# ClimateImpactLab/climate_toolbox

Hardware: AMD Instinct MI355X
Metric: gridcell-region-timesteps/sec (higher is better)
Workload: dtype f32

## Files before the change

climate_toolbox_amd/_lib.py:

```python
from __future__ import annotations

import ctypes as C
import os

_HERE = os.path.dirname(os.path.abspath(__file__))
LIB_PATH = os.path.join(_HERE, "lib", "libwagg.so")

EKEY, EINTERNAL = -6, -7
PLAN_NO_LC, PLAN_NO_STREAM, PLAN_NO_LINES, PLAN_LC_MFMA, PLAN_SERIAL_BUILD = 1, 2, 4, 8, 16
FORM_FULL, FORM_TILES, FORM_ENTRIES = 0, 1, 2
FORCE_FORM = {None: 0, "auto": 0, "full": 1, "tiles": 2, "entries": 3}
HOST_PIN, HOST_WHOLE, HOST_LINES, HOST_LINES_WHOLE = 1, 2, 4, 8
DENSE_GENERAL_SORT = 16
GATHER_AUTO, GATHER_RCCL, GATHER_PEER = 0, 1, 2
LAYOUT_TG, LAYOUT_GT = 0, 1
OUT_TR, OUT_RT = 0, 1

EXPORTS = (
    "wagg_version", "wagg_device_count", "wagg_shard_rows", "wagg_last_error", "wagg_profile_enable", "wagg_profile_read",
    "wagg_profile_event_overhead",
    "wagg_resolve_cells", "wagg_backup_fill", "wagg_relabel", "wagg_factorize_i64", "wagg_factorize_bytes",
    "wagg_plan_create", "wagg_plan_destroy", "wagg_plan_get_info", "wagg_plan_get_den", "wagg_plan_status",
    "wagg_apply_f32", "wagg_apply_f64", "wagg_apply_host_f32", "wagg_apply_host_f64",
    "wagg_apply_host_ex_f32", "wagg_apply_host_ex_f64", "wagg_dense_apply_host_f32", "wagg_dense_apply_host_f64",
    "wagg_apply_poly_f32", "wagg_apply_poly_f64", "wagg_apply_edd_f32", "wagg_apply_edd_f64",
    "wagg_apply_poly_host_f32", "wagg_apply_poly_host_f64", "wagg_apply_edd_host_f32", "wagg_apply_edd_host_f64",
    "wagg_gather_f32", "wagg_gather_f64",
    "wagg_transform_poly_f32", "wagg_transform_poly_f64", "wagg_transform_edd_f32", "wagg_transform_edd_f64",
    "wagg_any_less_f32", "wagg_any_less_f64",
    "wagg_dense_create_synth", "wagg_dense_create_host", "wagg_dense_create_from_segments", "wagg_dense_create_synth_blocklocal", "wagg_dense_create_synth_sparse", "wagg_dense_get_info",
    "wagg_dense_destroy", "wagg_dense_clone", "wagg_release_scratch", "wagg_scratch_bytes", "wagg_dense_get_den", "wagg_dense_apply_f32", "wagg_dense_apply_poly_f32",
    "wagg_dense_apply_edd_f32", "wagg_dense_saw_inf",
    "wagg_dense_create_synth_f64", "wagg_dense_create_host_f64", "wagg_dense_create_from_segments_f64",
    "wagg_dense_create_synth_blocklocal_f64", "wagg_dense_apply_f64", "wagg_dense_apply_poly_f64", "wagg_dense_apply_edd_f64",
    "wagg_synth_field_f32", "wagg_synth_field_f64",
    "wagg_apply_host_multi_f32", "wagg_apply_host_multi_f64", "wagg_dense_apply_host_multi_f32", "wagg_dense_apply_host_multi_f64",
    "wagg_host_block_plan", "wagg_host_stats_read",
    "wagg_combine_planes_f32", "wagg_combine_planes_f64", "wagg_take_axis", "wagg_relayout_f32", "wagg_relayout_f64",
    "wagg_dense_create_from_csr", "wagg_dense_create_from_csr_f64", "wagg_synth_table_csr", "wagg_relayout_to_f64", "wagg_upload",
    "wagg_shard_group_create", "wagg_shard_group_destroy", "wagg_shard_group_info",
    "wagg_apply_sharded_f32", "wagg_apply_sharded_f64", "wagg_dense_apply_sharded_f32", "wagg_dense_apply_sharded_f64",
    "wagg_apply", "wagg_struct_size", "wagg_struct_ordinals", "wagg_plan_get_info_sized", "wagg_dense_get_info_sized",
    "wagg_host_stats_read_sized",
    "wagg_plan_create_many", "wagg_plan_many_info", "wagg_plan_get_den_many",
    "wagg_period_reduce_f32", "wagg_period_reduce_f64", "wagg_period_reduce_work_bytes",
    "wagg_season_reduce_f32", "wagg_season_reduce_f64", "wagg_season_reduce_work_bytes", "wagg_season_mask",
    "wagg_edd_ladder_reduce_f32", "wagg_edd_ladder_reduce_f64", "wagg_edd_ladder_work_bytes",
    "wagg_bin_days_reduce_f32", "wagg_bin_days_reduce_f64", "wagg_bin_days_work_bytes",
    "wagg_hinge_reduce_f32", "wagg_hinge_reduce_f64", "wagg_hinge_work_bytes",
    "wagg_plan_compact_info", "wagg_plan_compact_cells", "wagg_pack_rows_f32", "wagg_pack_rows_f64",
    "wagg_pack_rows_host_f32", "wagg_pack_rows_host_f64",
)
STRUCT_PLAN_INFO, STRUCT_DENSE_INFO, STRUCT_HOST_STATS, STRUCT_APPLY_DESC = 0, 1, 2, 3
PLAN_SEGMENT, PLAN_DENSE = 0, 1
SRC_DEVICE, SRC_HOST, SRC_HOST_MULTI, SRC_SHARDED = 0, 1, 2, 3
XF_NONE, XF_POLY, XF_EDD = 0, 1, 2
APPLY_EXACT_F32 = 0x10000
APPLY_COMPACT_ROWS = 0x20000
EUNSUPPORTED = -5
T_F32, T_F64 = 7, 8
PERIOD_KEEP_NAN, PERIOD_ROWS_CHECKED = 1, 2
SEASON_INVERT, SEASON_NULL = 1 << 20, 1 << 21
EDD_LADDER_MAX, EDD_LADDER_GROUP = 64, 8
BIN_EDGES_MAX, BIN_GROUP = 65, 8
HINGE_MAX, HINGE_GROUP = 64, 8
HINGE_ABOVE, HINGE_BELOW = 0, 1


class HostStats(C.Structure):
    _fields_ = [(k, C.c_int64) for k in ("calls", "blocks", "registered", "register_failed", "unregistered", "unregister_failed",
                                         "cleanup_failed", "staged_h2d_bytes", "staged_d2h_bytes", "direct_h2d_bytes",
                                         "direct_d2h_bytes", "lines_h2d_bytes", "lines_wait_pack_us", "lines_wait_copy_us", "blocks_retired", "found_page_locked",
                                         "watched_calls", "last_rate_permille")]


def host_stats(reset=False):
    st = HostStats()
    check(load().wagg_host_stats_read_sized(C.byref(st), C.sizeof(st), 1 if reset else 0), "wagg_host_stats_read_sized")
    return {k: int(getattr(st, k)) for k, _ in HostStats._fields_}


def host_block_plan(T, row_bytes, quantum, n_devices=1):
    b, n = C.c_int64(0), C.c_int64(0)
    check(load().wagg_host_block_plan(int(T), int(row_bytes), int(quantum), int(n_devices), C.byref(b), C.byref(n)),
          "wagg_host_block_plan")
    return int(b.value), int(n.value)


class DenseInfo(C.Structure):
    _fields_ = [("G", C.c_int64), ("n_tiles", C.c_int64), ("w_bytes", C.c_int64),
                ("R", C.c_int32), ("n_kt", C.c_int32), ("n_nt", C.c_int32), ("tiled", C.c_int32),
                ("form", C.c_int32), ("elem_bytes", C.c_int32), ("nnz", C.c_int64),
                ("build_s", C.c_double), ("build_upload_s", C.c_double),
                ("est_full_s", C.c_double), ("est_tiles_s", C.c_double), ("est_entries_s", C.c_double), ("walked_entries", C.c_int64),
                ("one_pass_sort", C.c_int32), ("reserved0", C.c_int32)]


class WaggError(RuntimeError):
    pass


class PlanInfo(C.Structure):
    _fields_ = [("nseg_in", C.c_int64), ("nnz", C.c_int64), ("n_groups", C.c_int64),
                ("n_chunks", C.c_int64), ("n_ucells", C.c_int64), ("n_giant", C.c_int64),
                ("n_empty", C.c_int64), ("G", C.c_int64), ("R", C.c_int32), ("lines", C.c_int32),
                ("n_lines128", C.c_int64), ("n_sectors64", C.c_int64), ("n_partial_rows", C.c_int64),
                ("lines_chunks", C.c_int64), ("lines_ucells", C.c_int64), ("lines_lines128", C.c_int64),
                ("n_partial_rows64", C.c_int64), ("lines64_chunks", C.c_int64), ("lines64_ucells", C.c_int64)]


class ApplyDesc(C.Structure):
    _fields_ = [("struct_size", C.c_uint64), ("plan_kind", C.c_int32), ("elem", C.c_int32), ("source", C.c_int32), ("transform", C.c_int32),
                ("plan", C.c_void_p), ("x", C.c_void_p), ("x2", C.c_void_p), ("out", C.c_void_p),
                ("T", C.c_int64), ("ldx", C.c_int64), ("ldo", C.c_int64), ("out_pstride", C.c_int64),
                ("layout", C.c_int32), ("out_layout", C.c_int32), ("offset", C.c_double), ("pow_first", C.c_int32), ("n_pow", C.c_int32),
                ("thresholds", C.c_void_p), ("n_thr", C.c_int32), ("flags", C.c_int32), ("ksplit", C.c_int32), ("n_plans", C.c_int32),
                ("devices", C.c_void_p), ("rows", C.c_void_p), ("group", C.c_void_p), ("root", C.c_int32), ("reserved0", C.c_int32),
                ("stream", C.c_void_p)]


STRUCTS = {STRUCT_PLAN_INFO: PlanInfo, STRUCT_DENSE_INFO: DenseInfo, STRUCT_HOST_STATS: HostStats, STRUCT_APPLY_DESC: ApplyDesc}


def _ptr(v):
    if v is None:
        return None
    if isinstance(v, int):
        return v
    if isinstance(v, C.c_void_p):
        return v.value
    return C.cast(v, C.c_void_p).value


def run(what, **fields):
    d = ApplyDesc()
    d.struct_size = C.sizeof(ApplyDesc)
    d.pow_first = d.n_pow = 1
    for k, v in fields.items():
        setattr(d, k, _ptr(v) if k in _DESC_POINTERS else v)
    check(load().wagg_apply(C.byref(d)), what)


_DESC_POINTERS = frozenset(k for k, t in ApplyDesc._fields_ if t is C.c_void_p)

_lib = None


def load():
    global _lib
    if _lib is not None:
        return _lib
    if not os.path.exists(LIB_PATH):
        raise WaggError(
            "HIP engine not built: %s is missing. Run `python -c \"import __graft_entry__ as g; "
            "g.build()\"` or `make -C climate_toolbox_amd/csrc`. There is no CPU fallback." % LIB_PATH)
    import torch
    L = C.CDLL(LIB_PATH)
    vp, i32p, f64p, f32p = C.c_void_p, C.POINTER(C.c_int32), C.POINTER(C.c_double), C.POINTER(C.c_float)
    L.wagg_version.restype = C.c_int
    L.wagg_shard_rows.argtypes = [C.c_int64, C.c_int, C.c_int, C.POINTER(C.c_int64), C.POINTER(C.c_int64)]
    L.wagg_device_count.restype = C.c_int
    L.wagg_last_error.restype = C.c_char_p
    L.wagg_profile_enable.argtypes = [C.c_int]
    L.wagg_profile_read.argtypes = [f32p, C.c_int, C.POINTER(C.c_int)]
    L.wagg_profile_event_overhead.argtypes = [vp, C.c_int, f32p, f32p]
    u8p, i64p = C.POINTER(C.c_uint8), C.POINTER(C.c_int64)
    L.wagg_resolve_cells.argtypes = [f64p, C.c_int64, f64p, C.c_int64, f64p, f64p, C.c_int64, C.c_int, i32p, i64p]
    L.wagg_backup_fill.argtypes = [f64p, f64p, C.c_int64, f64p]
    L.wagg_relabel.argtypes = [f64p, C.c_int64, C.c_double, C.c_double]
    L.wagg_factorize_i64.argtypes = [i64p, u8p, C.c_int64, i32p, i64p, i64p]
    L.wagg_factorize_bytes.argtypes = [C.c_char_p, C.c_int64, u8p, C.c_int64, i32p, i64p, i64p]
    L.wagg_plan_create.argtypes = [i32p, i32p, f64p, C.c_int64, C.c_int64, C.c_int32, C.c_int64,
                                   C.c_int, C.POINTER(vp)]
    L.wagg_plan_create_many.argtypes = [i32p, i32p, C.POINTER(f64p), C.c_int, C.c_int64, C.c_int64, C.c_int32, C.c_int64,
                                        C.POINTER(i32p), i32p, C.c_int, C.c_int, C.POINTER(vp)]
    L.wagg_plan_many_info.argtypes = [vp, C.POINTER(C.c_int), C.POINTER(C.c_int), i32p, i64p]
    L.wagg_plan_get_den_many.argtypes = [vp, C.c_int, C.c_int, f64p]
    L.wagg_plan_destroy.argtypes = [vp]
    L.wagg_plan_get_info.argtypes = [vp, C.POINTER(PlanInfo)]
    L.wagg_plan_get_info_sized.argtypes = [vp, vp, C.c_uint64]
    L.wagg_dense_get_info_sized.argtypes = [vp, vp, C.c_uint64]
    L.wagg_host_stats_read_sized.argtypes = [vp, C.c_uint64, C.c_int]
    L.wagg_struct_size.argtypes = [C.c_int]
    L.wagg_struct_ordinals.argtypes = [C.c_int, vp, C.c_uint64]
    L.wagg_apply.argtypes = [C.POINTER(ApplyDesc)]
    L.wagg_plan_get_den.argtypes = [vp, f64p]
    L.wagg_plan_status.argtypes = [vp, vp]
    for name in ("wagg_apply_f32", "wagg_apply_f64"):
        getattr(L, name).argtypes = [vp, vp, C.c_int64, C.c_int64, C.c_int, vp, C.c_int64, C.c_int, vp]
    for name in ("wagg_apply_poly_f32", "wagg_apply_poly_f64"):
        getattr(L, name).argtypes = [vp, vp, C.c_int64, C.c_int64, C.c_int, C.c_double, C.c_int, C.c_int, vp,
                                     C.c_int64, C.c_int64, C.c_int, vp]
    for name in ("wagg_apply_poly_host_f32", "wagg_apply_poly_host_f64"):
        getattr(L, name).argtypes = [vp, vp, C.c_int64, C.c_int64, C.c_double, C.c_int, C.c_int, vp, C.c_int64, C.c_int64, C.c_int]
    for name in ("wagg_apply_edd_host_f32", "wagg_apply_edd_host_f64"):
        getattr(L, name).argtypes = [vp, vp, vp, C.c_int64, C.c_int64, C.c_double, f64p, C.c_int, vp, C.c_int64, C.c_int64, C.c_int]
    for name in ("wagg_apply_edd_f32", "wagg_apply_edd_f64"):
        getattr(L, name).argtypes = [vp, vp, vp, C.c_int64, C.c_int64, C.c_int, C.c_double, f64p, C.c_int, vp,
                                     C.c_int64, C.c_int64, C.c_int, vp]
    for name in ("wagg_apply_host_f32", "wagg_apply_host_f64"):
        getattr(L, name).argtypes = [vp, vp, C.c_int64, C.c_int64, C.c_int, vp, C.c_int64, C.c_int]
    for name in ("wagg_apply_host_ex_f32", "wagg_apply_host_ex_f64"):
        getattr(L, name).argtypes = [vp, vp, C.c_int64, C.c_int64, C.c_int, vp, C.c_int64, C.c_int, C.c_int]
    for name in ("wagg_dense_apply_host_f32", "wagg_dense_apply_host_f64"):
        getattr(L, name).argtypes = [vp, vp, C.c_int64, C.c_int64, vp, C.c_int64, C.c_int]
    for name in ("wagg_apply_host_multi_f32", "wagg_apply_host_multi_f64", "wagg_dense_apply_host_multi_f32",
                 "wagg_dense_apply_host_multi_f64"):
        getattr(L, name).argtypes = [C.POINTER(vp), i32p, C.c_int, vp, C.c_int64, C.c_int64, vp, C.c_int64, C.c_int]
    for name in ("wagg_combine_planes_f32", "wagg_combine_planes_f64"):
        getattr(L, name).argtypes = [vp, C.c_int, C.c_int64, f64p, C.c_int64, vp, vp]
    L.wagg_take_axis.argtypes = [vp, C.c_int64, C.c_int64, C.c_int64, vp, C.c_int64, vp, vp]
    for name in ("wagg_relayout_f32", "wagg_relayout_f64"):
        getattr(L, name).argtypes = [vp, C.c_int, C.POINTER(C.c_int64), C.POINTER(C.c_int64), vp, vp]
    L.wagg_relayout_to_f64.argtypes = [vp, C.c_int, C.c_int, C.POINTER(C.c_int64), C.POINTER(C.c_int64), vp, vp]
    L.wagg_upload.argtypes = [vp, vp, C.c_int64]
    L.wagg_host_block_plan.argtypes = [C.c_int64, C.c_int64, C.c_int64, C.c_int, C.POINTER(C.c_int64), C.POINTER(C.c_int64)]
    L.wagg_host_stats_read.argtypes = [C.POINTER(HostStats), C.c_int]
    for name in ("wagg_gather_f32", "wagg_gather_f64"):
        getattr(L, name).argtypes = [vp, C.c_int64, C.c_int64, C.c_int, vp, C.c_int64, vp, C.c_int64,
                                     C.c_int, vp]
    for name in ("wagg_transform_poly_f32", "wagg_transform_poly_f64"):
        getattr(L, name).argtypes = [vp, C.c_int64, C.c_double, C.c_int, vp, vp]
    for name in ("wagg_transform_edd_f32", "wagg_transform_edd_f64"):
        getattr(L, name).argtypes = [vp, vp, C.c_int64, C.c_double, f64p, f64p, C.c_int, vp, vp]
    for name in ("wagg_any_less_f32", "wagg_any_less_f64"):
        getattr(L, name).argtypes = [vp, vp, C.c_int64, C.POINTER(C.c_int), vp]
    L.wagg_dense_create_synth.argtypes = [C.c_int64, C.c_int32, C.c_uint32, C.POINTER(vp)]
    L.wagg_dense_create_host.argtypes = [f32p, C.c_int64, C.c_int32, C.POINTER(vp)]
    L.wagg_dense_create_from_segments.argtypes = [i32p, i32p, f64p, C.c_int64, C.c_int64, C.c_int32, C.c_int,
                                                  C.POINTER(vp)]
    L.wagg_dense_create_synth_blocklocal.argtypes = [C.c_int64, C.c_int32, C.c_uint32, C.c_double, C.POINTER(vp)]
    L.wagg_dense_create_synth_sparse.argtypes = [C.c_int64, C.c_int32, C.c_uint32, C.c_double, C.POINTER(vp)]
    L.wagg_dense_get_info.argtypes = [vp, C.POINTER(DenseInfo)]
    L.wagg_dense_destroy.argtypes = [vp]
    L.wagg_dense_clone.argtypes = [vp, C.c_int, C.POINTER(vp)]
    L.wagg_release_scratch.argtypes = []
    L.wagg_scratch_bytes.argtypes = []
    L.wagg_scratch_bytes.restype = C.c_int64
    L.wagg_dense_get_den.argtypes = [vp, f64p]
    L.wagg_dense_apply_f32.argtypes = [vp, vp, C.c_int64, C.c_int64, vp, C.c_int64, C.c_int, vp]
    L.wagg_dense_apply_poly_f32.argtypes = [vp, vp, C.c_int64, C.c_int64, C.c_double, C.c_int, vp, C.c_int64, C.c_int, vp]
    L.wagg_dense_apply_edd_f32.argtypes = [vp, vp, vp, C.c_int64, C.c_int64, C.c_double, C.c_double, vp, C.c_int64,
                                           C.c_int, vp]
    L.wagg_dense_saw_inf.argtypes = [vp, vp, C.POINTER(C.c_int)]
    L.wagg_dense_create_synth_f64.argtypes = [C.c_int64, C.c_int32, C.c_uint32, C.c_double, C.POINTER(vp)]
    L.wagg_dense_create_synth_blocklocal_f64.argtypes = [C.c_int64, C.c_int32, C.c_uint32, C.c_double, C.POINTER(vp)]
    L.wagg_dense_create_host_f64.argtypes = [f64p, C.c_int64, C.c_int32, C.POINTER(vp)]
    L.wagg_dense_create_from_segments_f64.argtypes = [i32p, i32p, f64p, C.c_int64, C.c_int64, C.c_int32, C.c_int, C.POINTER(vp)]
    for name in ("wagg_dense_create_from_csr", "wagg_dense_create_from_csr_f64"):
        getattr(L, name).argtypes = [i64p, i32p, f64p, C.c_int64, C.c_int32, C.c_int, C.POINTER(vp)]
    L.wagg_synth_table_csr.argtypes = [C.c_int64, C.c_int32, C.c_uint32, C.c_double, C.c_int, i64p, i32p, f64p, C.c_int64, i64p]
    L.wagg_dense_apply_f64.argtypes = [vp, vp, C.c_int64, C.c_int64, vp, C.c_int64, C.c_int, vp]
    L.wagg_dense_apply_poly_f64.argtypes = [vp, vp, C.c_int64, C.c_int64, C.c_double, C.c_int, vp, C.c_int64, C.c_int, vp]
    L.wagg_dense_apply_edd_f64.argtypes = [vp, vp, vp, C.c_int64, C.c_int64, C.c_double, C.c_double, vp, C.c_int64,
                                           C.c_int, vp]
    L.wagg_synth_field_f32.argtypes = [vp, C.c_int64, C.c_int64, C.c_int64, C.c_uint32, C.c_float,
                                       C.c_float, vp]
    L.wagg_synth_field_f64.argtypes = [vp, C.c_int64, C.c_int64, C.c_int64, C.c_uint32, C.c_double,
                                       C.c_double, vp]
    L.wagg_shard_group_create.argtypes = [i32p, C.c_int, C.c_int, C.POINTER(vp)]
    L.wagg_shard_group_destroy.argtypes = [vp]
    L.wagg_shard_group_info.argtypes = [vp, C.POINTER(C.c_int), C.POINTER(C.c_int)]
    for name in ("wagg_apply_sharded_f32", "wagg_apply_sharded_f64", "wagg_dense_apply_sharded_f32", "wagg_dense_apply_sharded_f64"):
        getattr(L, name).argtypes = [vp, C.POINTER(vp), C.POINTER(vp), i64p, C.c_int64, vp, C.c_int64, C.c_int]
    for name in ("wagg_period_reduce_f32", "wagg_period_reduce_f64"):
        getattr(L, name).argtypes = [vp, vp, C.c_int64, C.c_int64, C.c_int64, vp, vp, C.c_int32, C.c_int64, C.c_int, C.c_double, C.c_int,
                                     C.c_int, f64p, C.c_int, C.c_int, vp, C.c_int64, C.c_int64, vp, vp, C.c_int64, vp]
    L.wagg_period_reduce_work_bytes.argtypes = [C.c_int64, C.c_int32, C.c_int64, C.c_int]
    L.wagg_period_reduce_work_bytes.restype = C.c_int64
    for name in ("wagg_season_reduce_f32", "wagg_season_reduce_f64"):
        getattr(L, name).argtypes = [vp, vp, C.c_int64, C.c_int64, C.c_int64, vp, vp, C.c_int32, C.c_int64, vp, vp, C.c_int, C.c_double,
                                     C.c_int, C.c_int, f64p, C.c_int, C.c_int, vp, C.c_int64, C.c_int64, vp, vp, C.c_int64, vp]
    L.wagg_season_reduce_work_bytes.argtypes = [C.c_int64, C.c_int32, C.c_int64, C.c_int]
    L.wagg_season_reduce_work_bytes.restype = C.c_int64
    L.wagg_season_mask.argtypes = [vp, C.c_int64, vp, C.c_int64, vp, vp]
    for name in ("wagg_edd_ladder_reduce_f32", "wagg_edd_ladder_reduce_f64"):
        getattr(L, name).argtypes = [vp, vp, C.c_int64, C.c_int64, C.c_int64, vp, vp, C.c_int32, C.c_int64, vp, vp, C.c_double, f64p,
                                     C.c_int, C.c_int, vp, C.c_int64, C.c_int64, vp, vp, C.c_int64, vp]
    L.wagg_edd_ladder_work_bytes.argtypes = [C.c_int64, C.c_int32, C.c_int64, C.c_int]
    L.wagg_edd_ladder_work_bytes.restype = C.c_int64
    for name in ("wagg_bin_days_reduce_f32", "wagg_bin_days_reduce_f64"):
        getattr(L, name).argtypes = [vp, C.c_int64, C.c_int64, C.c_int64, vp, vp, C.c_int32, C.c_int64, vp, vp, C.c_double, f64p, C.c_int,
                                     C.c_int, vp, C.c_int64, C.c_int64, vp, vp, C.c_int64, vp]
    L.wagg_bin_days_work_bytes.argtypes = [C.c_int64, C.c_int32, C.c_int64, C.c_int]
    L.wagg_bin_days_work_bytes.restype = C.c_int64
    for name in ("wagg_hinge_reduce_f32", "wagg_hinge_reduce_f64"):
        getattr(L, name).argtypes = [vp, C.c_int64, C.c_int64, C.c_int64, vp, vp, C.c_int32, C.c_int64, vp, vp, C.c_double, f64p, C.c_int,
                                     C.c_int, C.c_int, f64p, f64p, f64p, C.c_int, vp, C.c_int64, C.c_int64, vp, vp, C.c_int64, vp]
    L.wagg_hinge_work_bytes.argtypes = [C.c_int64, C.c_int32, C.c_int64, C.c_int]
    L.wagg_hinge_work_bytes.restype = C.c_int64
    L.wagg_plan_compact_info.argtypes = [vp, C.c_int, i64p]
    L.wagg_plan_compact_cells.argtypes = [vp, C.c_int, i32p]
    for name in ("wagg_pack_rows_f32", "wagg_pack_rows_f64"):
        getattr(L, name).argtypes = [vp, vp, vp, C.c_int64, C.c_int64, vp, C.c_int64, vp]
    for name in ("wagg_pack_rows_host_f32", "wagg_pack_rows_host_f64"):
        getattr(L, name).argtypes = [vp, vp, vp, C.c_int64, C.c_int64, vp, C.c_int64, C.c_int]
    for name in EXPORTS:
        fn = getattr(L, name)
        if name not in ("wagg_last_error", "wagg_scratch_bytes", "wagg_period_reduce_work_bytes", "wagg_season_reduce_work_bytes",
                        "wagg_edd_ladder_work_bytes", "wagg_bin_days_work_bytes", "wagg_hinge_work_bytes"):
            fn.restype = C.c_int
    _lib = L
    return L


def check(rc, what):
    if rc != 0:
        msg = load().wagg_last_error().decode("utf-8", "replace")
        err = WaggError("%s failed (%d): %s" % (what, rc, msg))
        err.code = int(rc)
        raise err
```

climate_toolbox_amd/csrc/wagg_common.h:

```cpp
#pragma once
#include <hip/hip_runtime.h>
#include <hip/hip_ext.h>
#include <cstdarg>
#include <cstdint>
#include <cstdio>
#include <cstring>
#include <new>
#include <vector>

#include "../../include/wagg.h"

namespace wagg {

void set_error(const char *fmt, ...);

#define WAGG_HIP(expr)                                                                        \
    do {                                                                                      \
        hipError_t e__ = (expr);                                                              \
        if (e__ != hipSuccess) {                                                              \
            wagg::set_error("%s:%d: %s -> %s", __FILE__, __LINE__, #expr,                     \
                            hipGetErrorString(e__));                                          \
            return WAGG_EHIP;                                                                 \
        }                                                                                     \
    } while (0)

#define WAGG_REQUIRE(cond, ...)                                                               \
    do {                                                                                      \
        if (!(cond)) {                                                                        \
            wagg::set_error(__VA_ARGS__);                                                     \
            return WAGG_EINVAL;                                                               \
        }                                                                                     \
    } while (0)

__host__ __device__ inline uint32_t hash32(uint64_t idx, uint32_t seed) {
    uint32_t lo = (uint32_t)idx, hi = (uint32_t)(idx >> 32);
    uint32_t x = lo ^ (hi * 0x85EBCA6Bu) ^ (seed * 0x9E3779B9u);
    x ^= x >> 16; x *= 0x7FEB352Du; x ^= x >> 15; x *= 0x846CA68Bu; x ^= x >> 16;
    return x;
}
__host__ __device__ inline float hash_u01(uint64_t idx, uint32_t seed) {
    return (float)(hash32(idx, seed) >> 8) * (1.0f / 16777216.0f);
}

constexpr int XF_EDD = -1;

template <typename T> __device__ __forceinline__ T snyder_edd1(T tmin, T tmax, T e) {
    const T M = (tmax + tmin) / T(2), w = (tmax - tmin) / T(2);
    if (!(tmin < e)) return M - e;
    if (!(tmax > e)) return T(0);
    const T pi = T(3.14159265358979323846);
    const T z = (e - M) / w;
    T theta, c;
    if constexpr (sizeof(T) == 4) { theta = asinf(z); c = sqrtf((T(1) - z) * (T(1) + z)); }
    else { theta = asin(z); c = sqrt((T(1) - z) * (T(1) + z)); }
    const T r = ((M - e) * (pi / T(2) - theta) + w * c) / pi;
    return r < T(0) ? T(0) : r;
}

__device__ __forceinline__ float snyder_edd1_finite(float tmin, float tmax, float e) {
    const float M = 0.5f * (tmax + tmin), w = 0.5f * (tmax - tmin);
    const float d = M - e;
    const float z = -d * __builtin_amdgcn_rcpf(w);
    const bool below = tmin < e;
    const float az = (below && tmax > e) ? __builtin_fminf(__builtin_fabsf(z), 1.0f) : 1.0f;
    const float t = 1.0f - az;
    float p = 7.577220821985975e-05f;
    p = __builtin_fmaf(p, az, -0.0003951705584768206f);
    p = __builtin_fmaf(p, az, 0.0010792884277179837f);
    p = __builtin_fmaf(p, az, -0.002406827174127102f);
    p = __builtin_fmaf(p, az, 0.005977150052785873f);
    p = __builtin_fmaf(p, az, -0.022534651681780815f);
    p = __builtin_fmaf(p, az, 0.31830987334251404f);
    const float q = __builtin_amdgcn_sqrtf(t) * t;
    return __builtin_fmaf(w, q * p, below ? __builtin_fmaxf(d, 0.0f) : d);
}
__device__ __forceinline__ double snyder_edd1_finite(double tmin, double tmax, double e) {
    const double M = 0.5 * (tmax + tmin), w = 0.5 * (tmax - tmin);
    const double d = M - e;
    double rw = __builtin_amdgcn_rcp(w);
    rw = __builtin_fma(rw, __builtin_fma(-w, rw, 1.0), rw);
    const bool below = tmin < e;
    const double az = (below && tmax > e) ? __builtin_fmin(__builtin_fabs(d * rw), 1.0) : 1.0;
    const double t = 1.0 - az;
    const double ty = __builtin_amdgcn_rsq(__builtin_fmax(t, 1e-300));
    double st = t * ty;
    st = __builtin_fma(__builtin_fma(-st, st, t), 0.5 * ty, st);
    double p = -8.644295123170258e-07;
    p = __builtin_fma(p, az, 7.147532263874047e-06);
    p = __builtin_fma(p, az, -2.807399717529102e-05);
    p = __builtin_fma(p, az, 7.126284961634285e-05);
    p = __builtin_fma(p, az, -0.0001359898123558899);
    p = __builtin_fma(p, az, 0.0002182750865254441);
    p = __builtin_fma(p, az, -0.0003242640574299061);
    p = __builtin_fma(p, az, 0.000480605991421148);
    p = __builtin_fma(p, az, -0.0007477719612718598);
    p = __builtin_fma(p, az, 0.0012691227365052833);
    p = __builtin_fma(p, az, -0.0024647062510063378);
    p = __builtin_fma(p, az, 0.005985979570242935);
    p = __builtin_fma(p, az, -0.0225351707225776);
    p = __builtin_fma(p, az, 0.3183098861837864);
    return __builtin_fma(w, st * t * p, below ? __builtin_fmax(d, 0.0) : d);
}
template <> __device__ __forceinline__ float snyder_edd1<float>(float tmin, float tmax, float e) {
    const float d = 0.5f * (tmax + tmin) - e;
    const float inner = snyder_edd1_finite(tmin, tmax, e);
    return !(tmin < e) ? d : (!(tmax > e) ? 0.0f : inner);
}

template <typename T> __device__ __forceinline__ T xform1(T x, T off, int pw) {
    const T y = x + off;
    T r = y;
    for (int i = 1; i < pw; ++i) r *= y;
    return r;
}
template <typename V, typename T> __device__ __forceinline__ V xform4(V v, T off, int pw) {
    V r;
#pragma unroll
    for (int c = 0; c < 4; ++c) r[c] = xform1<T>(v[c], off, pw);
    return r;
}

void copy_sized(void *dst, uint64_t dst_size, const void *src, size_t src_size);

hipError_t allow_dynamic_lds(const void *kern, size_t bytes);

bool profile_slot(hipEvent_t *start, hipEvent_t *stop);

inline hipError_t launch_timed_ptr(bool timed, const void *kern, dim3 grid, dim3 block, void **args, size_t shmem, hipStream_t st) {
    hipEvent_t a = nullptr, b = nullptr;
    if (timed && profile_slot(&a, &b)) return hipExtLaunchKernel(kern, grid, block, args, shmem, st, a, b, 0);
    return hipLaunchKernel(kern, grid, block, args, shmem, st);
}
template <typename... Args, typename F = void (*)(Args...)>
inline void launch_timed(bool timed, F kern, dim3 grid, dim3 block, size_t shmem, hipStream_t st, Args... args) {
    hipEvent_t a = nullptr, b = nullptr;
    if (timed && profile_slot(&a, &b)) hipExtLaunchKernelGGL(kern, grid, block, (std::uint32_t)shmem, st, a, b, 0u, args...);
    else hipLaunchKernelGGL(kern, grid, block, shmem, st, args...);
}

hipError_t staged_h2d(void *dst_dev, const void *src_host, size_t bytes, hipStream_t st);
hipError_t staged_d2h_rows(void *dst_host, const void *src_dev, int64_t rows, size_t ld_bytes, size_t row_bytes, hipStream_t st);
inline hipError_t staged_d2h(void *dst_host, const void *src_dev, size_t bytes, hipStream_t st = nullptr) {
    return staged_d2h_rows(dst_host, src_dev, 1, bytes, bytes, st);
}
void clear_error();

hipError_t scratch_alloc(void **p, size_t bytes);
void scratch_free(void *p, bool keep = true);
hipError_t scratch_stream(hipStream_t *st, int role = 0);
void scratch_stream_done(hipStream_t st, int role = 0, bool keep = true);
void release_scratch(int what = 7);
template <typename T>
struct ScratchBuf {
    T *p = nullptr;
    ScratchBuf() = default;
    ScratchBuf(const ScratchBuf &) = delete;
    ScratchBuf &operator=(const ScratchBuf &) = delete;
    hipError_t alloc(size_t count) { return scratch_alloc(reinterpret_cast<void **>(&p), (count ? count : 1) * sizeof(T)); }
    ~ScratchBuf() { if (p) { (void)hipDeviceSynchronize(); scratch_free(p); } }
};

template <typename T>
struct DevBuf {
    T *p = nullptr;
    size_t n = 0;
    DevBuf() = default;
    DevBuf(const DevBuf &) = delete;
    DevBuf &operator=(const DevBuf &) = delete;
    ~DevBuf() { if (p) (void)hipFree(p); }
    hipError_t alloc(size_t count) {
        if (p) { (void)hipFree(p); p = nullptr; }
        n = count;
        hipError_t e = hipMalloc((void **)&p, (count ? count : 1) * sizeof(T));
        if (e == hipErrorOutOfMemory) {
            (void)hipGetLastError();
            release_scratch();
            e = hipMalloc((void **)&p, (count ? count : 1) * sizeof(T));
        }
        return e;
    }
    hipError_t upload(const std::vector<T> &h, hipStream_t st = nullptr) {
        hipError_t e = alloc(h.size());
        if (e != hipSuccess || h.empty()) return e;
        return staged_h2d(p, h.data(), h.size() * sizeof(T), st);
    }
};

}
```

climate_toolbox_amd/csrc/wagg_dense.hip:

```cpp
#include <algorithm>
#include <cfloat>
#include <chrono>
#include <cmath>
#include <limits>
#include <cstdlib>
#include <type_traits>

#include "wagg_dense_int.h"
#include "wagg_entry.h"

namespace wagg {

constexpr int D_MT = 23;
constexpr int D_BN = 256;
constexpr int D_ROWB = 128;
constexpr int D_THREADS = 512;
constexpr int D_WTB = D_BN * D_ROWB;
constexpr int D_WSLOTS = D_WTB / 16;
static_assert(D_WTB / 1024 == 32, "4 one-KiB W pieces per wave");
constexpr int d_xt_bytes(int mt) { return mt * 16 * D_ROWB; }
constexpr int d_buf_bytes(int mt) { return d_xt_bytes(mt) + D_WTB; }
static_assert(2 * d_buf_bytes(D_MT) <= 160 * 1024, "LDS budget");

typedef float f32x4 __attribute__((ext_vector_type(4)));
// ... 159 lines not shown
    }
    (void)R;
}

__global__ void dense_colsum_combine_kernel(const double *__restrict__ part, int n_strips, int n_nt, int32_t R,
                                            double *__restrict__ den) {
    const int64_t r = (int64_t)blockIdx.x * blockDim.x + threadIdx.x;
    if (r >= R) return;
    const int64_t nt = r / D_BN, c = r % D_BN;
    double s = 0.0;
    for (int st = 0; st < n_strips; ++st)
        for (int p = 0; p < 8; ++p) s += part[((int64_t)st * n_nt + nt) * D_WSLOTS + c * 8 + p];
    den[r] = s;
}

__global__ void dense_den32_kernel(const double *__restrict__ den64, float *__restrict__ den32, int32_t R) {
    const int r = blockIdx.x * blockDim.x + threadIdx.x;
    if (r < R) den32[r] = (float)den64[r];
}

template <typename T>
__global__ void dense_scatter_kernel(T *__restrict__ Wp, int n_kt, const int32_t *__restrict__ cell,
                                     const int32_t *__restrict__ region, const T *__restrict__ w, int64_t n) {
    const int64_t i = (int64_t)blockIdx.x * blockDim.x + threadIdx.x;
    if (i < n) Wp[wp_index<T>(cell[i], region[i], n_kt)] = w[i];
}

template <typename T>
__global__ void dense_scatter_at_kernel(T *__restrict__ Wp, const int64_t *__restrict__ at,
                                        const T *__restrict__ w, int64_t n) {
    const int64_t i = (int64_t)blockIdx.x * blockDim.x + threadIdx.x;
    if (i < n) Wp[at[i]] = w[i];
}

template <typename T>
__global__ void dense_synth_blocklocal_kernel(typename DT<T>::vec *__restrict__ Wp, const int32_t *__restrict__ tile_kt,
                                              const int32_t *__restrict__ tile_nt, int64_t n_tiles, int64_t G,
                                              int32_t R, uint32_t seed, float fill) {
    const int64_t stride = (int64_t)gridDim.x * blockDim.x, n_slots = n_tiles * D_WSLOTS;
    for (int64_t s = (int64_t)blockIdx.x * blockDim.x + threadIdx.x; s < n_slots; s += stride) {
        const int64_t ti = s / D_WSLOTS;
        const int64_t kt = tile_kt[ti], nt = tile_nt[ti];
        int cl, kl;
        slot_to_ck<T>((int)(s % D_WSLOTS), cl, kl);
        const int64_t r = nt * D_BN + cl, g0 = kt * DT<T>::BK + kl;
        typename DT<T>::vec v;
#pragma unroll
        for (int c = 0; c < DT<T>::EPP; ++c) {
            const uint64_t id = (uint64_t)(g0 + c) * (uint64_t)R + (uint64_t)r;
            v[c] = (r < R && g0 + c < G && hash_u01(id, seed ^ 0x9e3779b9u) < fill) ? (T)hash_u01(id, seed) : T(0);
        }
        Wp[s] = v;
    }
}

template <typename T>
__global__ void dense_colsum_tiled_kernel(const typename DT<T>::vec *__restrict__ Wp, const int32_t *__restrict__ tile_first,
                                          int32_t R, double *__restrict__ den) {
    const int64_t r = (int64_t)blockIdx.x * blockDim.x + threadIdx.x;
    if (r >= R) return;
    const int64_t nt = r / D_BN, c = r % D_BN;
    double s = 0.0;
    for (int64_t ti = tile_first[nt]; ti < tile_first[nt + 1]; ++ti)
        for (int p = 0; p < 8; ++p) {
            const typename DT<T>::vec v = Wp[ti * D_WSLOTS + c * 8 + p];
#pragma unroll
            for (int e = 0; e < DT<T>::EPP; ++e) s += (double)v[e];
        }
    den[r] = s;
}

template <typename T>
__global__ void dense_pack_w_kernel(const T *__restrict__ W, int64_t G, int32_t R, int n_kt,
                                    int64_t n_slots, typename DT<T>::vec *__restrict__ Wp) {
    const int64_t stride = (int64_t)gridDim.x * blockDim.x;
    for (int64_t s = (int64_t)blockIdx.x * blockDim.x + threadIdx.x; s < n_slots; s += stride) {
        const int64_t tk = s / D_WSLOTS;
        const int64_t kt = tk % n_kt, nt = tk / n_kt;
        int cl, kl;
        slot_to_ck<T>((int)(s % D_WSLOTS), cl, kl);
        const int64_t r = nt * D_BN + cl, g0 = kt * DT<T>::BK + kl;
        typename DT<T>::vec v;
#pragma unroll
        for (int c = 0; c < DT<T>::EPP; ++c) v[c] = (r < R && g0 + c < G) ? W[(g0 + c) * R + r] : T(0);
        Wp[s] = v;
    }
}

}

namespace wagg {

template <typename T>
static int dense_alloc(int64_t G, int32_t R, wagg_dense **out, int64_t stored_tiles = -1, bool spmm = false) {
    constexpr int BK = DT<T>::BK;
    WAGG_REQUIRE(out != nullptr, "out is NULL");
    *out = nullptr;
    WAGG_REQUIRE(G > 0 && R > 0, "bad sizes G=%lld R=%d", (long long)G, R);
    WAGG_REQUIRE((G + BK - 1) / BK < (int64_t)0x7fffffff / 8, "G too large");
    wagg_dense *d = new (std::nothrow) wagg_dense();
    if (!d) { set_error("host allocation failed"); return WAGG_ENOMEM; }
    d->G = G; d->R = R;
    d->f64 = sizeof(T) == 8;
    d->n_kt = (int)((G + BK - 1) / BK);
    d->n_nt = (int)(((int64_t)R + D_BN - 1) / D_BN);
    d->n_tiles = spmm ? 0 : (stored_tiles >= 0 ? stored_tiles : (int64_t)d->n_nt * d->n_kt);
    d->tiled = !spmm && stored_tiles >= 0;
    d->spmm = spmm;
    int dev = 0;
    hipError_t e = hipGetDevice(&dev);
    d->device = dev;
    if (e == hipSuccess) e = hipDeviceGetAttribute(&d->ncu, hipDeviceAttributeMultiprocessorCount, dev);
    if (e == hipSuccess) e = d->nonfinite.alloc(1);
    if (e == hipSuccess) e = hipHostMalloc((void **)&d->inf_host, 2 * sizeof(int), hipHostMallocMapped);
    if (e == hipSuccess) { d->inf_host[0] = d->inf_host[1] = 0; e = hipHostGetDevicePointer((void **)&d->inf_dev, d->inf_host, 0); }
    if (e == hipSuccess) e = d->W.alloc((size_t)(d->w_slots() > 0 ? d->w_slots() : 1) * 4);
    if (e == hipSuccess) e = d->den32.alloc((size_t)R);
    if (e == hipSuccess) e = d->den64.alloc((size_t)R);
    if (e != hipSuccess) {
        set_error("dense W allocation of %.1f GB failed: %s", (double)d->w_slots() * 16e-9, hipGetErrorString(e));
        delete d;
        return e == hipErrorOutOfMemory ? WAGG_ENOMEM : WAGG_EHIP;
    }
    *out = d;
    return WAGG_OK;
}

static int dense_den_to_host(wagg_dense *d, hipStream_t st = nullptr) {
    hipLaunchKernelGGL(dense_den32_kernel, dim3((unsigned)((d->R + 255) / 256)), dim3(256), 0, st,
                       d->den64.p, d->den32.p, d->R);
    WAGG_HIP(hipGetLastError());
    d->den_host.resize((size_t)d->R);
    WAGG_HIP(staged_d2h(d->den_host.data(), d->den64.p, sizeof(double) * (size_t)d->R, st));
    return WAGG_OK;
}

template <typename T>
static int dense_finish_den(wagg_dense *d) {
    typedef typename DT<T>::vec vec_t;
    const int kt_per_block = 128;
    const int n_strips = (d->n_kt + kt_per_block - 1) / kt_per_block;
    dim3 grid((unsigned)d->n_nt, (unsigned)n_strips);
    DevBuf<double> part;
    WAGG_HIP(part.alloc((size_t)n_strips * (size_t)d->n_nt * D_WSLOTS));
    hipLaunchKernelGGL((dense_colsum_kernel<T>), grid, dim3(512), 0, nullptr,
                       reinterpret_cast<const vec_t *>(d->W.p), d->R, d->n_kt, kt_per_block, part.p);
    hipLaunchKernelGGL(dense_colsum_combine_kernel, dim3((unsigned)((d->R + 255) / 256)), dim3(256), 0, nullptr,
                       (const double *)part.p, n_strips, d->n_nt, d->R, d->den64.p);
    WAGG_HIP(hipGetLastError());
    WAGG_HIP(hipDeviceSynchronize());
    return dense_den_to_host(d);
}

static int dense_finish_scales(wagg_dense *d, hipStream_t st = nullptr) {
    if (d->f64 || d->tiled || d->spmm) return WAGG_OK;
    const int kt_per_block = 128;
    const int n_strips = (d->n_kt + kt_per_block - 1) / kt_per_block;
    WAGG_HIP(d->wmax.alloc((size_t)d->n_nt * D_BN));
    WAGG_HIP(hipMemsetAsync(d->wmax.p, 0, sizeof(float) * d->wmax.n, st));
    hipLaunchKernelGGL(dense_colmax_kernel, dim3((unsigned)d->n_nt, (unsigned)n_strips), dim3(512), 0, st,
                       reinterpret_cast<const f32x4 *>(d->W.p), d->n_kt, kt_per_block, reinterpret_cast<unsigned *>(d->wmax.p));
    WAGG_HIP(hipGetLastError());
    return WAGG_OK;
}

static hipError_t dense_set_tiles(wagg_dense *d, const std::vector<int64_t> &tiles, std::vector<int32_t> *nt_out = nullptr,
                                  hipStream_t st = nullptr) {
    std::vector<int32_t> kt(tiles.size() + 2, 0), ntv(tiles.size() + 1, 0);
    std::vector<int64_t> first((size_t)d->n_nt + 1, 0);
    for (size_t i = 0; i < tiles.size(); ++i) {
        kt[i] = (int32_t)(tiles[i] % d->n_kt);
        ntv[i] = (int32_t)(tiles[i] / d->n_kt);
        first[(size_t)ntv[i] + 1]++;
    }
    for (int nt = 0; nt < d->n_nt; ++nt) first[(size_t)nt + 1] += first[(size_t)nt];
    d->nt_first.assign(first.size(), 0);
    for (size_t i = 0; i < first.size(); ++i) d->nt_first[i] = (int32_t)first[i];
    hipError_t e = d->tile_kt.upload(kt, st);
    if (nt_out) *nt_out = ntv;
    return e;
}

static int tile_pieces_for(wagg_dense *d, int n_mb, hipStream_t st, const wagg_dense::TilePieces **out) {
    for (const auto &tp : d->pieces)
        if (tp->n_mb == n_mb) { *out = tp.get(); return WAGG_OK; }
    try {
        std::unique_ptr<wagg_dense::TilePieces> tp(new wagg_dense::TilePieces());
        const int n_nt = d->n_nt;
        const int64_t per_mb = d->n_tiles, total = per_mb * n_mb;
        int64_t n_wg = total / 8;
        if (n_wg > d->ncu) n_wg = d->ncu;
        if (n_wg < 1) n_wg = 1;
        std::vector<int32_t> first_piece((size_t)n_wg + 1, 0), rec, slab_first(2 * (size_t)n_mb * n_nt, 0);
        int64_t pos = 0;
        int slab = 0, w = 0;
        int64_t w_end = total * 1 / n_wg;
        bool nt_major = false;
#ifdef WAGG_DIAG
        if (const char *e = getenv("WAGG_PIECES_ORDER")) nt_major = e[0] == 'n';
#endif
        for (int64_t pair = 0; pair < (int64_t)n_mb * n_nt; ++pair) {
            const int mb = nt_major ? (int)(pair % n_mb) : (int)(pair / n_nt), nt = nt_major ? (int)(pair / n_mb) : (int)(pair % n_nt);
            {
                const int slab0 = slab;
                slab_first[2 * ((size_t)mb * n_nt + nt)] = slab;
                int64_t t0 = d->nt_first[(size_t)nt];
                const int64_t t1 = d->nt_first[(size_t)nt + 1];
                while (t0 < t1) {
                    while (pos >= w_end && w + 1 < n_wg) { ++w; first_piece[(size_t)w] = (int32_t)(rec.size() / 8); w_end = total * (w + 1) / n_wg; }
                    const int64_t room = w + 1 < n_wg ? w_end - pos : t1 - t0;
                    const int64_t take = room < t1 - t0 ? room : t1 - t0;
                    const int32_t r8[8] = {nt, mb, (int32_t)t0, (int32_t)take, slab, 0, 0, 0};
                    rec.insert(rec.end(), r8, r8 + 8);
                    ++slab;
                    t0 += take;
                    pos += take;
                }
                slab_first[2 * ((size_t)mb * n_nt + nt) + 1] = slab - slab0;
            }
        }
        for (int64_t k = w + 1; k <= n_wg; ++k) first_piece[(size_t)k] = (int32_t)(rec.size() / 8);
        tp->n_mb = n_mb; tp->n_wg = (int)n_wg; tp->n_slabs = slab;
        std::vector<int32_t> all;
        all.reserve(first_piece.size() + rec.size() + slab_first.size());
        all.insert(all.end(), first_piece.begin(), first_piece.end());
        all.insert(all.end(), rec.begin(), rec.end());
        tp->slab_first_at = (int64_t)all.size();
        all.insert(all.end(), slab_first.begin(), slab_first.end());
        WAGG_HIP(tp->tab.upload(all, st));
        *out = tp.get();
        d->pieces.push_back(std::move(tp));
        return WAGG_OK;
    } catch (const std::bad_alloc &) { set_error("host allocation failed"); return WAGG_ENOMEM; }
}

constexpr double SPMM_MAX_FILL = 0.10;

struct FormRates { double full, tiled, entries_scale, dma; };
constexpr FormRates FORM_RATES_F32 = {420e12, 144e12, 1.0, 10.1e12};
constexpr FormRates FORM_RATES_F64 = {70e12, 73e12, 0.44, 10.1e12};
static double entry_loop_rate(double mean_list) {
    static const double L[] = {170, 325, 541, 812, 1625}, Rt[] = {30e12, 23e12, 19.5e12, 17.3e12, 15.9e12};
    if (mean_list <= L[0]) return Rt[0];
    for (int i = 1; i < 5; ++i)
        if (mean_list <= L[i]) return Rt[i - 1] + (Rt[i] - Rt[i - 1]) * (mean_list - L[i - 1]) / (L[i] - L[i - 1]);
    return Rt[4];
}

struct FormCost { double t_full, t_tiled, t_entries; };
static FormCost table_form_cost(int64_t G, int elem_bytes, int64_t n_tiles_stored, int64_t n_tiles_all, int64_t walked, int n_rb,
                                int64_t n_lists, int n_nt) {
    const FormRates &rt = elem_bytes == 8 ? FORM_RATES_F64 : FORM_RATES_F32;
    const double tile_flop = 2.0 * (128.0 / elem_bytes) * 256.0;
    FormCost c;
    const int64_t n_kt = n_tiles_all / (n_nt > 0 ? n_nt : 1);
    const double s_max = n_kt / 32 >= 64 ? 64.0 : (n_kt / 32 >= 16 ? (double)(n_kt / 32 / 8 * 8) : 8.0);
    const double util = n_nt * s_max < 256.0 ? n_nt * s_max / 256.0 : 1.0;
    c.t_full = tile_flop * (double)n_tiles_all / (rt.full * util);
    c.t_tiled = tile_flop * (double)n_tiles_stored / rt.tiled;
    const double rate = rt.entries_scale * entry_loop_rate((double)walked / (double)(n_lists > 0 ? n_lists : 1));
    const double t_loop = 2.0 * (double)walked / rate, t_stream = (double)elem_bytes * (double)G * (double)n_rb / rt.dma;
    c.t_entries = t_loop > t_stream ? t_loop : t_stream;
    return c;
}
static void pick_table_form(const FormCost &c, bool *tiled, bool *entries) {
    *entries = c.t_entries < c.t_full && c.t_entries < c.t_tiled;
    *tiled = !*entries && c.t_tiled < c.t_full;
}

static int pick_ksplit(int64_t items, int n_kt) {
    int best = 8;
    double best_eff = 0.0;
    for (int S = 8; S <= 64; S += 8) {
        if (S > 8 && n_kt / S < 32) break;
        const double w = (double)items * S / 256.0;
        const double eff = w / std::ceil(w);
        if (eff > best_eff + 1e-9) { best_eff = eff; best = S; }
        if (eff >= 0.985) break;
    }
    return best;
}

template <typename T>
static int create_synth(int64_t G, int32_t R, uint32_t seed, double fill, wagg_dense **out) {
    typedef typename DT<T>::vec vec_t;
    WAGG_REQUIRE(fill > 0.0 && fill <= 1.0, "fill must be in (0, 1]");
    if (fill < SPMM_MAX_FILL) {
        int rc = dense_alloc<T>(G, R, out, -1, true);
        if (rc != WAGG_OK) return rc;
        rc = spmm_build_synth<T>(*out, seed, fill);
        if (rc != WAGG_OK) { delete *out; *out = nullptr; }
        return rc;
    }
    int rc = dense_alloc<T>(G, R, out);
    if (rc != WAGG_OK) return rc;
    wagg_dense *d = *out;
    hipLaunchKernelGGL((dense_synth_w_kernel<T>), dim3(256 * 32), dim3(256), 0, nullptr,
                       reinterpret_cast<vec_t *>(d->W.p), G, R, d->n_kt, d->w_slots(), seed, (float)fill);
    hipError_t e = hipGetLastError();
    if (e == hipSuccess) rc = dense_finish_den<T>(d); else { set_error("synth launch: %s", hipGetErrorString(e)); rc = WAGG_EHIP; }
    if (rc == WAGG_OK) rc = dense_finish_scales(d);
    if (rc == WAGG_OK && hipDeviceSynchronize() != hipSuccess) { set_error("synth: column maxima"); rc = WAGG_EHIP; }
    if (rc != WAGG_OK) { delete d; *out = nullptr; }
    return rc;
}

template <typename T>
static int create_synth_blocklocal(int64_t G, int32_t R, uint32_t seed, double fill, wagg_dense **out) {
    typedef typename DT<T>::vec vec_t;
    constexpr int BK = DT<T>::BK;
    WAGG_REQUIRE(out != nullptr, "out is NULL");
    *out = nullptr;
    WAGG_REQUIRE(G > 0 && R > 0 && fill > 0.0 && fill <= 1.0, "bad arguments");
    const int n_kt = (int)((G + BK - 1) / BK), n_nt = (int)(((int64_t)R + D_BN - 1) / D_BN);
    std::vector<int64_t> tiles;
    tiles.reserve((size_t)n_kt);
    for (int kt = 0; kt < n_kt; ++kt) tiles.push_back((int64_t)(((int64_t)97 * (kt / (64 / BK))) % n_nt) * n_kt + kt);
    std::sort(tiles.begin(), tiles.end());
    int rc = dense_alloc<T>(G, R, out, (int64_t)tiles.size());
    if (rc != WAGG_OK) return rc;
    wagg_dense *d = *out;
    std::vector<int32_t> ntv;
    DevBuf<int32_t> dnt, dfirst;
    hipError_t e = dense_set_tiles(d, tiles, &ntv);
    if (e == hipSuccess) e = dnt.upload(ntv);
    if (e == hipSuccess) {
        std::vector<int32_t> first((size_t)n_nt + 1, 0);
        for (size_t i = 0; i < tiles.size(); ++i) first[(size_t)ntv[i] + 1]++;
        for (int nt = 0; nt < n_nt; ++nt) first[(size_t)nt + 1] += first[(size_t)nt];
        e = dfirst.upload(first);
    }
    if (e == hipSuccess) {
        hipLaunchKernelGGL((dense_synth_blocklocal_kernel<T>), dim3(256 * 16), dim3(256), 0, nullptr,
                           reinterpret_cast<vec_t *>(d->W.p), d->tile_kt.p, dnt.p, d->n_tiles, G, R, seed, (float)fill);
        e = hipGetLastError();
    }
    if (e == hipSuccess) {
        hipLaunchKernelGGL((dense_colsum_tiled_kernel<T>), dim3((unsigned)((R + 255) / 256)), dim3(256), 0, nullptr,
                           reinterpret_cast<const vec_t *>(d->W.p), (const int32_t *)dfirst.p, R, d->den64.p);
        e = hipGetLastError();
    }
    if (e != hipSuccess) { set_error("block-local synth: %s", hipGetErrorString(e)); delete d; *out = nullptr; return WAGG_EHIP; }
    rc = dense_den_to_host(d);
    if (rc != WAGG_OK) { delete d; *out = nullptr; }
    return rc;
}

template <typename T>
static int create_host(const T *W_host, int64_t G, int32_t R, wagg_dense **out) {
    typedef typename DT<T>::vec vec_t;
    WAGG_REQUIRE(W_host != nullptr, "W_host is NULL");
    int rc = dense_alloc<T>(G, R, out);
    if (rc != WAGG_OK) return rc;
    wagg_dense *d = *out;
    DevBuf<T> plain;
    hipError_t e = plain.alloc((size_t)(G * R));
    if (e == hipSuccess && copy_to_device(plain.p, W_host, sizeof(T) * (size_t)(G * R), true) != WAGG_OK) { delete d; *out = nullptr; return WAGG_EHIP; }
    if (e == hipSuccess) {
        hipLaunchKernelGGL((dense_pack_w_kernel<T>), dim3(256 * 8), dim3(256), 0, nullptr, (const T *)plain.p, G, R, d->n_kt,
                           d->w_slots(), reinterpret_cast<vec_t *>(d->W.p));
        e = hipGetLastError();
    }
    if (e == hipSuccess) e = hipDeviceSynchronize();
    if (e != hipSuccess) { set_error("dense upload: %s", hipGetErrorString(e)); delete d; *out = nullptr; return WAGG_EHIP; }
    rc = dense_finish_den<T>(d);
    if (rc == WAGG_OK) rc = dense_finish_scales(d);
    if (rc == WAGG_OK && hipDeviceSynchronize() != hipSuccess) { set_error("dense upload: column maxima"); rc = WAGG_EHIP; }
    if (rc != WAGG_OK) { delete d; *out = nullptr; }
    return rc;
}

template <typename T>
__global__ __launch_bounds__(256) void table_tiles_kernel(const uint64_t *__restrict__ key, int64_t n, EntryKeyGeom geom, int n_kt,
                                                          uint32_t *__restrict__ bitmap) {
    const int64_t i = (int64_t)blockIdx.x * blockDim.x + threadIdx.x;
    const int lane = threadIdx.x & 63;
    int64_t t = -1;
    if (i < n) {
        int64_t cell; int32_t region; int cic, j;
        geom.decode(key[i], cell, region, cic, j);
        t = (int64_t)(region / D_BN) * n_kt + cell / DT<T>::BK;
    }
    uint64_t todo = __ballot(i < n);
    while (todo) {
        const int leader = __ffsll((unsigned long long)todo) - 1;
        const int64_t tl = __shfl(t, leader, 64);
        if (lane == leader) atomicOr(&bitmap[tl >> 5], 1u << (tl & 31));
        todo &= ~__ballot(t == tl);
    }
}

template <typename T>
__global__ __launch_bounds__(256) void table_scatter_kernel(const uint64_t *__restrict__ key, const double *__restrict__ w, int64_t n,
                                                            EntryKeyGeom geom, int n_kt, const uint32_t *__restrict__ bitmap,
                                                            const uint32_t *__restrict__ word_rank, T *__restrict__ Wp) {
    constexpr int E = DT<T>::EPP, BK = DT<T>::BK;
    const int64_t i = (int64_t)blockIdx.x * blockDim.x + threadIdx.x;
    if (i >= n) return;
    int64_t cell; int32_t region; int cic, j;
    geom.decode(key[i], cell, region, cic, j);
    int64_t at;
    if (word_rank) {
        const int64_t t = (int64_t)(region / D_BN) * n_kt + cell / BK;
        const int64_t ti = (int64_t)word_rank[t >> 5] + __popc(bitmap[t >> 5] & ((1u << (t & 31)) - 1u));
        const int cl = region % D_BN, kk = (int)(cell % BK);
        at = (ti * D_WSLOTS + tile_slot(cl, kk / E)) * E + (kk % E);
    } else {
        at = wp_index<T>(cell, region, n_kt);
    }
    Wp[at] = (T)w[i];
}

static double wall_s() { return std::chrono::duration<double>(std::chrono::steady_clock::now().time_since_epoch()).count(); }

template <typename T>
static int create_from_table(const int32_t *cell_idx, const int64_t *rowptr, const int32_t *region_code, const double *w_eff,
                             int64_t n, int64_t G, int32_t R, int flags, wagg_dense **out) {
    constexpr int BK = DT<T>::BK;
    WAGG_REQUIRE(out != nullptr, "out is NULL");
    *out = nullptr;
    WAGG_REQUIRE(G > 0 && R > 0, "bad sizes G=%lld R=%d", (long long)G, R);
    const bool general_sort = (flags & WAGG_DENSE_GENERAL_SORT) != 0;
    flags &= ~WAGG_DENSE_GENERAL_SORT;
    WAGG_REQUIRE(flags >= WAGG_DENSE_FORM_AUTO && flags <= WAGG_DENSE_FORCE_ENTRIES, "unknown form flag %d", flags);
    if (rowptr) {
        WAGG_REQUIRE(rowptr[0] == 0, "rowptr[0] must be 0");
        for (int64_t g = 0; g < G; ++g) WAGG_REQUIRE(rowptr[g] <= rowptr[g + 1], "rowptr decreases at row %lld", (long long)g);
        n = rowptr[G];
    }
    WAGG_REQUIRE(n >= 0 && n < (int64_t)0x7fffffff, "table of %lld rows: at most 2^31 - 1", (long long)n);
    WAGG_REQUIRE(n == 0 || ((cell_idx || rowptr) && region_code && w_eff), "NULL table arrays");
    const double t0 = wall_s();
    SpmmPlan geo;
// ... 5 lines not shown
    const int64_t n_buckets = (int64_t)geo.n_rb * geo.n_chunks * SP_WAVES;
    const size_t after_sort = 2 * (sizeof(uint32_t) * (size_t)n_words + 512) + 2 * (sizeof(int32_t) * ((size_t)n_buckets + 1) + 512) +
                              sizeof(uint32_t) * ((size_t)n_buckets / 2048 + 2) + 8192;
    size_t arena = build_arena_bytes(n, G, R, rowptr != nullptr);
    if (rowptr) arena += chunk_sort_scratch_bytes(kg);
    if (arena < after_sort) arena = after_sort;
    BuildCtx ctx;
    WAGG_BUILD_STAMP(ctx, "^start");
    {
        const hipError_t e = ctx.init(arena);
        if (e != hipSuccess) {
            set_error("plan build: %.2f GB of device scratch for a table of %lld rows -> %s", (double)arena * 1e-9, (long long)n, hipGetErrorString(e));
            return e == hipErrorOutOfMemory ? WAGG_ENOMEM : WAGG_EHIP;
        }
    }
    WAGG_BUILD_STAMP(ctx, "arena");
    SortedEntries se;
    double t_up = 0.0;
    {
        int32_t *dcell = nullptr, *dreg = nullptr;
        int64_t *drow = nullptr;
        double *dw = nullptr;
        if (n > 0) {
            if (rowptr) { drow = ctx.take_input<int64_t>((size_t)G + 1); } else { dcell = ctx.take_input<int32_t>((size_t)n); }
            dreg = ctx.take_input<int32_t>((size_t)n);
            dw = ctx.take_input<double>((size_t)n);
            if (!(drow || dcell) || !dreg || !dw) { set_error("build arena too small for the table"); return WAGG_ENOMEM; }
            int rc = rowptr ? copy_to_device(drow, rowptr, sizeof(int64_t) * ((size_t)G + 1), true, ctx.st)
                            : copy_to_device(dcell, cell_idx, sizeof(int32_t) * (size_t)n, true, ctx.st);
            if (rc == WAGG_OK) rc = copy_to_device(dreg, region_code, sizeof(int32_t) * (size_t)n, true, ctx.st);
            if (rc == WAGG_OK) rc = copy_to_device(dw, w_eff, sizeof(double) * (size_t)n, true, ctx.st);
            if (rc != WAGG_OK) return rc;
        }
        t_up = wall_s() - t0;
        WAGG_BUILD_STAMP(ctx, "upload");
        if (int rc = build_sorted_entries(ctx, dcell, drow, dreg, dw, n, G, R, kg, &se, general_sort)) return rc;
    }
    uint32_t *bitmap, *word_rank = nullptr;
    WAGG_TAKE(bitmap, ctx, uint32_t, n_words);
    WAGG_HIP(hipMemsetAsync(bitmap, 0, sizeof(uint32_t) * (size_t)n_words, ctx.st));
    const unsigned nblk = (unsigned)((se.n_u + 255) / 256);
    if (se.n_u > 0) {
        hipLaunchKernelGGL((table_tiles_kernel<T>), dim3(nblk), dim3(256), 0, ctx.st, (const uint64_t *)se.key.p, se.n_u, kg, n_kt, bitmap);
        WAGG_HIP(hipGetLastError());
    }
    WAGG_BUILD_STAMP(ctx, "den + tile census");
    std::vector<uint32_t> hbits, hrank;
    std::vector<int64_t> tiles;
    try {
        hbits.resize((size_t)n_words);
        hrank.resize((size_t)n_words);
        WAGG_HIP(staged_d2h(hbits.data(), bitmap, sizeof(uint32_t) * hbits.size(), ctx.st));
        int64_t cnt = 0;
        for (int64_t i = 0; i < n_words; ++i) { hrank[(size_t)i] = (uint32_t)cnt; cnt += __builtin_popcount(hbits[(size_t)i]); }
        tiles.reserve((size_t)cnt);
        for (int64_t i = 0; i < n_words; ++i)
            for (uint32_t m = hbits[(size_t)i]; m; m &= m - 1) tiles.push_back(i * 32 + __builtin_ctz(m));
    } catch (const std::bad_alloc &) { set_error("host allocation failed"); return WAGG_ENOMEM; }
    const double fill_all = (double)se.n_u / ((double)G * (double)R);
    int64_t walked = 0;
    if (se.n_u > 0) { if (int rc = spmm_list_cost(ctx, se, &walked)) return rc; }
    WAGG_BUILD_STAMP(ctx, "bitmap to host + list cost");
    const FormCost cost = table_form_cost(G, (int)sizeof(T), (int64_t)tiles.size(), n_tiles_all, walked, geo.n_rb, n_buckets, n_nt);
    bool tiled, entries;
    pick_table_form(cost, &tiled, &entries);
    if (flags == WAGG_DENSE_FORCE_FULL) { tiled = false; entries = false; }
    else if (flags == WAGG_DENSE_FORCE_TILES) { tiled = true; entries = false; }
    else if (flags == WAGG_DENSE_FORCE_ENTRIES) { tiled = false; entries = true; }
#ifdef WAGG_DIAG
    if (getenv("WAGG_DENSE_NO_TILED") && tiled) { tiled = false; entries = fill_all < SPMM_MAX_FILL; }
#else
    (void)fill_all;
#endif
    int rc = dense_alloc<T>(G, R, out, tiled ? (int64_t)tiles.size() : -1, entries);
    if (rc != WAGG_OK) return rc;
    wagg_dense *d = *out;
    WAGG_BUILD_STAMP(ctx, "plan alloc");
    auto fail = [&](int code) { (void)ctx.sync(); delete d; *out = nullptr; return code; };
    if (entries) {
        ctx.release_to(0);
        rc = spmm_build_from_sorted<T>(ctx, d, se);
        if (rc != WAGG_OK) return fail(rc);
    } else {
        hipError_t e = hipMemsetAsync(d->W.p, 0, 16 * (size_t)d->w_slots(), ctx.st);
        if (e == hipSuccess && tiled) e = dense_set_tiles(d, tiles, nullptr, ctx.st);
        if (e == hipSuccess && tiled) {
            word_rank = ctx.take<uint32_t>((size_t)n_words);
            e = word_rank ? staged_h2d(word_rank, hrank.data(), sizeof(uint32_t) * hrank.size(), ctx.st) : hipErrorOutOfMemory;
        }
        if (e == hipSuccess && se.n_u > 0) {
            hipLaunchKernelGGL((table_scatter_kernel<T>), dim3(nblk), dim3(256), 0, ctx.st, (const uint64_t *)se.key.p, (const double *)se.w.p,
                               se.n_u, kg, n_kt, (const uint32_t *)bitmap, (const uint32_t *)word_rank, reinterpret_cast<T *>(d->W.p));
            e = hipGetLastError();
        }
        if (e != hipSuccess) { set_error("densify: %s", hipGetErrorString(e)); return fail(WAGG_EHIP); }
    }
    hipError_t e = hipMemcpyAsync(d->den64.p, se.den.p, sizeof(double) * (size_t)R, hipMemcpyDeviceToDevice, ctx.st);
    if (e != hipSuccess) { set_error("densify den: %s", hipGetErrorString(e)); return fail(WAGG_EHIP); }
    rc = dense_den_to_host(d, ctx.st);
    if (rc == WAGG_OK) rc = dense_finish_scales(d, ctx.st);
    if (rc != WAGG_OK) return fail(rc);
    e = ctx.sync();
    if (e != hipSuccess) { set_error("plan build: %s", hipGetErrorString(e)); return fail(WAGG_EHIP); }
    WAGG_BUILD_STAMP(ctx, "pack + den to host");
    if (entries) d->sp.nnz = se.n_u;
    d->nnz_table = se.n_u;
    d->est_row_s[0] = cost.t_full; d->est_row_s[1] = cost.t_tiled; d->est_row_s[2] = cost.t_entries;
    d->walked_entries = walked;
    d->one_pass_sort = se.chunkwise;
    d->build.upload_s = t_up;
    d->build.total_s = wall_s() - t0;
    d->build.device_s = d->build.total_s - t_up;
    return WAGG_OK;
}

template <typename T, bool TILED, int MT, bool RM = false>
static const void *mfma_kernel_ptr() {
    if constexpr (TILED) return (const void *)dense_pieces_kernel<T, MT, RM>;
    else return (const void *)dense_mfma_kernel<T, 0, false, MT, RM>;
}
template <typename T>
static const void *pick_full_rm_kernel(int MT, bool rm) {
#define WAGG_PICK(M) case M: return rm ? (const void *)dense_mfma_kernel<T, 0, false, M, true> \
                                       : (const void *)dense_mfma_kernel<T, 256, false, M, false>
    if constexpr (sizeof(T) == 4) {
        switch (MT) { WAGG_PICK(20); WAGG_PICK(21); WAGG_PICK(22); WAGG_PICK(23); default: return nullptr; }
    } else {
        switch (MT) { WAGG_PICK(10); WAGG_PICK(11); default: return nullptr; }
    }
#undef WAGG_PICK
}

template <typename T>
static const void *pick_mfma_kernel(int MT, bool tiled, bool rm = false) {
#define WAGG_PICK(M) case M: return tiled ? (rm ? mfma_kernel_ptr<T, true, M, true>() : mfma_kernel_ptr<T, true, M>()) \
                                          : mfma_kernel_ptr<T, false, M>()
    if constexpr (sizeof(T) == 4) {
        switch (MT) {
            WAGG_PICK(1); WAGG_PICK(2); WAGG_PICK(3); WAGG_PICK(4); WAGG_PICK(5); WAGG_PICK(6); WAGG_PICK(8);
            WAGG_PICK(10); WAGG_PICK(12); WAGG_PICK(14); WAGG_PICK(16); WAGG_PICK(18); WAGG_PICK(20);
            WAGG_PICK(21); WAGG_PICK(22); WAGG_PICK(23);
            default: return nullptr;
        }
    } else {
        switch (MT) {
            WAGG_PICK(1); WAGG_PICK(2); WAGG_PICK(3); WAGG_PICK(4); WAGG_PICK(5); WAGG_PICK(6); WAGG_PICK(8);
            WAGG_PICK(10); WAGG_PICK(11);
            default: return nullptr;
        }
    }
#undef WAGG_PICK
}

static const void *pick_split_kernel(int MT) {
#define WAGG_PICK(M) case M: return (const void *)dense_split_kernel<M>
    switch (MT) {
        WAGG_PICK(1); WAGG_PICK(2); WAGG_PICK(3); WAGG_PICK(4); WAGG_PICK(5); WAGG_PICK(6); WAGG_PICK(8);
        WAGG_PICK(10); WAGG_PICK(12); WAGG_PICK(14); WAGG_PICK(16); WAGG_PICK(18); WAGG_PICK(20);
        WAGG_PICK(21); WAGG_PICK(22); WAGG_PICK(23);
        default: return nullptr;
    }
#undef WAGG_PICK
}

static int dense_apply_split(wagg_dense *d, const float *X_dev, int64_t Tn, int64_t ldx, const PackXfT<float> &xf,
                             float *out_dev, int64_t ldo, int MT, int n_mb, int S, hipStream_t st) {
    const int n_nt = d->n_nt, n_kt = d->n_kt, bm = MT * 16;
    const int kt_per_slice = (n_kt + S - 1) / S;
    const int64_t nblk = (int64_t)n_nt * n_mb * S;
    WAGG_REQUIRE(nblk < (int64_t)0x7fffffff, "grid too large");
    const void *kern = pick_split_kernel(MT);
    if (!kern) { set_error("no split kernel for MT=%d", MT); return WAGG_EINVAL; }
    const size_t need = (size_t)nblk * bm * D_BN;
    if (d->slabs.n < need) WAGG_HIP(d->slabs.alloc(need));
    const int64_t x_slots = (int64_t)n_mb * n_kt * bm * 8;
    if (d->xp.n < (size_t)x_slots * 4) WAGG_HIP(d->xp.alloc((size_t)x_slots * 4));
    if (d->xmax.n < (size_t)Tn) WAGG_HIP(d->xmax.alloc((size_t)Tn));
    const int aligned = ((ldx * sizeof(float)) % 16 == 0) && ((reinterpret_cast<uintptr_t>(X_dev) & 15) == 0) &&
                        (xf.mode != XF_EDD || (reinterpret_cast<uintptr_t>(xf.X2) & 15) == 0);
#ifdef WAGG_DIAG
    if (const char *dbg = MT == D_MT ? getenv("WAGG_SPLIT_DBG") : nullptr) {
        switch (atoi(dbg)) {
            case 1: kern = (const void *)dense_split_kernel<D_MT, 1>; break;
            case 4: kern = (const void *)dense_split_kernel<D_MT, 4>; break;
            case 5: kern = (const void *)dense_split_kernel<D_MT, 5>; break;
            case 8: kern = (const void *)dense_split_kernel<D_MT, 8>; break;
            case 9: kern = (const void *)dense_split_kernel<D_MT, 9>; break;
            default: break;
        }
    }
#endif
    const size_t shmem = 3 * (size_t)d_xt_bytes(MT);
    WAGG_HIP(allow_dynamic_lds(kern, shmem));
    unsigned *xmax = reinterpret_cast<unsigned *>(d->xmax.p);
    WAGG_HIP(hipMemsetAsync(xmax, 0, sizeof(unsigned) * (size_t)Tn, st));
    const int64_t gx = (d->G + 4095) / 4096 < 64 ? (d->G + 4095) / 4096 : 64;
    hipLaunchKernelGGL(dense_rowmax_kernel, dim3((unsigned)gx, (unsigned)Tn), dim3(256), 0, st, X_dev, ldx, d->G, xf, xmax);
    hipLaunchKernelGGL(dense_pack_x_split_kernel, dim3(256 * 16), dim3(256), 0, st, X_dev, Tn, ldx, d->G, n_kt, bm, x_slots, aligned,
                       (const unsigned *)xmax, reinterpret_cast<f16x8 *>(d->xp.p), xf, d->inf_dev);
    WAGG_HIP(hipGetLastError());
    const f16x8 *xp = reinterpret_cast<const f16x8 *>(d->xp.p);
    const float *wp = d->W.p, *wmax = d->wmax.p;
    float *slabs = d->slabs.p;
    int n_kt_a = n_kt, n_nt_a = n_nt, n_mb_a = n_mb, S_a = S, kps = kt_per_slice;
    void *args[] = {&xp, &wp, &wmax, &n_kt_a, &n_nt_a, &n_mb_a, &S_a, &kps, &slabs};
    WAGG_HIP(launch_timed_ptr(true, kern, dim3((unsigned)nblk), dim3(D_THREADS), args, shmem, st));
    hipLaunchKernelGGL(dense_reduce_split_kernel, dim3((unsigned)((d->R + 255) / 256), (unsigned)Tn), dim3(256), 0, st,
                       (const float *)slabs, n_nt, S, bm, d->R, (const float *)d->den32.p, (const unsigned *)xmax, wmax, out_dev, ldo);
    WAGG_HIP(hipGetLastError());
    return WAGG_OK;
}

template <typename T>
static int dense_apply(wagg_dense *d, const T *X_dev, int64_t Tn, int64_t ldx, const PackXfT<T> &xf,
                       T *out_dev, int64_t ldo, int ksplit, void *stream, bool exact = false) {
    typedef typename DT<T>::vec vec_t;
    WAGG_REQUIRE(d != nullptr, "dense plan is NULL");
    WAGG_REQUIRE(d->f64 == (sizeof(T) == 8), "this plan holds %s weights: use the matching wagg_dense_apply_*",
                 d->f64 ? "fp64" : "fp32");
    WAGG_REQUIRE(Tn >= 0, "T < 0");
    if (Tn == 0) return WAGG_OK;
    WAGG_REQUIRE(X_dev && out_dev, "X/out is NULL");
    WAGG_REQUIRE(xf.mode != XF_EDD || xf.X2 != nullptr, "tasmax is NULL");
    WAGG_REQUIRE(ldx >= d->G && ldo >= d->R, "ldx/ldo too small");
    WAGG_REQUIRE(ksplit >= 0 && ksplit % 8 == 0, "ksplit must be 0 or a multiple of 8");
    if (d->spmm) return spmm_apply<T>(d, X_dev, Tn, ldx, xf, out_dev, ldo, (hipStream_t)stream);
    constexpr int64_t ROWS_MAX = (int64_t)(65535 / (DT<T>::MT_MAX * 16)) * (DT<T>::MT_MAX * 16);
    if (Tn > ROWS_MAX) {
        for (int64_t t0 = 0; t0 < Tn; t0 += ROWS_MAX) {
            PackXfT<T> xg = xf;
            if (xg.X2) xg.X2 += t0 * ldx;
            const int64_t rows = Tn - t0 < ROWS_MAX ? Tn - t0 : ROWS_MAX;
            if (int rc = dense_apply<T>(d, X_dev + t0 * ldx, rows, ldx, xg, out_dev + t0 * ldo, ldo, ksplit, stream, exact)) return rc;
        }
        return WAGG_OK;
    }
    const int n_nt = d->n_nt, n_kt = d->n_kt;
    constexpr int BM_MAX = DT<T>::MT_MAX * 16;
    const int n_mb = (int)((Tn + BM_MAX - 1) / BM_MAX);
    const int rows = (int)((Tn + n_mb - 1) / n_mb);
    static const int mts32[] = {1, 2, 3, 4, 5, 6, 8, 10, 12, 14, 16, 18, 20, 21, 22, 23};
    static const int mts64[] = {1, 2, 3, 4, 5, 6, 8, 10, 11};
    int MT = DT<T>::MT_MAX;
    if constexpr (sizeof(T) == 4) { for (int m : mts32) if (m * 16 >= rows) { MT = m; break; } }
    else { for (int m : mts64) if (m * 16 >= rows) { MT = m; break; } }
    const int bm = MT * 16;
    if (n_mb >= 2) {
        const int64_t head = (int64_t)(n_mb - 1) * bm, tail = Tn - head;
        if (tail > 0) {
            int MT_tail = DT<T>::MT_MAX;
            if constexpr (sizeof(T) == 4) { for (int m : mts32) if ((int64_t)m * 16 >= tail) { MT_tail = m; break; } }
            else { for (int m : mts64) if ((int64_t)m * 16 >= tail) { MT_tail = m; break; } }
            if (MT_tail >= 4 && MT - MT_tail >= 2) {
                PackXfT<T> xt = xf;
                if (xt.X2) xt.X2 += head * ldx;
                if (int rc = dense_apply<T>(d, X_dev, head, ldx, xf, out_dev, ldo, ksplit, stream, exact)) return rc;
                return dense_apply<T>(d, X_dev + head * ldx, tail, ldx, xt, out_dev + head * ldo, ldo, ksplit, stream, exact);
            }
        }
    }
    int S = ksplit ? ksplit : pick_ksplit((int64_t)n_nt * n_mb, n_kt);
    if constexpr (sizeof(T) == 4) {
        if (!d->tiled && !exact && d->wmax.p != nullptr) return dense_apply_split(d, X_dev, Tn, ldx, xf, out_dev, ldo, MT, n_mb, S, (hipStream_t)stream);
    }
    const wagg_dense::TilePieces *tp = nullptr;
    if (d->tiled) {
        if (int rc = tile_pieces_for(d, n_mb, (hipStream_t)stream, &tp)) return rc;
        S = 1;
    }
    const int kt_per_slice = (n_kt + S - 1) / S;
    const int64_t nblk = tp ? (int64_t)tp->n_wg : (int64_t)n_nt * n_mb * S;
    WAGG_REQUIRE(nblk < (int64_t)0x7fffffff, "grid too large");
    const size_t n_slabs = tp ? (size_t)tp->n_slabs : (size_t)n_nt * n_mb * S;
    const size_t need = (n_slabs ? n_slabs : 1) * bm * D_BN * (sizeof(T) / 4);
    if (d->slabs.n < need) WAGG_HIP(d->slabs.alloc(need));
    const int64_t x_slots = (int64_t)n_mb * n_kt * bm * 8;
    if (d->xp.n < (size_t)x_slots * 4) WAGG_HIP(d->xp.alloc((size_t)x_slots * 4));
    const int aligned = ((ldx * sizeof(T)) % 16 == 0) && ((reinterpret_cast<uintptr_t>(X_dev) & 15) == 0) &&
                        (xf.mode != XF_EDD || (reinterpret_cast<uintptr_t>(xf.X2) & 15) == 0);
    const size_t shmem = 2 * (size_t)d_buf_bytes(MT);
    hipStream_t st = (hipStream_t)stream;
    const void *kern = pick_mfma_kernel<T>(MT, d->tiled);
    if (!kern) { set_error("no kernel for MT=%d", MT); return WAGG_EINVAL; }
    bool rm = xf.mode == 0 && aligned && d->G % DT<T>::BK == 0 && ((volatile int *)d->inf_host)[1] == 0;
    const void *kern_rm = nullptr;
    if (rm && d->tiled) kern_rm = pick_mfma_kernel<T>(MT, true, true);
    else if (rm && n_mb >= 2 && (kern_rm = pick_full_rm_kernel<T>(MT, true)) != nullptr) kern = pick_full_rm_kernel<T>(MT, false);
    rm = kern_rm != nullptr;
    if (rm) WAGG_HIP(allow_dynamic_lds(kern_rm, shmem));
#ifdef WAGG_DIAG
    if (getenv("WAGG_DENSE_PACKED") || (!d->tiled && getenv("WAGG_DENSE_DBG"))) {
        rm = false; kern_rm = nullptr;
        kern = pick_mfma_kernel<T>(MT, d->tiled);
    }
    if constexpr (sizeof(T) == 4) {
        if (const char *dbg = (d->tiled || MT != D_MT) ? nullptr : getenv("WAGG_DENSE_DBG")) {
            switch (atoi(dbg)) {
                case 1: kern = (const void *)dense_mfma_kernel<float, 1>; break;
                case 4: kern = (const void *)dense_mfma_kernel<float, 4>; break;
                case 5: kern = (const void *)dense_mfma_kernel<float, 5>; break;
                case 8: kern = (const void *)dense_mfma_kernel<float, 8>; break;
                case 16: kern = (const void *)dense_mfma_kernel<float, 16>; break;
                case 32: kern = (const void *)dense_mfma_kernel<float, 32>; break;
                case 64: kern = (const void *)dense_mfma_kernel<float, 64>; break;
                case 96: kern = (const void *)dense_mfma_kernel<float, 96>; break;
                case 128: kern = (const void *)dense_mfma_kernel<float, 128>; break;
                case 160: kern = (const void *)dense_mfma_kernel<float, 160>; break;
                case 192: kern = (const void *)dense_mfma_kernel<float, 192>; break;
                case 224: kern = (const void *)dense_mfma_kernel<float, 224>; break;
                default: break;
            }
        }
    }
#endif
    WAGG_HIP(allow_dynamic_lds(kern, shmem));
    const T *xp = reinterpret_cast<const T *>(d->xp.p), *wp = reinterpret_cast<const T *>(d->W.p);
    T *slabs = reinterpret_cast<T *>(d->slabs.p);
    int n_kt_a = n_kt, n_nt_a = n_nt, n_mb_a = n_mb, S_a = S, kps = kt_per_slice;
    const int32_t *tkt = d->tile_kt.p;
    const int32_t *toff = tp ? tp->tab.p : nullptr;
    const int32_t *slab_first = tp ? tp->tab.p + tp->slab_first_at : nullptr;
    int64_t ldxB = ldx * (int64_t)sizeof(T);
    int Tn_a = (int)Tn;
    const T *den;
    if constexpr (sizeof(T) == 4) den = d->den32.p; else den = d->den64.p;
    const dim3 rgrid((unsigned)((d->R + 255) / 256), (unsigned)Tn);
    const int *gate = nullptr;
    if (rm) {
        gate = d->nonfinite.p;
        WAGG_HIP(hipMemsetAsync(d->nonfinite.p, 0, sizeof(int), st));
        const int *no_gate = nullptr;
        void *args_rm[] = {&X_dev, &wp, &n_kt_a, &n_nt_a, &n_mb_a, &S_a, &kps, &slabs, &tkt, &toff, &ldxB, &Tn_a, &no_gate};
        WAGG_HIP(launch_timed_ptr(true, kern_rm, dim3((unsigned)nblk), dim3(D_THREADS), args_rm, shmem, st));
        hipLaunchKernelGGL((dense_reduce_kernel<T>), rgrid, dim3(256), 0, st, (const T *)slabs, n_nt, S, bm, Tn, d->R, den,
                           out_dev, ldo, d->nonfinite.p, (const int *)nullptr, d->inf_dev + 1, slab_first);
        WAGG_HIP(hipGetLastError());
    }
    hipLaunchKernelGGL((dense_pack_x_kernel<T>), dim3(256 * 16), dim3(256), 0, st, X_dev, Tn, ldx, d->G, n_kt, bm, x_slots,
                       aligned, reinterpret_cast<vec_t *>(d->xp.p), xf, d->inf_dev, gate);
    WAGG_HIP(hipGetLastError());
    void *args[] = {&xp, &wp, &n_kt_a, &n_nt_a, &n_mb_a, &S_a, &kps, &slabs, &tkt, &toff, &ldxB, &Tn_a, &gate};
    WAGG_HIP(launch_timed_ptr(!rm, kern, dim3((unsigned)nblk), dim3(D_THREADS), args, shmem, st));
    hipLaunchKernelGGL((dense_reduce_kernel<T>), rgrid, dim3(256), 0, st, (const T *)slabs, n_nt, S, bm, Tn, d->R, den,
                       out_dev, ldo, (int *)nullptr, gate, (int *)nullptr, slab_first);
    WAGG_HIP(hipGetLastError());
    return WAGG_OK;
}

template <typename T>
int entry::dense_apply(wagg_dense *d, const T *X_dev, int64_t Tn, int64_t ldx, T *out_dev, int64_t ldo, int ksplit, void *stream,
                       bool exact) {
    return wagg::dense_apply<T>(d, X_dev, Tn, ldx, PackXfT<T>{}, out_dev, ldo, ksplit, stream, exact);
}

template <typename T>
int entry::dense_apply_poly(wagg_dense *d, const T *X_dev, int64_t Tn, int64_t ldx, double offset, int power, T *out_dev,
                            int64_t ldo, int ksplit, void *stream, bool exact) {
    WAGG_REQUIRE(power >= 1 && power <= 16, "power must lie in [1, 16], got %d", power);
    PackXfT<T> xf;
    xf.mode = power; xf.off = (T)offset;
    return wagg::dense_apply<T>(d, X_dev, Tn, ldx, xf, out_dev, ldo, ksplit, stream, exact);
}

template <typename T>
int entry::dense_apply_edd(wagg_dense *d, const T *tasmin, const T *tasmax, int64_t Tn, int64_t ldx, double offset,
                           double threshold, T *out_dev, int64_t ldo, int ksplit, void *stream, bool exact) {
    PackXfT<T> xf;
    xf.mode = XF_EDD; xf.off = (T)offset; xf.thr = (T)threshold; xf.X2 = tasmax;
    return wagg::dense_apply<T>(d, tasmin, Tn, ldx, xf, out_dev, ldo, ksplit, stream, exact);
}

}

extern "C" int wagg_dense_create_synth(int64_t G, int32_t R, uint32_t seed, wagg_dense **out) {
    return wagg::create_synth<float>(G, R, seed, 1.0, out);
}
extern "C" int wagg_dense_create_synth_sparse(int64_t G, int32_t R, uint32_t seed, double fill, wagg_dense **out) {
    return wagg::create_synth<float>(G, R, seed, fill, out);
}
extern "C" int wagg_dense_create_synth_f64(int64_t G, int32_t R, uint32_t seed, double fill, wagg_dense **out) {
    return wagg::create_synth<double>(G, R, seed, fill, out);
}
extern "C" int wagg_dense_create_synth_blocklocal(int64_t G, int32_t R, uint32_t seed, double fill, wagg_dense **out) {
    return wagg::create_synth_blocklocal<float>(G, R, seed, fill, out);
}
extern "C" int wagg_dense_create_synth_blocklocal_f64(int64_t G, int32_t R, uint32_t seed, double fill, wagg_dense **out) {
    return wagg::create_synth_blocklocal<double>(G, R, seed, fill, out);
}
extern "C" int wagg_dense_create_host(const float *W_host, int64_t G, int32_t R, wagg_dense **out) {
    return wagg::create_host<float>(W_host, G, R, out);
}
extern "C" int wagg_dense_create_host_f64(const double *W_host, int64_t G, int32_t R, wagg_dense **out) {
    return wagg::create_host<double>(W_host, G, R, out);
}
extern "C" int wagg_dense_create_from_segments(const int32_t *cell_idx, const int32_t *region_code,
                                               const double *w_eff, int64_t nseg, int64_t G, int32_t R,
                                               int flags, wagg_dense **out) {
    return wagg::create_from_table<float>(cell_idx, nullptr, region_code, w_eff, nseg, G, R, flags, out);
}
extern "C" int wagg_dense_create_from_segments_f64(const int32_t *cell_idx, const int32_t *region_code,
                                                   const double *w_eff, int64_t nseg, int64_t G, int32_t R,
                                                   int flags, wagg_dense **out) {
    return wagg::create_from_table<double>(cell_idx, nullptr, region_code, w_eff, nseg, G, R, flags, out);
}

extern "C" int wagg_dense_create_from_csr(const int64_t *rowptr, const int32_t *col, const double *val, int64_t G, int32_t R,
                                          int flags, wagg_dense **out) {
    using namespace wagg;
    WAGG_REQUIRE(rowptr != nullptr, "rowptr is NULL");
    return create_from_table<float>(nullptr, rowptr, col, val, 0, G, R, flags, out);
}
extern "C" int wagg_dense_create_from_csr_f64(const int64_t *rowptr, const int32_t *col, const double *val, int64_t G, int32_t R,
                                              int flags, wagg_dense **out) {
    using namespace wagg;
    WAGG_REQUIRE(rowptr != nullptr, "rowptr is NULL");
    return create_from_table<double>(nullptr, rowptr, col, val, 0, G, R, flags, out);
}

extern "C" int wagg_dense_get_info_sized(const wagg_dense *d, void *info_buf, uint64_t size) {
    using namespace wagg;
    WAGG_REQUIRE(d && info_buf, "NULL argument");
    wagg_dense_info st;
    std::memset(&st, 0, sizeof(st));
    wagg_dense_info *info = &st;
    info->G = d->G; info->R = d->R; info->n_kt = d->n_kt; info->n_nt = d->n_nt;
    info->n_tiles = d->n_tiles; info->tiled = d->tiled ? 1 : 0;
    info->w_bytes = d->spmm ? (int64_t)d->sp.n_groups * 4 * (d->f64 ? wagg::SpT<double>::GW : wagg::SpT<float>::GW) : d->w_slots() * 16;
    info->form = d->spmm ? WAGG_FORM_ENTRIES : (d->tiled ? WAGG_FORM_TILES : WAGG_FORM_FULL);
    info->elem_bytes = d->f64 ? 8 : 4;
    info->nnz = d->spmm ? d->sp.nnz : d->nnz_table;
    info->build_s = d->build.total_s;
    info->build_upload_s = d->build.upload_s;
    for (int k = 0; k < 3; ++k) info->est_row_s[k] = d->est_row_s[k];
    info->walked_entries = d->walked_entries;
    info->one_pass_sort = d->one_pass_sort ? 1 : 0;
    info->reserved0 = 0;
    copy_sized(info_buf, size, &st, sizeof(st));
    return WAGG_OK;
}
extern "C" int wagg_dense_get_info(const wagg_dense *d, wagg_dense_info *info) {
    return wagg_dense_get_info_sized(d, info, sizeof(wagg_dense_info));
}

namespace wagg {
template <typename E>
static hipError_t clone_buf(DevBuf<E> &dst, int dst_dev, const DevBuf<E> &src, int src_dev) {
    if (!src.p) return hipSuccess;
    hipError_t e = dst.alloc(src.n);
    if (e == hipSuccess && src.n) e = hipMemcpyPeer(dst.p, dst_dev, src.p, src_dev, src.n * sizeof(E));
    return e;
}
}

extern "C" int wagg_dense_clone(const wagg_dense *src, int device, wagg_dense **out) {
    using namespace wagg;
    clear_error();
    WAGG_REQUIRE(out != nullptr, "out is NULL");
    *out = nullptr;
    WAGG_REQUIRE(src != nullptr, "dense plan is NULL");
    int n_dev = 0, cur = 0;
    WAGG_HIP(hipGetDeviceCount(&n_dev));
    WAGG_REQUIRE(device >= 0 && device < n_dev, "no device %d (%d visible)", device, n_dev);
    WAGG_HIP(hipGetDevice(&cur));
    wagg_dense *d = new (std::nothrow) wagg_dense();
    if (!d) { set_error("host allocation failed"); return WAGG_ENOMEM; }
    hipError_t e = hipSetDevice(device);
    try {
        d->G = src->G; d->R = src->R; d->n_kt = src->n_kt; d->n_nt = src->n_nt; d->f64 = src->f64;
        d->tiled = src->tiled; d->n_tiles = src->n_tiles; d->spmm = src->spmm;
        d->sp.rw = src->sp.rw; d->sp.n_rb = src->sp.n_rb; d->sp.n_chunks = src->sp.n_chunks;
        d->sp.nnz = src->sp.nnz; d->sp.n_groups = src->sp.n_groups;
        d->nnz_table = src->nnz_table; d->walked_entries = src->walked_entries; d->one_pass_sort = src->one_pass_sort;
        for (int k = 0; k < 3; ++k) d->est_row_s[k] = src->est_row_s[k];
        d->den_host = src->den_host;
        d->nt_first = src->nt_first;
        d->device = device;
        const double t0 = wall_s();
        if (e == hipSuccess) e = hipDeviceGetAttribute(&d->ncu, hipDeviceAttributeMultiprocessorCount, device);
        if (e == hipSuccess) e = d->nonfinite.alloc(1);
        if (e == hipSuccess) e = hipHostMalloc((void **)&d->inf_host, 2 * sizeof(int), hipHostMallocMapped);
        if (e == hipSuccess) { d->inf_host[0] = d->inf_host[1] = 0; e = hipHostGetDevicePointer((void **)&d->inf_dev, d->inf_host, 0); }
        if (e == hipSuccess) e = clone_buf(d->W, device, src->W, src->device);
        if (e == hipSuccess) e = clone_buf(d->den32, device, src->den32, src->device);
        if (e == hipSuccess) e = clone_buf(d->den64, device, src->den64, src->device);
        if (e == hipSuccess) e = clone_buf(d->wmax, device, src->wmax, src->device);
        if (e == hipSuccess) e = clone_buf(d->tile_kt, device, src->tile_kt, src->device);
        if (e == hipSuccess) e = clone_buf(d->sp.ent, device, src->sp.ent, src->device);
        if (e == hipSuccess) e = clone_buf(d->sp.grp_off, device, src->sp.grp_off, src->device);
        if (e == hipSuccess) e = hipStreamSynchronize(nullptr);
        d->build.total_s = d->build.device_s = wall_s() - t0;
    } catch (const std::bad_alloc &) {
        (void)hipSetDevice(cur);
        delete d;
        set_error("host allocation failed");
        return WAGG_ENOMEM;
    }
    const hipError_t back = hipSetDevice(cur);
    if (e != hipSuccess || back != hipSuccess) {
        set_error("clone of a dense plan onto device %d: %s", device, hipGetErrorString(e != hipSuccess ? e : back));
        delete d;
        return e == hipErrorOutOfMemory ? WAGG_ENOMEM : WAGG_EHIP;
    }
    *out = d;
    return WAGG_OK;
}

extern "C" int wagg_dense_destroy(wagg_dense *d) {
    delete d;
    return WAGG_OK;
}

extern "C" int wagg_dense_get_den(const wagg_dense *d, double *den_host) {
    using namespace wagg;
    WAGG_REQUIRE(d && den_host, "NULL argument");
    std::memcpy(den_host, d->den_host.data(), sizeof(double) * (size_t)d->R);
    return WAGG_OK;
}

namespace wagg {
static int check_dense_device(const wagg_dense *d) {
    int cur = 0;
    WAGG_HIP(hipGetDevice(&cur));
    WAGG_REQUIRE(cur == d->device, "the dense plan was created on device %d, the current device is %d", d->device, cur);
    return WAGG_OK;
}

template <typename T>
int entry::dense_apply_host(wagg_dense *d, const T *X_host, int64_t Tn, int64_t ldx, T *out_host, int64_t ldo, int flags, bool exact) {
    clear_error();
    WAGG_REQUIRE(d != nullptr, "dense plan is NULL");
    WAGG_REQUIRE(Tn >= 0, "T < 0");
    if (Tn == 0) return WAGG_OK;
    WAGG_REQUIRE(X_host && out_host, "X/out is NULL");
    WAGG_REQUIRE(ldx >= d->G && ldo >= d->R, "ldx/ldo too small");
    WAGG_REQUIRE((flags & ~(WAGG_HOST_PIN | WAGG_HOST_WHOLE)) == 0, "unknown host flags 0x%x", flags);
    if (int rc = check_dense_device(d)) return rc;
    if (flags & WAGG_HOST_WHOLE) {
        ScratchBuf<T> dx, dout;
        WAGG_HIP(dx.alloc((size_t)(Tn * ldx)));
        WAGG_HIP(dout.alloc((size_t)(Tn * ldo)));
        const bool pin = (flags & WAGG_HOST_PIN) != 0;
        if (int rc = copy_to_device(dx.p, X_host, sizeof(T) * (size_t)((Tn - 1) * ldx + d->G), pin)) return rc;
        const int rc = entry::dense_apply<T>(d, dx.p, Tn, ldx, dout.p, ldo, 0, nullptr, exact);
        if (rc != WAGG_OK) return rc;
        WAGG_HIP(hipDeviceSynchronize());
        return copy_rows_to_host(out_host, dout.p, Tn, sizeof(T) * (size_t)ldo, sizeof(T) * (size_t)d->R, pin);
    }
    return stream_host_rows<T>(X_host, Tn, ldx, d->G, out_host, ldo, d->R, flags, d->spmm ? SpT<T>::TB : DT<T>::MT_MAX * 16, 1, nullptr,
                               [&](int, const T *xd, int64_t rows, T *od, hipStream_t st) {
                                   return entry::dense_apply<T>(d, xd, rows, ldx, od, ldo, 0, (void *)st, exact);
                               },
                               [](int, hipStream_t) {});
}

template <typename T>
int entry::dense_apply_host_multi(wagg_dense *const *plans, const int *devices, int n, const T *X_host, int64_t Tn, int64_t ldx,
                                  T *out_host, int64_t ldo, int flags) {
    clear_error();
    WAGG_REQUIRE(plans && devices && n >= 1 && n <= 64, "need 1..64 plan replicas and their devices");
    WAGG_REQUIRE((flags & ~WAGG_HOST_PIN) == 0, "unknown host flags 0x%x", flags);
    WAGG_REQUIRE(Tn >= 0, "T < 0");
    for (int s = 0; s < n; ++s) {
        WAGG_REQUIRE(plans[s] != nullptr, "plan replica %d is NULL", s);
        WAGG_REQUIRE(plans[s]->device == devices[s], "plan replica %d lives on device %d, not %d", s, plans[s]->device, devices[s]);
        WAGG_REQUIRE(plans[s]->G == plans[0]->G && plans[s]->R == plans[0]->R && plans[s]->f64 == (sizeof(T) == 8) &&
                     plans[s]->spmm == plans[0]->spmm, "plan replica %d has another shape, element type or form", s);
        for (int q = 0; q < s; ++q) WAGG_REQUIRE(plans[q] != plans[s], "replicas %d and %d are the same plan (a dense-family plan owns "
                                                 "its workspaces: one replica per pipeline)", q, s);
    }
    if (Tn == 0) return WAGG_OK;
    WAGG_REQUIRE(X_host && out_host, "X/out is NULL");
    wagg_dense *d0 = plans[0];
    WAGG_REQUIRE(ldx >= d0->G && ldo >= d0->R, "ldx/ldo too small");
    const int rc = stream_host_rows<T>(X_host, Tn, ldx, d0->G, out_host, ldo, d0->R, flags, d0->spmm ? SpT<T>::TB : DT<T>::MT_MAX * 16, n, devices,
                                       [&](int s, const T *xd, int64_t rows, T *od, hipStream_t st) {
                                           return entry::dense_apply<T>(plans[s], xd, rows, ldx, od, ldo, 0, (void *)st);
                                       },
                                       [](int, hipStream_t) {});
    for (int s = 1; s < n; ++s) {
        volatile int *note = plans[s]->inf_host;
        if (note[0]) { *(volatile int *)d0->inf_host = 1; note[0] = 0; }
    }
    return rc;
}
}

extern "C" int wagg_dense_saw_inf(wagg_dense *d, void *stream, int *saw) {
    using namespace wagg;
    WAGG_REQUIRE(d && saw, "NULL argument");
    WAGG_HIP(hipStreamSynchronize((hipStream_t)stream));
    *saw = *(volatile int *)d->inf_host;
    *(volatile int *)d->inf_host = 0;
    return WAGG_OK;
}

namespace wagg {
#define WAGG_ENTRY_DENSE(T)                                                                                                              \
    template int entry::dense_apply<T>(wagg_dense *, const T *, int64_t, int64_t, T *, int64_t, int, void *, bool);                      \
    template int entry::dense_apply_poly<T>(wagg_dense *, const T *, int64_t, int64_t, double, int, T *, int64_t, int, void *, bool);    \
    template int entry::dense_apply_edd<T>(wagg_dense *, const T *, const T *, int64_t, int64_t, double, double, T *, int64_t, int,      \
                                           void *, bool);                                                                                \
    template int entry::dense_apply_host<T>(wagg_dense *, const T *, int64_t, int64_t, T *, int64_t, int, bool);                         \
    template int entry::dense_apply_host_multi<T>(wagg_dense *const *, const int *, int, const T *, int64_t, int64_t, T *, int64_t, int);
WAGG_ENTRY_DENSE(float)
WAGG_ENTRY_DENSE(double)
#undef WAGG_ENTRY_DENSE
}
```

climate_toolbox_amd/csrc/wagg_dense_int.h:

```cpp
#pragma once
#include <memory>

#include "wagg_build.h"
#include "wagg_host.h"

namespace wagg {

template <typename T> struct PackXfT {
    int mode = 0;
    T off = T(0), thr = T(0);
    const T *X2 = nullptr;
};
typedef PackXfT<float> PackXf;

template <typename T>
__device__ __forceinline__ T pack_xf(const PackXfT<T> &xf, T x, T x2, bool &inf_seen) {
    T y = x;
    if (xf.mode > 0) y = xform1<T>(x, xf.off, xf.mode);
    else if (xf.mode == XF_EDD) y = snyder_edd1<T>(x + xf.off, x2 + xf.off, xf.thr);
    inf_seen |= __builtin_isinf(y);
    return y == y ? y : T(0);
}

constexpr int SP_WAVES = 16;
constexpr int SP_THREADS = SP_WAVES * 64;
constexpr int SP_ROW = 512;
constexpr int SP_KC = 128;
constexpr int SP_ACC = 88;
constexpr int SP_RW_MAX = SP_ACC / 2 - 1;
constexpr int SP_TRASH = 2 * SP_RW_MAX;
constexpr int SP_GROUP = 8;
constexpr int SP_PAD_GROUPS = 48;
template <typename T> struct SpT {
    static constexpr int TB = SP_ROW / (int)sizeof(T);
    static constexpr int GW = 4 + 8 * (int)(sizeof(T) / 4);
    static constexpr int WSLOT = 128 * (int)sizeof(T);
};
__host__ __device__ inline unsigned sp_entry_lo(int cell_in_chunk, int j) { return (unsigned)(cell_in_chunk << 9 | 2 * j); }
template <typename T> __host__ __device__ inline int64_t sp_lo16_index(int64_t pos) {
    return (pos >> 3) * (2 * SpT<T>::GW) + (pos & 7);
}
template <typename T> __host__ __device__ inline int64_t sp_w_index(int64_t pos) {
    return (pos >> 3) * SpT<T>::GW + 4 + (pos & 7) * (int)(sizeof(T) / 4);
}

struct SpmmPlan {
    int rw = 0;
    int n_rb = 0;
    int n_chunks = 0;
    int64_t nnz = 0, n_groups = 0;
    DevBuf<uint32_t> ent;
    DevBuf<int32_t> grp_off;
};

}

struct wagg_dense {
    int64_t G = 0;
    int32_t R = 0;
    int n_kt = 0, n_nt = 0;
    bool f64 = false;
    wagg::DevBuf<float> W, den32, slabs, xp;
    wagg::DevBuf<double> den64;
    wagg::DevBuf<float> wmax, xmax;
    std::vector<double> den_host;
    bool tiled = false;
    int64_t n_tiles = 0;
    wagg::DevBuf<int32_t> tile_kt;
    std::vector<int32_t> nt_first;
    struct TilePieces {
        int n_mb = 0, n_wg = 0, n_slabs = 0;
        wagg::DevBuf<int32_t> tab;
        int64_t slab_first_at = 0;
    };
    std::vector<std::unique_ptr<TilePieces>> pieces;
    int64_t w_slots() const { return n_tiles * (8192 / 4); }
    bool spmm = false;
    wagg::SpmmPlan sp;
    int ncu = 256;
    int device = 0;
    int *inf_host = nullptr, *inf_dev = nullptr;
    wagg::DevBuf<int> nonfinite;
    int64_t nnz_table = -1;
    wagg::BuildTimes build;
    double est_row_s[3] = {0, 0, 0};
    int64_t walked_entries = 0;
    bool one_pass_sort = false;
    ~wagg_dense() { if (inf_host) wagg::note_cleanup(hipHostFree(inf_host), "hipHostFree(inf note)"); }
};

namespace wagg {
template <typename T> int spmm_build_synth(wagg_dense *d, uint32_t seed, double fill);
void spmm_geometry(int64_t G, int32_t R, SpmmPlan &sp);
template <typename T> int spmm_build_from_sorted(BuildCtx &ctx, wagg_dense *d, const SortedEntries &se);
int spmm_list_cost(BuildCtx &ctx, const SortedEntries &se, int64_t *walked_entries);
template <typename T> int spmm_apply(wagg_dense *d, const T *X, int64_t Tn, int64_t ldx, const PackXfT<T> &xf, T *out,
                                     int64_t ldo, hipStream_t stream);
int dense_alloc_common(wagg_dense *d);
}
```

climate_toolbox_amd/csrc/wagg_dense_split.inc:

```
typedef _Float16 f16x8 __attribute__((ext_vector_type(8)));

__host__ __device__ __forceinline__ int split_exp(float m) {
    int e = 0;
    if (!(m > 0.0f)) return 0;
    (void)frexpf(m, &e);
    return 15 - e;
}

typedef _Float16 f16x2 __attribute__((ext_vector_type(2)));
typedef unsigned u32x4 __attribute__((ext_vector_type(4)));
__device__ __forceinline__ void split_w8(f32x4 a, f32x4 b, int e, f16x8 &hi, f16x8 &lo) {
    u32x4 H, L;
#pragma unroll
    for (int p = 0; p < 4; ++p) {
        const float v0 = __builtin_amdgcn_ldexpf(p < 2 ? a[2 * p] : b[2 * p - 4], e);
        const float v1 = __builtin_amdgcn_ldexpf(p < 2 ? a[2 * p + 1] : b[2 * p - 3], e);
        const unsigned h = __builtin_bit_cast(unsigned, f16x2{(_Float16)v0, (_Float16)v1});
        unsigned l;
        asm("v_fma_mixlo_f16 %0, %1, -1.0, %2 op_sel_hi:[1,0,0]\n\t"
            "v_fma_mixhi_f16 %0, %1, -1.0, %3 op_sel:[1,0,0] op_sel_hi:[1,0,0]\n\t"
            "s_nop 1"
            : "=&v"(l) : "v"(h), "v"(v0), "v"(v1));
        H[p] = h;
        L[p] = l;
    }
    hi = __builtin_bit_cast(f16x8, H);
    lo = __builtin_bit_cast(f16x8, L);
}


__device__ __forceinline__ __amdgpu_buffer_rsrc_t split_tile_rsrc(const char *base, int bytes) {
    const uint64_t a = reinterpret_cast<uint64_t>(base);
    const uint64_t u = (uint64_t)(uint32_t)__builtin_amdgcn_readfirstlane((unsigned)a) |
                       (uint64_t)(uint32_t)__builtin_amdgcn_readfirstlane((unsigned)(a >> 32)) << 32;
    return __builtin_amdgcn_make_buffer_rsrc(reinterpret_cast<void *>(u), (short)0, bytes, 0x00020000);
}

template <int MT, int DBG = 0>
__global__ __launch_bounds__(D_THREADS, 2) void dense_split_kernel(
    const f16x8 *__restrict__ Xp, const float *__restrict__ Wp, const float *__restrict__ wmax, int n_kt, int n_nt, int n_mb,
    int S, int kt_per_slice, float *__restrict__ slabs) {
    static_assert(MT <= D_MT, "accumulators of MT row blocks must fit the register file");
    extern __shared__ __attribute__((aligned(16))) char lds[];
    constexpr int XT4 = d_xt_bytes(MT);
    constexpr int XPIECES = XT4 / 1024;
    constexpr int NXP = (XPIECES + 7) / 8;
    static_assert(NXP <= 6, "at most six X pieces per wave");
    constexpr int VM_KEEP = 4 + NXP;
    constexpr int WAIT_TILE = (VM_KEEP & 15) | (7 << 4) | (0 << 8) | ((VM_KEEP >> 4) << 14);

    const int tid = threadIdx.x;
    const int lane = tid & 63;
    const int wave = __builtin_amdgcn_readfirstlane(tid >> 6);
    const int lr = lane & 15, kq = lane >> 4;

    int j = (int)(blockIdx.x >> 3);
    const int nt = j % n_nt; j /= n_nt;
    const int mb = j % n_mb;
    const int ks = (int)(blockIdx.x & 7) + 8 * (j / n_mb);
    const int kt0 = ks * kt_per_slice;
    const int kt1 = kt0 + kt_per_slice < n_kt ? kt0 + kt_per_slice : n_kt;
    const int ntiles = kt1 > kt0 ? kt1 - kt0 : 0;
    const int64_t w_first = (int64_t)nt * n_kt + kt0;
    const int ew0 = split_exp(wmax[nt * D_BN + wave * 32 + lr]);
    const int ew1 = split_exp(wmax[nt * D_BN + wave * 32 + 16 + lr]);

    const int f = lr >> 1;
    const unsigned frag0 = (lr * 8 + (kq ^ f)) * 16;
    const unsigned frag1 = (lr * 8 + ((kq ^ f) ^ 4)) * 16;
    const char *xslice = reinterpret_cast<const char *>(Xp) + ((int64_t)mb * n_kt + kt0) * XT4;
    const char *wslice = reinterpret_cast<const char *>(Wp) + w_first * D_WTB;
    const unsigned lane16 = lane * 16;
    const unsigned wfrag0 = wave * 4096 + frag0, wfrag1 = wave * 4096 + frag1;
#define WAGG_RSRC(base, bytes) split_tile_rsrc(base, bytes)
#define WAGG_DMA_X(i, xr, buf)                                                                    \
    do {                                                                                          \
        constexpr int i_ = (i);                                                                   \
        const int q_ = (wave + 8 * i_) % XPIECES;                                                 \
        __builtin_amdgcn_raw_ptr_buffer_load_lds(xr, (lptr_t)(lds + (buf) * XT4 + q_ * 1024), 16, lane16, q_ * 1024, 0, 0); \
    } while (0)
#define WAGG_DMA_XALL(tile, buf)                                                                  \
    do {                                                                                          \
        const auto xr_ = WAGG_RSRC(xslice + (int64_t)(tile) * XT4, XT4);                          \
        WAGG_DMA_X(0, xr_, buf);                                                                  \
        if constexpr (NXP > 1) WAGG_DMA_X(NXP > 1 ? 1 : 0, xr_, buf);                             \
        if constexpr (NXP > 2) WAGG_DMA_X(NXP > 2 ? 2 : 0, xr_, buf);                             \
        if constexpr (NXP > 3) WAGG_DMA_X(NXP > 3 ? 3 : 0, xr_, buf);                             \
        if constexpr (NXP > 4) WAGG_DMA_X(NXP > 4 ? 4 : 0, xr_, buf);                             \
        if constexpr (NXP > 5) WAGG_DMA_X(NXP > 5 ? 5 : 0, xr_, buf);                             \
    } while (0)
#define WAGG_LOAD_W(tile)                                                                         \
    do {                                                                                          \
        const auto wr_ = WAGG_RSRC(wslice + (int64_t)(tile) * D_WTB, D_WTB);                      \
        b00 = __builtin_bit_cast(f32x4, __builtin_amdgcn_raw_buffer_load_b128(wr_, wfrag0, 0, 0));        \
        b01 = __builtin_bit_cast(f32x4, __builtin_amdgcn_raw_buffer_load_b128(wr_, wfrag1, 0, 0));        \
        b10 = __builtin_bit_cast(f32x4, __builtin_amdgcn_raw_buffer_load_b128(wr_, wfrag0 + 2048, 0, 0)); \
        b11 = __builtin_bit_cast(f32x4, __builtin_amdgcn_raw_buffer_load_b128(wr_, wfrag1 + 2048, 0, 0)); \
    } while (0)

    f32x4 acc[MT][2];
#pragma unroll
    for (int m = 0; m < MT; ++m) acc[m][0] = acc[m][1] = f32x4{0, 0, 0, 0};

    f32x4 b00, b01, b10, b11;
    if (ntiles > 0) {
        const int t1 = ntiles > 1 ? 1 : 0;
        WAGG_LOAD_W(0);
        WAGG_DMA_XALL(0, 0);
        WAGG_DMA_XALL(t1, 1);
        asm volatile("s_waitcnt vmcnt(0)" ::: "memory");
        __builtin_amdgcn_s_barrier();
    }

#define WAGG_SPLIT(A, B, E, HI, LO)                                                               \
    do {                                                                                          \
        if constexpr (DBG & 8) { HI = __builtin_bit_cast(f16x8, A); LO = __builtin_bit_cast(f16x8, B); } \
        else split_w8(A, B, E, HI, LO);                                                           \
    } while (0)
#define WAGG_MFMA16(RB, CB, A, B) acc[RB][CB] = __builtin_amdgcn_mfma_f32_16x16x32_f16(A, B, acc[RB][CB], 0, 0, 0)
#define WAGG_READ_A(H, L, RB)                                                                     \
    do {                                                                                          \
        H = *reinterpret_cast<const f16x8 *>(img + frag0 + (RB) * 2048);                          \
        L = *reinterpret_cast<const f16x8 *>(img + frag1 + (RB) * 2048);                          \
    } while (0)
    constexpr auto xdma_block = [](int i) { return MT <= 2 ? MT - 1 : 2 + i * (MT - 2) / NXP; };
#define WAGG_DMA_AT(RB, i)                                                                        \
    do {                                                                                          \
        if constexpr (!(DBG & 1) && (i) < NXP && xdma_block(i) == (RB)) WAGG_DMA_X((i) < NXP ? (i) : 0, xfar, bfar); \
    } while (0)
#define WAGG_DMA_BLOCK(RB)                                                                        \
    do {                                                                                          \
        WAGG_DMA_AT(RB, 0); WAGG_DMA_AT(RB, 1); WAGG_DMA_AT(RB, 2);                               \
        WAGG_DMA_AT(RB, 3); WAGG_DMA_AT(RB, 4); WAGG_DMA_AT(RB, 5);                               \
    } while (0)
#define WAGG_BLOCK_(RB, H, L, NH, NL)                                                             \
    do {                                                                                          \
        __builtin_amdgcn_sched_barrier(0);                                                        \
        WAGG_MFMA16(RB, 0, H, wl0);                                                               \
        __builtin_amdgcn_sched_barrier(0);                                                        \
        if constexpr ((RB) + 1 < MT) WAGG_READ_A(NH, NL, (RB) + 1 < MT ? (RB) + 1 : 0);           \
        __builtin_amdgcn_sched_barrier(0);                                                        \
        WAGG_MFMA16(RB, 1, H, wl1);                                                               \
        WAGG_MFMA16(RB, 0, L, wh0);                                                               \
        WAGG_MFMA16(RB, 1, L, wh1);                                                               \
        WAGG_MFMA16(RB, 0, H, wh0);                                                               \
        WAGG_MFMA16(RB, 1, H, wh1);                                                               \
        __builtin_amdgcn_sched_barrier(0);                                                        \
        WAGG_DMA_BLOCK(RB);                                                                       \
    } while (0)
#define WAGG_BLOCK(RB)                                                                            \
    do {                                                                                          \
        if constexpr ((RB) < MT) {                                                                \
            constexpr int rb_ = (RB) < MT ? (RB) : 0;                                             \
            if constexpr ((RB) & 1) WAGG_BLOCK_(rb_, aBh, aBl, aAh, aAl);                         \
            else WAGG_BLOCK_(rb_, aAh, aAl, aBh, aBl);                                            \
        }                                                                                         \
    } while (0)

    int bcur = 0;
    for (int tile = 0; tile < ntiles; ++tile) {
        const char *img = lds + bcur * XT4;
        const int bfar = bcur == 0 ? 2 : bcur - 1;
        const int tnext = tile + 1 < ntiles ? tile + 1 : ntiles - 1;
        const int tfar = tile + 2 < ntiles ? tile + 2 : ntiles - 1;
        const auto xfar = WAGG_RSRC(xslice + (int64_t)tfar * XT4, XT4);
        f16x8 wh0, wl0, wh1, wl1, aAh, aAl, aBh, aBl;
        WAGG_READ_A(aAh, aAl, 0);
        WAGG_SPLIT(b00, b01, ew0, wh0, wl0);
        if constexpr (MT > 1) WAGG_READ_A(aBh, aBl, MT > 1 ? 1 : 0);
        __builtin_amdgcn_sched_barrier(0);
        WAGG_MFMA16(0, 0, aAh, wl0);
        WAGG_MFMA16(0, 0, aAl, wh0);
        WAGG_MFMA16(0, 0, aAh, wh0);
        if constexpr (MT > 1) {
            WAGG_MFMA16(MT > 1 ? 1 : 0, 0, aBh, wl0);
            WAGG_MFMA16(MT > 1 ? 1 : 0, 0, aBl, wh0);
            WAGG_MFMA16(MT > 1 ? 1 : 0, 0, aBh, wh0);
        }
        WAGG_SPLIT(b10, b11, ew1, wh1, wl1);
        __builtin_amdgcn_sched_barrier(0);
        if constexpr (!(DBG & 1)) WAGG_LOAD_W(tnext);
        __builtin_amdgcn_sched_barrier(0);
        WAGG_MFMA16(0, 1, aAh, wl1);
        WAGG_MFMA16(0, 1, aAl, wh1);
        WAGG_MFMA16(0, 1, aAh, wh1);
        __builtin_amdgcn_sched_barrier(0);
        if constexpr (MT > 2) WAGG_READ_A(aAh, aAl, MT > 2 ? 2 : 0);
        __builtin_amdgcn_sched_barrier(0);
        if constexpr (MT > 1) {
            WAGG_MFMA16(MT > 1 ? 1 : 0, 1, aBh, wl1);
            WAGG_MFMA16(MT > 1 ? 1 : 0, 1, aBl, wh1);
            WAGG_MFMA16(MT > 1 ? 1 : 0, 1, aBh, wh1);
        }
        __builtin_amdgcn_sched_barrier(0);
        WAGG_DMA_BLOCK(0); WAGG_DMA_BLOCK(1);
        WAGG_BLOCK(2); WAGG_BLOCK(3); WAGG_BLOCK(4); WAGG_BLOCK(5);
        WAGG_BLOCK(6); WAGG_BLOCK(7); WAGG_BLOCK(8); WAGG_BLOCK(9); WAGG_BLOCK(10); WAGG_BLOCK(11);
        WAGG_BLOCK(12); WAGG_BLOCK(13); WAGG_BLOCK(14); WAGG_BLOCK(15); WAGG_BLOCK(16); WAGG_BLOCK(17);
        WAGG_BLOCK(18); WAGG_BLOCK(19); WAGG_BLOCK(20); WAGG_BLOCK(21); WAGG_BLOCK(22);
        static_assert(MT <= 23, "row blocks are written out up to 22");
        __builtin_amdgcn_sched_barrier(0);
        if constexpr (!(DBG & 4)) {
            __builtin_amdgcn_s_waitcnt(WAIT_TILE);
            __builtin_amdgcn_s_barrier();
        }
        bcur = bcur == 2 ? 0 : bcur + 1;
    }
    asm volatile("s_waitcnt vmcnt(0)" ::: "memory");

    float *slab = slabs + ((((int64_t)mb * n_nt + nt) * S + ks) * (MT * 16)) * D_BN;
#pragma unroll
    for (int m = 0; m < MT; ++m)
#pragma unroll
        for (int cb = 0; cb < 2; ++cb)
#pragma unroll
            for (int r = 0; r < 4; ++r)
                slab[(m * 16 + kq * 4 + r) * D_BN + wave * 32 + cb * 16 + lr] = acc[m][cb][r];
#undef WAGG_RSRC
#undef WAGG_DMA_X
#undef WAGG_DMA_XALL
#undef WAGG_LOAD_W
#undef WAGG_DMA_AT
#undef WAGG_DMA_BLOCK
#undef WAGG_SPLIT
#undef WAGG_MFMA16
#undef WAGG_READ_A
#undef WAGG_BLOCK_
#undef WAGG_BLOCK
}

__global__ void dense_rowmax_kernel(const float *__restrict__ X, int64_t ldx, int64_t G, PackXfT<float> xf,
                                    unsigned *__restrict__ rowmax) {
    const int64_t t = blockIdx.y;
    const float *src = X + t * ldx;
    const float *src2 = xf.mode == XF_EDD ? xf.X2 + t * ldx : src;
    bool inf_seen = false;
    float m = 0.0f;
    for (int64_t g = (int64_t)blockIdx.x * blockDim.x + threadIdx.x; g < G; g += (int64_t)gridDim.x * blockDim.x) {
        const float y = pack_xf<float>(xf, src[g], src2[g], inf_seen);
        const float a = fabsf(y);
        m = a <= FLT_MAX && a > m ? a : m;
    }
#pragma unroll
    for (int o = 32; o >= 1; o >>= 1) m = fmaxf(m, __shfl_xor(m, o, 64));
    __shared__ float wm[16];
    if ((threadIdx.x & 63) == 0) wm[threadIdx.x >> 6] = m;
    __syncthreads();
    if (threadIdx.x == 0) {
        for (int w = 1; w < (int)(blockDim.x >> 6); ++w) m = fmaxf(m, wm[w]);
        if (m > 0.0f) atomicMax(rowmax + t, __float_as_uint(m));
    }
}

__global__ void dense_pack_x_split_kernel(const float *__restrict__ X, int64_t Tn, int64_t ldx, int64_t G, int n_kt, int bm,
                                          int64_t n_slots, int aligned, const unsigned *__restrict__ rowmax,
                                          f16x8 *__restrict__ Xp, PackXfT<float> xf, int *__restrict__ inf_flag) {
    const int64_t stride = (int64_t)gridDim.x * blockDim.x;
    const int tile_slots = bm * 8;
    bool inf_seen = false;
    for (int64_t s = (int64_t)blockIdx.x * blockDim.x + threadIdx.x; s < n_slots; s += stride) {
        const int slot = (int)(s % tile_slots);
        const int64_t tk = s / tile_slots;
        const int kt = (int)(tk % n_kt);
        const int64_t mb = tk / n_kt;
        const int row = slot >> 3, p = (slot & 7) ^ ((row >> 1) & 7);
        const bool low = p >= 4;
        const int64_t t = mb * bm + row, k0 = (int64_t)kt * 32 + 4 * (p & 3);
        f16x8 o;
#pragma unroll
        for (int c = 0; c < 8; ++c) o[c] = (_Float16)0.0f;
        if (t < Tn) {
            const int ex = split_exp(__uint_as_float(rowmax[t]));
            const float *src = X + t * ldx;
            const float *src2 = xf.mode == XF_EDD ? xf.X2 + t * ldx : src;
            float v[8], h[8];
#pragma unroll
            for (int c = 0; c < 8; ++c) { v[c] = 0.0f; h[c] = 0.0f; }
#pragma unroll
            for (int half = 0; half < 2; ++half) {
                const int64_t kk = k0 + 16 * half;
                if (aligned && kk + 4 <= G) {
                    const f32x4 a = *reinterpret_cast<const f32x4 *>(src + kk);
                    const f32x4 b = xf.mode == XF_EDD ? *reinterpret_cast<const f32x4 *>(src2 + kk) : a;
#pragma unroll
                    for (int c = 0; c < 4; ++c) { v[4 * half + c] = a[c]; h[4 * half + c] = b[c]; }
                } else {
#pragma unroll
                    for (int c = 0; c < 4; ++c) if (kk + c < G) { v[4 * half + c] = src[kk + c]; h[4 * half + c] = src2[kk + c]; }
                }
            }
#pragma unroll
            for (int c = 0; c < 8; ++c) {
                const int64_t k = k0 + 16 * (c >> 2) + (c & 3);
                if (k >= G) continue;
                const float y = __builtin_amdgcn_ldexpf(pack_xf<float>(xf, v[c], h[c], inf_seen), ex);
                const _Float16 hi = (_Float16)y;
                o[c] = low ? (__builtin_isinf(y) ? (_Float16)0.0f : (_Float16)(y - (float)hi)) : hi;
            }
        }
        Xp[s] = o;
    }
    if (inf_seen) __hip_atomic_store(inf_flag, 1, __ATOMIC_RELAXED, __HIP_MEMORY_SCOPE_SYSTEM);
}

__global__ void dense_reduce_split_kernel(const float *__restrict__ slabs, int n_nt, int S, int bm, int32_t R,
                                          const float *__restrict__ den, const unsigned *__restrict__ rowmax,
                                          const float *__restrict__ wmax, float *__restrict__ out, int64_t ldo) {
    const int64_t r = (int64_t)blockIdx.x * blockDim.x + threadIdx.x;
    const int64_t t = blockIdx.y;
    if (r >= R) return;
    const int mb = (int)(t / bm), tl = (int)(t % bm);
    const int nt = (int)(r / D_BN), c = (int)(r % D_BN);
    const float *p = slabs + ((((int64_t)mb * n_nt + nt) * S) * bm + tl) * D_BN + c;
    float s = 0.0f;
    for (int k = 0; k < S; ++k) s += p[(int64_t)k * bm * D_BN];
    const int e = split_exp(__uint_as_float(rowmax[t])) + split_exp(wmax[r]);
    out[t * ldo + r] = __builtin_amdgcn_ldexpf(s, -e) / den[r];
}

__global__ void dense_colmax_kernel(const f32x4 *__restrict__ Wp, int n_kt, int kt_per_block, unsigned *__restrict__ wmax) {
    const int nt = blockIdx.x;
    const int ktb = blockIdx.y * kt_per_block;
    const int kte = ktb + kt_per_block < n_kt ? ktb + kt_per_block : n_kt;
    for (int slot = threadIdx.x; slot < D_WSLOTS; slot += blockDim.x) {
        float m = 0.0f;
        for (int kt = ktb; kt < kte; ++kt) {
            const f32x4 v = Wp[((int64_t)nt * n_kt + kt) * D_WSLOTS + slot];
#pragma unroll
            for (int c = 0; c < 4; ++c) { const float a = fabsf(v[c]); m = a <= FLT_MAX && a > m ? a : m; }
        }
        m = fmaxf(m, __shfl_xor(m, 1, 64));
        m = fmaxf(m, __shfl_xor(m, 2, 64));
        m = fmaxf(m, __shfl_xor(m, 4, 64));
        if ((slot & 7) == 0 && m > 0.0f) atomicMax(wmax + nt * D_BN + (slot >> 3), __float_as_uint(m));
    }
}
```

climate_toolbox_amd/csrc/wagg_desc.hip:

```cpp
#include <cstddef>
#include <cstring>
#include <type_traits>

#include "wagg_common.h"
#include "wagg_dense_int.h"
#include "wagg_entry.h"
#include "wagg_host.h"
#include "wagg_sparse_int.h"

namespace wagg {
namespace {

const char *src_name(int s) {
    switch (s) {
        case WAGG_SRC_DEVICE: return "device";
        case WAGG_SRC_HOST: return "host";
        case WAGG_SRC_HOST_MULTI: return "host-multi";
        case WAGG_SRC_SHARDED: return "sharded";
        default: return "?";
    }
}
const char *xf_name(int x) { return x == WAGG_XF_NONE ? "none" : x == WAGG_XF_POLY ? "poly" : x == WAGG_XF_EDD ? "edd" : "?"; }

int unsupported(const wagg_apply_desc &d, const char *why) {
// ... 165 lines not shown
    WAGG_REQUIRE(d.plan_kind == WAGG_PLAN_SEGMENT || d.plan_kind == WAGG_PLAN_DENSE, "wagg_apply: unknown plan_kind %d", d.plan_kind);
    WAGG_REQUIRE(d.elem == WAGG_T_F32 || d.elem == WAGG_T_F64, "wagg_apply: elem must be WAGG_T_F32 or WAGG_T_F64, got %d", d.elem);
    WAGG_REQUIRE(d.source >= WAGG_SRC_DEVICE && d.source <= WAGG_SRC_SHARDED, "wagg_apply: unknown source %d", d.source);
    WAGG_REQUIRE(d.transform >= WAGG_XF_NONE && d.transform <= WAGG_XF_EDD, "wagg_apply: unknown transform %d", d.transform);
    WAGG_REQUIRE(d.plan != nullptr, "wagg_apply: plan is NULL");
    if (d.source == WAGG_SRC_HOST_MULTI) WAGG_REQUIRE(d.n_plans >= 1, "wagg_apply: the multi-device host form needs n_plans >= 1 plan handles in `plan`");
    if (d.source == WAGG_SRC_SHARDED) WAGG_REQUIRE(d.group != nullptr, "wagg_apply: the sharded form needs a wagg_shard_group");
    if (d.plan_kind == WAGG_PLAN_SEGMENT) return d.elem == WAGG_T_F32 ? run_segment<float>(d) : run_segment<double>(d);
    return d.elem == WAGG_T_F32 ? run_dense<float>(d) : run_dense<double>(d);
}

#define SEG WAGG_PLAN_SEGMENT
#define DEN WAGG_PLAN_DENSE
using wagg::edd; using wagg::lay; using wagg::on_device; using wagg::on_host; using wagg::on_host_multi; using wagg::on_shards; using wagg::poly;
using wagg::run;

extern "C" int wagg_apply_f32(const wagg_plan *plan, const float *X_dev, int64_t T, int64_t ldx, int layout, float *out_dev, int64_t ldo,
                              int out_layout, void *stream) {
    return run(lay(on_device(SEG, plan, X_dev, T, ldx, out_dev, ldo, stream), layout, out_layout));
}
extern "C" int wagg_apply_f64(const wagg_plan *plan, const double *X_dev, int64_t T, int64_t ldx, int layout, double *out_dev, int64_t ldo,
                              int out_layout, void *stream) {
    return run(lay(on_device(SEG, plan, X_dev, T, ldx, out_dev, ldo, stream), layout, out_layout));
}
extern "C" int wagg_apply_host_ex_f32(const wagg_plan *plan, const float *X_host, int64_t T, int64_t ldx, int layout, float *out_host,
                                      int64_t ldo, int out_layout, int flags) {
    return run(lay(on_host(SEG, plan, X_host, T, ldx, out_host, ldo, flags), layout, out_layout));
}
extern "C" int wagg_apply_host_ex_f64(const wagg_plan *plan, const double *X_host, int64_t T, int64_t ldx, int layout, double *out_host,
                                      int64_t ldo, int out_layout, int flags) {
    return run(lay(on_host(SEG, plan, X_host, T, ldx, out_host, ldo, flags), layout, out_layout));
}
extern "C" int wagg_apply_host_f32(const wagg_plan *plan, const float *X_host, int64_t T, int64_t ldx, int layout, float *out_host,
                                   int64_t ldo, int out_layout) {
    return wagg_apply_host_ex_f32(plan, X_host, T, ldx, layout, out_host, ldo, out_layout, WAGG_HOST_PIN | WAGG_HOST_LINES);
}
extern "C" int wagg_apply_host_f64(const wagg_plan *plan, const double *X_host, int64_t T, int64_t ldx, int layout, double *out_host,
                                   int64_t ldo, int out_layout) {
    return wagg_apply_host_ex_f64(plan, X_host, T, ldx, layout, out_host, ldo, out_layout, WAGG_HOST_PIN | WAGG_HOST_LINES);
}
extern "C" int wagg_apply_host_multi_f32(const wagg_plan *const *plans, const int *devices, int n_devices, const float *X_host, int64_t T,
                                         int64_t ldx, float *out_host, int64_t ldo, int flags) {
    return run(on_host_multi(SEG, plans, devices, n_devices, X_host, T, ldx, out_host, ldo, flags));
}
extern "C" int wagg_apply_host_multi_f64(const wagg_plan *const *plans, const int *devices, int n_devices, const double *X_host, int64_t T,
                                         int64_t ldx, double *out_host, int64_t ldo, int flags) {
    return run(on_host_multi(SEG, plans, devices, n_devices, X_host, T, ldx, out_host, ldo, flags));
}
extern "C" int wagg_apply_poly_f32(const wagg_plan *plan, const float *X_dev, int64_t T, int64_t ldx, int layout, double offset, int pow_first,
                                   int n_pow, float *out_dev, int64_t ldo, int64_t out_pstride, int out_layout, void *stream) {
    return run(lay(poly(on_device(SEG, plan, X_dev, T, ldx, out_dev, ldo, stream), offset, pow_first, n_pow, out_pstride), layout, out_layout));
}
extern "C" int wagg_apply_poly_f64(const wagg_plan *plan, const double *X_dev, int64_t T, int64_t ldx, int layout, double offset, int pow_first,
                                   int n_pow, double *out_dev, int64_t ldo, int64_t out_pstride, int out_layout, void *stream) {
    return run(lay(poly(on_device(SEG, plan, X_dev, T, ldx, out_dev, ldo, stream), offset, pow_first, n_pow, out_pstride), layout, out_layout));
}
extern "C" int wagg_apply_poly_host_f32(const wagg_plan *plan, const float *X_host, int64_t T, int64_t ldx, double offset, int pow_first, int n_pow,
                                        float *out_host, int64_t ldo, int64_t out_pstride, int flags) {
    return run(poly(on_host(SEG, plan, X_host, T, ldx, out_host, ldo, flags), offset, pow_first, n_pow, out_pstride));
}
extern "C" int wagg_apply_poly_host_f64(const wagg_plan *plan, const double *X_host, int64_t T, int64_t ldx, double offset, int pow_first, int n_pow,
                                        double *out_host, int64_t ldo, int64_t out_pstride, int flags) {
    return run(poly(on_host(SEG, plan, X_host, T, ldx, out_host, ldo, flags), offset, pow_first, n_pow, out_pstride));
}
extern "C" int wagg_apply_edd_f32(const wagg_plan *plan, const float *tasmin_dev, const float *tasmax_dev, int64_t T, int64_t ldx, int layout,
                                  double offset, const double *thresholds, int n_thr, float *out_dev, int64_t ldo, int64_t out_pstride,
                                  int out_layout, void *stream) {
    return run(lay(edd(on_device(SEG, plan, tasmin_dev, T, ldx, out_dev, ldo, stream), tasmax_dev, offset, thresholds, n_thr, out_pstride), layout, out_layout));
}
extern "C" int wagg_apply_edd_f64(const wagg_plan *plan, const double *tasmin_dev, const double *tasmax_dev, int64_t T, int64_t ldx, int layout,
                                  double offset, const double *thresholds, int n_thr, double *out_dev, int64_t ldo, int64_t out_pstride,
                                  int out_layout, void *stream) {
    return run(lay(edd(on_device(SEG, plan, tasmin_dev, T, ldx, out_dev, ldo, stream), tasmax_dev, offset, thresholds, n_thr, out_pstride), layout, out_layout));
}
extern "C" int wagg_apply_edd_host_f32(const wagg_plan *plan, const float *tasmin_host, const float *tasmax_host, int64_t T, int64_t ldx, double offset,
                                       const double *thresholds, int n_thr, float *out_host, int64_t ldo, int64_t out_pstride, int flags) {
    return run(edd(on_host(SEG, plan, tasmin_host, T, ldx, out_host, ldo, flags), tasmax_host, offset, thresholds, n_thr, out_pstride));
}
extern "C" int wagg_apply_edd_host_f64(const wagg_plan *plan, const double *tasmin_host, const double *tasmax_host, int64_t T, int64_t ldx, double offset,
                                       const double *thresholds, int n_thr, double *out_host, int64_t ldo, int64_t out_pstride, int flags) {
    return run(edd(on_host(SEG, plan, tasmin_host, T, ldx, out_host, ldo, flags), tasmax_host, offset, thresholds, n_thr, out_pstride));
}
extern "C" int wagg_apply_sharded_f32(wagg_shard_group *g, const wagg_plan *const *plans, const float *const *X_dev, const int64_t *rows, int64_t ldx,
                                      float *out_root, int64_t ldo, int root) {
    return run(on_shards(SEG, g, plans, X_dev, rows, ldx, out_root, ldo, root));
}
extern "C" int wagg_apply_sharded_f64(wagg_shard_group *g, const wagg_plan *const *plans, const double *const *X_dev, const int64_t *rows, int64_t ldx,
                                      double *out_root, int64_t ldo, int root) {
    return run(on_shards(SEG, g, plans, X_dev, rows, ldx, out_root, ldo, root));
}

extern "C" int wagg_dense_apply_f32(wagg_dense *p, const float *X_dev, int64_t T, int64_t ldx, float *out_dev, int64_t ldo, int ksplit, void *stream) {
    return run(on_device(DEN, p, X_dev, T, ldx, out_dev, ldo, stream, ksplit));
}
extern "C" int wagg_dense_apply_f64(wagg_dense *p, const double *X_dev, int64_t T, int64_t ldx, double *out_dev, int64_t ldo, int ksplit, void *stream) {
    return run(on_device(DEN, p, X_dev, T, ldx, out_dev, ldo, stream, ksplit));
}
extern "C" int wagg_dense_apply_poly_f32(wagg_dense *p, const float *X_dev, int64_t T, int64_t ldx, double offset, int power, float *out_dev, int64_t ldo,
                                         int ksplit, void *stream) {
    return run(poly(on_device(DEN, p, X_dev, T, ldx, out_dev, ldo, stream, ksplit), offset, power, 1, 0));
}
extern "C" int wagg_dense_apply_poly_f64(wagg_dense *p, const double *X_dev, int64_t T, int64_t ldx, double offset, int power, double *out_dev, int64_t ldo,
                                         int ksplit, void *stream) {
    return run(poly(on_device(DEN, p, X_dev, T, ldx, out_dev, ldo, stream, ksplit), offset, power, 1, 0));
}
extern "C" int wagg_dense_apply_edd_f32(wagg_dense *p, const float *tasmin_dev, const float *tasmax_dev, int64_t T, int64_t ldx, double offset,
                                        double threshold, float *out_dev, int64_t ldo, int ksplit, void *stream) {
    return run(edd(on_device(DEN, p, tasmin_dev, T, ldx, out_dev, ldo, stream, ksplit), tasmax_dev, offset, &threshold, 1, 0));
}
extern "C" int wagg_dense_apply_edd_f64(wagg_dense *p, const double *tasmin_dev, const double *tasmax_dev, int64_t T, int64_t ldx, double offset,
                                        double threshold, double *out_dev, int64_t ldo, int ksplit, void *stream) {
    return run(edd(on_device(DEN, p, tasmin_dev, T, ldx, out_dev, ldo, stream, ksplit), tasmax_dev, offset, &threshold, 1, 0));
}
extern "C" int wagg_dense_apply_host_f32(wagg_dense *p, const float *X_host, int64_t T, int64_t ldx, float *out_host, int64_t ldo, int flags) {
    return run(on_host(DEN, p, X_host, T, ldx, out_host, ldo, flags));
}
extern "C" int wagg_dense_apply_host_f64(wagg_dense *p, const double *X_host, int64_t T, int64_t ldx, double *out_host, int64_t ldo, int flags) {
    return run(on_host(DEN, p, X_host, T, ldx, out_host, ldo, flags));
}
extern "C" int wagg_dense_apply_host_multi_f32(wagg_dense *const *plans, const int *devices, int n_devices, const float *X_host, int64_t T, int64_t ldx,
                                               float *out_host, int64_t ldo, int flags) {
    return run(on_host_multi(DEN, plans, devices, n_devices, X_host, T, ldx, out_host, ldo, flags));
}
extern "C" int wagg_dense_apply_host_multi_f64(wagg_dense *const *plans, const int *devices, int n_devices, const double *X_host, int64_t T, int64_t ldx,
                                               double *out_host, int64_t ldo, int flags) {
    return run(on_host_multi(DEN, plans, devices, n_devices, X_host, T, ldx, out_host, ldo, flags));
}
extern "C" int wagg_dense_apply_sharded_f32(wagg_shard_group *g, wagg_dense *const *plans, const float *const *X_dev, const int64_t *rows, int64_t ldx,
                                            float *out_root, int64_t ldo, int root) {
    return run(on_shards(DEN, g, plans, X_dev, rows, ldx, out_root, ldo, root));
}
extern "C" int wagg_dense_apply_sharded_f64(wagg_shard_group *g, wagg_dense *const *plans, const double *const *X_dev, const int64_t *rows, int64_t ldx,
                                            double *out_root, int64_t ldo, int root) {
    return run(on_shards(DEN, g, plans, X_dev, rows, ldx, out_root, ldo, root));
}
#undef SEG
#undef DEN

namespace wagg {
namespace {
template <typename F> void put(int &k, F &f) {
    ++k;
    if constexpr (std::is_pointer_v<F>) f = reinterpret_cast<F>(static_cast<uintptr_t>(k));
    else f = static_cast<F>(k);
}
template <typename F, size_t N> void put(int &k, F (&f)[N]) { for (F &e : f) put(k, e); }
template <typename... F> void number(F &...f) { int k = 0; (put(k, f), ...); }

void ordinals(wagg_plan_info &s) {
    auto &[a1, a2, a3, a4, a5, a6, a7, a8, a9, a10, a11, a12, a13, a14, a15, a16, a17, a18, a19] = s;
    number(a1, a2, a3, a4, a5, a6, a7, a8, a9, a10, a11, a12, a13, a14, a15, a16, a17, a18, a19);
}
void ordinals(wagg_dense_info &s) {
    auto &[a1, a2, a3, a4, a5, a6, a7, a8, a9, a10, a11, a12, a13, a14, a15, a16] = s;
    number(a1, a2, a3, a4, a5, a6, a7, a8, a9, a10, a11, a12, a13, a14, a15, a16);
}
void ordinals(wagg_host_stats &s) {
    auto &[a1, a2, a3, a4, a5, a6, a7, a8, a9, a10, a11, a12, a13, a14, a15, a16, a17, a18] = s;
    number(a1, a2, a3, a4, a5, a6, a7, a8, a9, a10, a11, a12, a13, a14, a15, a16, a17, a18);
}
void ordinals(wagg_apply_desc &s) {
    auto &[a1, a2, a3, a4, a5, a6, a7, a8, a9, a10, a11, a12, a13, a14, a15, a16, a17, a18, a19, a20, a21, a22, a23, a24, a25, a26, a27, a28, a29] = s;
    number(a1, a2, a3, a4, a5, a6, a7, a8, a9, a10, a11, a12, a13, a14, a15, a16, a17, a18, a19, a20, a21, a22, a23, a24, a25, a26, a27, a28, a29);
}
template <typename S> int fill_ordinals(void *out, uint64_t size) {
    S s;
    std::memset(&s, 0, sizeof(s));
    ordinals(s);
    copy_sized(out, size, &s, sizeof(s));
    return WAGG_OK;
}
}

void copy_sized(void *dst, uint64_t dst_size, const void *src, size_t src_size) {
    const size_t n = dst_size < src_size ? (size_t)dst_size : src_size;
    std::memcpy(dst, src, n);
    if (dst_size > src_size) std::memset(static_cast<char *>(dst) + src_size, 0, (size_t)(dst_size - src_size));
}
}

extern "C" int wagg_struct_size(int which) {
    switch (which) {
        case WAGG_STRUCT_PLAN_INFO: return (int)sizeof(wagg_plan_info);
        case WAGG_STRUCT_DENSE_INFO: return (int)sizeof(wagg_dense_info);
        case WAGG_STRUCT_HOST_STATS: return (int)sizeof(wagg_host_stats);
        case WAGG_STRUCT_APPLY_DESC: return (int)sizeof(wagg_apply_desc);
        default: wagg::set_error("wagg_struct_size: unknown struct id %d", which); return WAGG_EINVAL;
    }
}

extern "C" int wagg_struct_ordinals(int which, void *out, uint64_t size) {
    using namespace wagg;
    WAGG_REQUIRE(out != nullptr && size <= ((uint64_t)1 << 20), "wagg_struct_ordinals: NULL buffer or absurd size");
    switch (which) {
        case WAGG_STRUCT_PLAN_INFO: return fill_ordinals<wagg_plan_info>(out, size);
        case WAGG_STRUCT_DENSE_INFO: return fill_ordinals<wagg_dense_info>(out, size);
        case WAGG_STRUCT_HOST_STATS: return fill_ordinals<wagg_host_stats>(out, size);
        case WAGG_STRUCT_APPLY_DESC: return fill_ordinals<wagg_apply_desc>(out, size);
        default: set_error("wagg_struct_ordinals: unknown struct id %d", which); return WAGG_EINVAL;
    }
}
```

climate_toolbox_amd/engine.py:

```python
from __future__ import annotations

import ctypes as C
import threading

import numpy as np

from . import _lib
from ._lib import LAYOUT_GT, LAYOUT_TG, OUT_RT, OUT_TR, WaggError

_LAYOUTS = {"TG": LAYOUT_TG, "GT": LAYOUT_GT}
_OUTS = {"TR": OUT_TR, "RT": OUT_RT}


def require_gpu():
    L = _lib.load()
    if L.wagg_device_count() < 1:
        raise WaggError("no HIP device visible: the aggregation engine has no CPU fallback")
    import torch
    if not torch.cuda.is_available():
        raise WaggError("torch sees no GPU (needed for device buffers and streams)")
    return torch


class _on_device:
# ... 289 lines not shown
                _lib.check(L.wagg_plan_get_den_many(self._h, i, lv, _np_ptr(d, C.c_double)), "wagg_plan_get_den_many")
                row.append(d)
            self.den.append(row)

    def close(self):
        if getattr(self, "_h", None) is not None and self._h.value and _lib is not None and _lib._lib is not None:
            _lib._lib.wagg_plan_destroy(self._h)
            self._h = C.c_void_p()

    __del__ = close

    def status(self, stream=None):
        _lib.check(_lib.load().wagg_plan_status(self._h, _stream_handle(stream)), "wagg_plan_status")

    def split(self, full, out_layout="TR"):
        if out_layout == "TR":
            return [[full[:, o:o + Rl] for o in offs] for offs, Rl in zip(self.offsets, self.level_R)]
        return [[full[o:o + Rl] for o in offs] for offs, Rl in zip(self.offsets, self.level_R)]

    def apply(self, X, layout="TG", out_layout="TR", out=None, stream=None):
        import torch
        X = _check_X(X, layout)
        T = X.shape[0] if layout == "TG" else X.shape[1]
        if (X.shape[1] if layout == "TG" else X.shape[0]) != self.G:
            raise ValueError("X has the wrong number of grid cells (plan expects %d)" % self.G)
        shape = (T, self.out_cols) if out_layout == "TR" else (self.out_cols, T)
        if out is None:
            out = torch.empty(shape, dtype=X.dtype, device=X.device)
        elif tuple(out.shape) != shape or out.dtype != X.dtype or (shape[1] > 1 and out.stride(1) != 1):
            raise ValueError("out must be a %s %s tensor with contiguous rows" % (shape, X.dtype))
        _lib.run("wagg_apply (many)", plan_kind=_lib.PLAN_SEGMENT, plan=self._h, elem=_elem(X.dtype), source=_lib.SRC_DEVICE,
                 x=X.data_ptr(), T=T, ldx=_ld(X), layout=_LAYOUTS[layout], out=out.data_ptr(), ldo=_ld(out),
                 out_layout=_OUTS[out_layout], stream=_stream_handle(stream))
        return self.split(out, out_layout)

    def apply_host(self, X, flags=0, out=None, layout="TG", out_layout="TR"):
        X = np.ascontiguousarray(X)
        if X.dtype not in (np.float32, np.float64) or X.ndim != 2:
            raise TypeError("X must be a 2-D float32/float64 array")
        T = X.shape[0] if layout == "TG" else X.shape[1]
        shape = (T, self.out_cols) if out_layout == "TR" else (self.out_cols, T)
        out = _host_out(out, shape, X.dtype)
        with _on_device(self.device):
            _lib.run("wagg_apply (many, host)", plan_kind=_lib.PLAN_SEGMENT, plan=self._h, elem=_elem(X.dtype), source=_lib.SRC_HOST,
                     x=X.ctypes.data, T=T, ldx=X.shape[1], layout=_LAYOUTS[layout], out=out.ctypes.data, ldo=max(1, shape[1]),
                     out_layout=_OUTS[out_layout], flags=int(flags))
        return self.split(out, out_layout)


def _exact_flag(exact):
    return _lib.APPLY_EXACT_F32 if exact else 0


class DensePlan:

    def __init__(self, handle, G, R, device=None, recipe=None):
        self._h, self.G, self.R = handle, int(G), int(R)
        self.device = _current_device() if device is None else int(device)
        self._recipe = recipe
        self._lease = threading.Lock()
        den = np.empty(self.R, dtype=np.float64)
        _lib.check(_lib.load().wagg_dense_get_den(self._h, _np_ptr(den, C.c_double)), "wagg_dense_get_den")
        self.den = den
        inf = _lib.DenseInfo()
        _lib.check(_lib.load().wagg_dense_get_info_sized(self._h, C.byref(inf), C.sizeof(inf)), "wagg_dense_get_info_sized")
        self.info = {k: (float if ct is C.c_double else int)(getattr(inf, k)) for k, ct in _lib.DenseInfo._fields_}
        self.dtype = "float64" if self.info["elem_bytes"] == 8 else "float32"

    @staticmethod
    def _is64(dtype):
        return str(dtype).endswith("float64") or dtype is np.float64

    @classmethod
    def synth_blocklocal(cls, G, R, seed, fill=0.952, dtype="float32", device=None):
        require_gpu()
        h = C.c_void_p()
        L = _lib.load()
        fn = L.wagg_dense_create_synth_blocklocal_f64 if cls._is64(dtype) else L.wagg_dense_create_synth_blocklocal
        with _on_device(device):
            dev = _current_device()
            _lib.check(fn(int(G), int(R), int(seed), float(fill), C.byref(h)), "wagg_dense_create_synth_blocklocal")
        return cls(h, G, R, dev, (cls.synth_blocklocal, (G, R, seed), dict(fill=fill, dtype=dtype)))

    @classmethod
    def synth(cls, G, R, seed, fill=1.0, dtype="float32", device=None):
        require_gpu()
        h = C.c_void_p()
        L = _lib.load()
        fn = L.wagg_dense_create_synth_f64 if cls._is64(dtype) else L.wagg_dense_create_synth_sparse
        with _on_device(device):
            dev = _current_device()
            _lib.check(fn(int(G), int(R), int(seed), float(fill), C.byref(h)), "wagg_dense_create_synth")
        return cls(h, G, R, dev, (cls.synth, (G, R, seed), dict(fill=fill, dtype=dtype)))

    @classmethod
    def from_host(cls, W, device=None):
        require_gpu()
        W = np.asarray(W)
        h = C.c_void_p()
        with _on_device(device):
            dev = _current_device()
            if W.dtype == np.float64:
                W = np.ascontiguousarray(W)
                _lib.check(_lib.load().wagg_dense_create_host_f64(_np_ptr(W, C.c_double), W.shape[0], W.shape[1], C.byref(h)),
                           "wagg_dense_create_host_f64")
            else:
                W = np.ascontiguousarray(W, dtype=np.float32)
                _lib.check(_lib.load().wagg_dense_create_host(_np_ptr(W, C.c_float), W.shape[0], W.shape[1], C.byref(h)),
                           "wagg_dense_create_host")
        return cls(h, W.shape[0], W.shape[1], dev)

    @classmethod
    def from_segments(cls, cell_idx, region_code, w_eff, G, R, dtype="float32", device=None, form=None):
        require_gpu()
        ci = np.ascontiguousarray(cell_idx, dtype=np.int32)
        rc = np.ascontiguousarray(region_code, dtype=np.int32)
        we = np.ascontiguousarray(w_eff, dtype=np.float64)
        h = C.c_void_p()
        L = _lib.load()
        fn = L.wagg_dense_create_from_segments_f64 if cls._is64(dtype) else L.wagg_dense_create_from_segments
        with _on_device(device):
            dev = _current_device()
            _lib.check(fn(_np_ptr(ci, C.c_int32), _np_ptr(rc, C.c_int32), _np_ptr(we, C.c_double), len(ci), int(G),
                          int(R), _lib.FORCE_FORM[form], C.byref(h)), "wagg_dense_create_from_segments")
        return cls(h, G, R, dev)

    @classmethod
    def from_csr(cls, rowptr, col, val, G, R, dtype="float32", device=None, form=None, general_sort=False):
        require_gpu()
        rp = np.ascontiguousarray(rowptr, dtype=np.int64)
        co = np.ascontiguousarray(col, dtype=np.int32)
        va = np.ascontiguousarray(val, dtype=np.float64)
        if rp.shape != (int(G) + 1,) or co.shape != va.shape or co.ndim != 1 or (len(rp) and int(rp[-1]) != len(co)):
            raise ValueError("rowptr must hold G + 1 offsets ending at len(col) == len(val)")
        h = C.c_void_p()
        L = _lib.load()
        fn = L.wagg_dense_create_from_csr_f64 if cls._is64(dtype) else L.wagg_dense_create_from_csr
        with _on_device(device):
            dev = _current_device()
            _lib.check(fn(_np_ptr(rp, C.c_int64), _np_ptr(co, C.c_int32), _np_ptr(va, C.c_double), int(G), int(R),
                          _lib.FORCE_FORM[form] | (_lib.DENSE_GENERAL_SORT if general_sort else 0), C.byref(h)),
                       "wagg_dense_create_from_csr")
        return cls(h, G, R, dev)

    def replica(self, device):
        if self._recipe is not None:
            fn, args, kw = self._recipe
            return fn(*args, device=device, **kw)
        require_gpu()
        h = C.c_void_p()
        _lib.check(_lib.load().wagg_dense_clone(self._h, int(device), C.byref(h)), "wagg_dense_clone")
        return type(self)(h, self.G, self.R, int(device))

    def close(self):
        for r in getattr(self, "_replicas", {}).values():
            r.close()
        if getattr(self, "_h", None) is not None and self._h.value and _lib is not None and _lib._lib is not None:
            _lib._lib.wagg_dense_destroy(self._h)
            self._h = C.c_void_p()

    __del__ = close

    def _prep(self, X, out):
        import torch
        X = _check_X(X, "TG")
        want = torch.float64 if self.dtype == "float64" else torch.float32
        if X.dtype != want:
            raise TypeError("this dense plan serves %s data, got %s" % (self.dtype, X.dtype))
        if X.shape[1] != self.G:
            raise ValueError("X has %d grid cells, plan expects %d" % (X.shape[1], self.G))
        T = X.shape[0]
        if out is None:
            out = torch.empty((T, self.R), dtype=want, device=X.device)
        elif tuple(out.shape) != (T, self.R) or out.dtype != want or (self.R > 1 and out.stride(1) != 1):
            raise ValueError("out must be a (%d, %d) %s tensor with contiguous rows" % (T, self.R, self.dtype))
        return X, T, out

    def _run(self, what, **fields):
        _lib.run(what, plan_kind=_lib.PLAN_DENSE, elem=_elem(self.dtype), **fields)

    def apply(self, X, out=None, ksplit=0, stream=None, exact=False):
        X, T, out = self._prep(X, out)
        self._run("wagg_apply (dense)", plan=self._h, source=_lib.SRC_DEVICE, x=X.data_ptr(), T=T, ldx=_ld(X), out=out.data_ptr(),
                  ldo=_ld(out), ksplit=int(ksplit), stream=_stream_handle(stream), flags=_exact_flag(exact))
        return out

    def apply_poly(self, X, offset, power, out=None, ksplit=0, stream=None, exact=False):
        X, T, out = self._prep(X, out)
        self._run("wagg_apply (dense, poly)", plan=self._h, source=_lib.SRC_DEVICE, transform=_lib.XF_POLY, offset=float(offset),
                  pow_first=int(power), n_pow=1, x=X.data_ptr(), T=T, ldx=_ld(X), out=out.data_ptr(), ldo=_ld(out), ksplit=int(ksplit),
                  stream=_stream_handle(stream), flags=_exact_flag(exact))
        return out

    def apply_edd(self, tasmin, tasmax, threshold, offset=0.0, out=None, ksplit=0, stream=None, exact=False):
        tasmin, T, out = self._prep(tasmin, out)
        tasmax = _check_X(tasmax, "TG")
        if tasmax.shape != tasmin.shape or tasmax.dtype != tasmin.dtype or _ld(tasmax) != _ld(tasmin):
            raise ValueError("tasmin and tasmax must have the same shape, dtype and row stride")
        thr = (C.c_double * 1)(float(threshold))
        self._run("wagg_apply (dense, edd)", plan=self._h, source=_lib.SRC_DEVICE, transform=_lib.XF_EDD, offset=float(offset),
                  thresholds=thr, n_thr=1, x=tasmin.data_ptr(), x2=tasmax.data_ptr(), T=T, ldx=_ld(tasmin), out=out.data_ptr(),
                  ldo=_ld(out), ksplit=int(ksplit), stream=_stream_handle(stream), flags=_exact_flag(exact))
        return out

    def apply_host(self, X, flags=0, replicas=(), out=None, exact=False):
        flags = int(flags) & ~(_lib.HOST_LINES | _lib.HOST_LINES_WHOLE)
        want = np.float64 if self.dtype == "float64" else np.float32
        X = np.ascontiguousarray(X)
        if X.dtype != want or X.ndim != 2 or X.shape[1] != self.G:
            raise TypeError("X must be a (T, %d) %s array" % (self.G, self.dtype))
        out = _host_out(out, (X.shape[0], self.R), want)
        if replicas:
            plans = (self,) + tuple(replicas)
            hs = (C.c_void_p * len(plans))(*[p._h for p in plans])
            devs = (C.c_int32 * len(plans))(*[p.device for p in plans])
            self._run("wagg_apply (dense, host, multi-device)", plan=hs, n_plans=len(plans), devices=devs, source=_lib.SRC_HOST_MULTI,
                      x=X.ctypes.data, T=X.shape[0], ldx=X.shape[1], out=out.ctypes.data, ldo=max(1, self.R), flags=int(flags))
            return out
        with _on_device(self.device):
            self._run("wagg_apply (dense, host)", plan=self._h, source=_lib.SRC_HOST, x=X.ctypes.data, T=X.shape[0], ldx=X.shape[1],
                      out=out.ctypes.data, ldo=max(1, self.R), flags=int(flags) | _exact_flag(exact))
        return out

    def saw_inf(self, stream=None):
        saw = C.c_int(0)
        _lib.check(_lib.load().wagg_dense_saw_inf(self._h, _stream_handle(stream), C.byref(saw)), "wagg_dense_saw_inf")
        return bool(saw.value)


class ShardGroup:

    _TRANSPORTS = {"auto": _lib.GATHER_AUTO, "rccl": _lib.GATHER_RCCL, "peer": _lib.GATHER_PEER}

    def __init__(self, devices, transport="auto"):
        require_gpu()
        self.devices = [int(d) for d in devices]
        arr = (C.c_int32 * len(self.devices))(*self.devices)
        self._h = C.c_void_p()
        _lib.check(_lib.load().wagg_shard_group_create(arr, len(self.devices), self._TRANSPORTS[transport], C.byref(self._h)),
                   "wagg_shard_group_create")
        n, tr = C.c_int(0), C.c_int(0)
        _lib.check(_lib.load().wagg_shard_group_info(self._h, C.byref(n), C.byref(tr)), "wagg_shard_group_info")
        self.transport = {_lib.GATHER_RCCL: "rccl", _lib.GATHER_PEER: "peer"}[tr.value]

    def close(self):
        if getattr(self, "_h", None) is not None and self._h.value and _lib._lib is not None:
            _lib._lib.wagg_shard_group_destroy(self._h)
            self._h = C.c_void_p()

    __del__ = close

    def apply(self, plans, shards, root=0, out=None):
        import torch
        n = len(self.devices)
        if len(plans) != n or len(shards) != n:
            raise ValueError("the group has %d shards: need as many plans and tensors" % n)
        dense = isinstance(plans[0], DensePlan)
        if any(isinstance(p, DensePlan) != dense for p in plans):
            raise TypeError("all plans of a call are of one family")
        dtype = shards[0].dtype
        rows, lds = [], set()
        for i, x in enumerate(shards):
            if not (x.is_cuda and x.dim() == 2 and x.dtype == dtype and x.device.index == self.devices[i] and x.shape[1] == plans[0].G):
                raise ValueError("shard %d must be a (rows, %d) %s tensor on device %d" % (i, plans[0].G, dtype, self.devices[i]))
            if x.shape[0] and x.shape[1] > 1 and x.stride(1) != 1:
                raise ValueError("shard %d: rows must be contiguous" % i)
            if x.shape[0] > 1:
                lds.add(_ld(x))
            rows.append(int(x.shape[0]))
        if len(lds) > 1:
            raise ValueError("the shards must share one row stride, got %r" % sorted(lds))
        ldx = lds.pop() if lds else plans[0].G
        R = plans[0].R
        total = sum(rows)
        if out is None:
            out = torch.empty((total, R), dtype=dtype, device="cuda:%d" % self.devices[root])
        elif tuple(out.shape) != (total, R) or out.dtype != dtype or out.device.index != self.devices[root] or (R > 1 and out.stride(1) != 1):
            raise ValueError("out must be a (%d, %d) %s tensor on device %d" % (total, R, dtype, self.devices[root]))
        hp = (C.c_void_p * n)(*[p._h for p in plans])
        xp = (C.c_void_p * n)(*[C.c_void_p(x.data_ptr()) for x in shards])
        rw = (C.c_int64 * n)(*rows)
        for d in set(self.devices):
            torch.cuda.synchronize(d)
        _lib.run("wagg_apply (sharded)", plan_kind=_lib.PLAN_DENSE if dense else _lib.PLAN_SEGMENT, plan=hp, n_plans=n, elem=_elem(dtype),
                 source=_lib.SRC_SHARDED, group=self._h, x=xp, rows=rw, ldx=ldx, out=out.data_ptr(), ldo=_ld(out), root=int(root))
        return out


def gather(X, cell_idx_dev, layout="TG", out_layout="TR", stream=None):
    import torch
    X = _check_X(X, layout)
    if not (cell_idx_dev.is_cuda and cell_idx_dev.dtype == torch.int32 and cell_idx_dev.is_contiguous()):
        raise TypeError("cell_idx_dev must be a contiguous int32 CUDA tensor")
    T = X.shape[0] if layout == "TG" else X.shape[1]
    n = cell_idx_dev.numel()
    shape = (T, n) if out_layout == "TR" else (n, T)
    out = torch.empty(shape, dtype=X.dtype, device=X.device)
    L = _lib.load()
    fn = L.wagg_gather_f32 if X.dtype == torch.float32 else L.wagg_gather_f64
    _lib.check(fn(C.c_void_p(X.data_ptr()), T, _ld(X), _LAYOUTS[layout],
                  C.c_void_p(cell_idx_dev.data_ptr()), n, C.c_void_p(out.data_ptr()), max(1, shape[1]),
                  _OUTS[out_layout], _stream_handle(stream)), "wagg_gather")
    return out


PACK_STATS = {"device": 0, "host": 0, "host_fallback": 0}
# ... 469 lines not shown
```

include/wagg.h:

```cpp
#ifndef WAGG_H
#define WAGG_H

#include <stdint.h>

#ifdef __cplusplus
extern "C" {
#endif

typedef enum wagg_status {
    WAGG_OK = 0,
    WAGG_EINVAL = -1,
    WAGG_EHIP = -2,
    WAGG_ENOMEM = -3,
    WAGG_ENODEV = -4,
    WAGG_EUNSUPPORTED = -5,
    WAGG_EKEY = -6,
    WAGG_EINTERNAL = -7
} wagg_status;

#define WAGG_LAYOUT_TG 0
#define WAGG_LAYOUT_GT 1
#define WAGG_OUT_TR 0
#define WAGG_OUT_RT 1

// ... 42 lines not shown
int wagg_factorize_bytes(const char *buf, int64_t width, const uint8_t *isnull, int64_t n,
                         int32_t *codes, int64_t *uniq_rows, int64_t *n_uniq);

#define WAGG_PLAN_NO_LC 1
#define WAGG_PLAN_NO_STREAM 2
#define WAGG_PLAN_NO_LINES 4
#define WAGG_PLAN_LC_MFMA 8
#define WAGG_PLAN_SERIAL_BUILD 16
int wagg_plan_create(const int32_t *cell_idx, const int32_t *region_code, const double *w_eff,
                     int64_t nseg, int64_t G, int32_t R, int64_t row_len, int flags,
                     wagg_plan **out);
int wagg_plan_destroy(wagg_plan *plan);
int wagg_plan_get_info(const wagg_plan *plan, wagg_plan_info *info);
int wagg_plan_get_den(const wagg_plan *plan, double *den_host );
int wagg_plan_status(const wagg_plan *plan, void *stream);

int wagg_apply_f32(const wagg_plan *plan, const float *X_dev, int64_t T, int64_t ldx, int layout,
                   float *out_dev, int64_t ldo, int out_layout, void *stream);
int wagg_apply_f64(const wagg_plan *plan, const double *X_dev, int64_t T, int64_t ldx, int layout,
                   double *out_dev, int64_t ldo, int out_layout, void *stream);
#define WAGG_HOST_PIN 1
#define WAGG_HOST_WHOLE 2
#define WAGG_HOST_LINES 4
#define WAGG_HOST_LINES_WHOLE 8
int wagg_apply_host_f32(const wagg_plan *plan, const float *X_host, int64_t T, int64_t ldx,
                        int layout, float *out_host, int64_t ldo, int out_layout);
int wagg_apply_host_f64(const wagg_plan *plan, const double *X_host, int64_t T, int64_t ldx,
                        int layout, double *out_host, int64_t ldo, int out_layout);
int wagg_apply_host_ex_f32(const wagg_plan *plan, const float *X_host, int64_t T, int64_t ldx,
                           int layout, float *out_host, int64_t ldo, int out_layout, int flags);
int wagg_apply_host_ex_f64(const wagg_plan *plan, const double *X_host, int64_t T, int64_t ldx,
                           int layout, double *out_host, int64_t ldo, int out_layout, int flags);
int wagg_apply_host_multi_f32(const wagg_plan *const *plans, const int *devices, int n_devices, const float *X_host,
                              int64_t T, int64_t ldx, float *out_host, int64_t ldo, int flags);
int wagg_apply_host_multi_f64(const wagg_plan *const *plans, const int *devices, int n_devices, const double *X_host,
                              int64_t T, int64_t ldx, double *out_host, int64_t ldo, int flags);
int wagg_host_block_plan(int64_t T, int64_t row_bytes, int64_t quantum, int n_devices, int64_t *block_rows, int64_t *n_blocks);
typedef struct wagg_host_stats {
    int64_t calls, blocks, registered, register_failed, unregistered, unregister_failed, cleanup_failed;
    int64_t staged_h2d_bytes, staged_d2h_bytes, direct_h2d_bytes, direct_d2h_bytes;
    int64_t lines_h2d_bytes;
    int64_t lines_wait_pack_us;
    int64_t lines_wait_copy_us;
    int64_t blocks_retired;
    int64_t found_page_locked;
    int64_t watched_calls;
    int64_t last_rate_permille;
} wagg_host_stats;
int wagg_host_stats_read(wagg_host_stats *out, int reset);

#define WAGG_STRUCT_PLAN_INFO 0
#define WAGG_STRUCT_DENSE_INFO 1
#define WAGG_STRUCT_HOST_STATS 2
#define WAGG_STRUCT_APPLY_DESC 3
int wagg_struct_size(int which);
int wagg_struct_ordinals(int which, void *out, uint64_t size);
int wagg_plan_get_info_sized(const wagg_plan *plan, void *info, uint64_t size);
int wagg_host_stats_read_sized(void *out, uint64_t size, int reset);

int wagg_apply_poly_f32(const wagg_plan *plan, const float *X_dev, int64_t T, int64_t ldx, int layout,
                        double offset, int pow_first, int n_pow, float *out_dev, int64_t ldo,
                        int64_t out_pstride, int out_layout, void *stream);
int wagg_apply_poly_f64(const wagg_plan *plan, const double *X_dev, int64_t T, int64_t ldx, int layout,
                        double offset, int pow_first, int n_pow, double *out_dev, int64_t ldo,
                        int64_t out_pstride, int out_layout, void *stream);
int wagg_apply_poly_host_f32(const wagg_plan *plan, const float *X_host, int64_t T, int64_t ldx, double offset, int pow_first,
                             int n_pow, float *out_host, int64_t ldo, int64_t out_pstride, int flags);
int wagg_apply_poly_host_f64(const wagg_plan *plan, const double *X_host, int64_t T, int64_t ldx, double offset, int pow_first,
                             int n_pow, double *out_host, int64_t ldo, int64_t out_pstride, int flags);

int wagg_apply_edd_f32(const wagg_plan *plan, const float *tasmin_dev, const float *tasmax_dev, int64_t T,
                       int64_t ldx, int layout, double offset, const double *thresholds, int n_thr,
                       float *out_dev, int64_t ldo, int64_t out_pstride, int out_layout, void *stream);
int wagg_apply_edd_f64(const wagg_plan *plan, const double *tasmin_dev, const double *tasmax_dev, int64_t T,
                       int64_t ldx, int layout, double offset, const double *thresholds, int n_thr,
                       double *out_dev, int64_t ldo, int64_t out_pstride, int out_layout, void *stream);
int wagg_apply_edd_host_f32(const wagg_plan *plan, const float *tasmin_host, const float *tasmax_host, int64_t T, int64_t ldx,
                            double offset, const double *thresholds, int n_thr, float *out_host, int64_t ldo,
                            int64_t out_pstride, int flags);
int wagg_apply_edd_host_f64(const wagg_plan *plan, const double *tasmin_host, const double *tasmax_host, int64_t T, int64_t ldx,
                            double offset, const double *thresholds, int n_thr, double *out_host, int64_t ldo,
                            int64_t out_pstride, int flags);

int wagg_transform_poly_f32(const float *X_dev, int64_t n, double offset, int power, float *out_dev, void *stream);
int wagg_transform_poly_f64(const double *X_dev, int64_t n, double offset, int power, double *out_dev, void *stream);
int wagg_transform_edd_f32(const float *tasmin_dev, const float *tasmax_dev, int64_t n, double offset,
                           const double *coefs, const double *thresholds, int n_terms, float *out_dev, void *stream);
int wagg_transform_edd_f64(const double *tasmin_dev, const double *tasmax_dev, int64_t n, double offset,
                           const double *coefs, const double *thresholds, int n_terms, double *out_dev, void *stream);
int wagg_combine_planes_f32(const float *planes_dev, int n_planes, int64_t plane_stride, const double *coefs, int64_t n,
                            float *out_dev, void *stream);
int wagg_combine_planes_f64(const double *planes_dev, int n_planes, int64_t plane_stride, const double *coefs, int64_t n,
                            double *out_dev, void *stream);
int wagg_take_axis(const void *src_dev, int64_t outer, int64_t n_src, int64_t inner_bytes, const int64_t *idx_dev,
                   int64_t n_idx, void *dst_dev, void *stream);
int wagg_relayout_f32(const float *src_dev, int ndim, const int64_t *shape, const int64_t *src_strides, float *dst_dev, void *stream);
int wagg_relayout_f64(const double *src_dev, int ndim, const int64_t *shape, const int64_t *src_strides, double *dst_dev, void *stream);
#define WAGG_T_F16 0
#define WAGG_T_BF16 1
#define WAGG_T_I8 2
#define WAGG_T_U8 3
#define WAGG_T_I16 4
#define WAGG_T_I32 5
#define WAGG_T_I64 6
#define WAGG_T_F32 7
#define WAGG_T_F64 8
int wagg_relayout_to_f64(const void *src_dev, int src_type, int ndim, const int64_t *shape, const int64_t *src_strides,
                         double *dst_dev, void *stream);
int wagg_upload(void *dst_dev, const void *src_host, int64_t bytes);
int wagg_any_less_f32(const float *a_dev, const float *b_dev, int64_t n, int *result, void *stream);
int wagg_any_less_f64(const double *a_dev, const double *b_dev, int64_t n, int *result, void *stream);

int wagg_gather_f32(const float *X_dev, int64_t T, int64_t ldx, int layout,
                    const int32_t *cell_idx_dev, int64_t nseg, float *out_dev, int64_t ldo,
                    int out_layout, void *stream);
int wagg_gather_f64(const double *X_dev, int64_t T, int64_t ldx, int layout,
                    const int32_t *cell_idx_dev, int64_t nseg, double *out_dev, int64_t ldo,
                    int out_layout, void *stream);

int wagg_dense_create_synth(int64_t G, int32_t R, uint32_t seed, wagg_dense **out);
int wagg_dense_create_synth_sparse(int64_t G, int32_t R, uint32_t seed, double fill, wagg_dense **out);
int wagg_dense_create_host(const float *W_host, int64_t G, int32_t R, wagg_dense **out);
#define WAGG_DENSE_FORM_AUTO 0
#define WAGG_DENSE_FORCE_FULL 1
#define WAGG_DENSE_FORCE_TILES 2
#define WAGG_DENSE_FORCE_ENTRIES 3
#define WAGG_DENSE_GENERAL_SORT 16
int wagg_dense_create_from_segments(const int32_t *cell_idx, const int32_t *region_code,
                                    const double *w_eff, int64_t nseg, int64_t G, int32_t R,
                                    int flags, wagg_dense **out);
int wagg_dense_create_from_csr(const int64_t *rowptr, const int32_t *col, const double *val, int64_t G, int32_t R,
                               int flags, wagg_dense **out);
int wagg_dense_create_synth_blocklocal(int64_t G, int32_t R, uint32_t seed, double fill, wagg_dense **out);
#define WAGG_FORM_FULL 0
#define WAGG_FORM_TILES 1
#define WAGG_FORM_ENTRIES 2
int wagg_dense_create_synth_f64(int64_t G, int32_t R, uint32_t seed, double fill, wagg_dense **out);
int wagg_dense_create_host_f64(const double *W_host, int64_t G, int32_t R, wagg_dense **out);
int wagg_dense_create_from_segments_f64(const int32_t *cell_idx, const int32_t *region_code,
                                        const double *w_eff, int64_t nseg, int64_t G, int32_t R,
                                        int flags, wagg_dense **out);
int wagg_dense_create_from_csr_f64(const int64_t *rowptr, const int32_t *col, const double *val, int64_t G, int32_t R,
                                   int flags, wagg_dense **out);
int wagg_dense_create_synth_blocklocal_f64(int64_t G, int32_t R, uint32_t seed, double fill, wagg_dense **out);
typedef struct wagg_dense_info {
    int64_t G, n_tiles, w_bytes;
    int32_t R, n_kt, n_nt, tiled;
    int32_t form, elem_bytes;
    int64_t nnz;
    double build_s, build_upload_s;
    double est_row_s[3];
    int64_t walked_entries;
    int32_t one_pass_sort, reserved0;
} wagg_dense_info;
int wagg_dense_get_info(const wagg_dense *d, wagg_dense_info *info);
int wagg_dense_get_info_sized(const wagg_dense *d, void *info, uint64_t size);
int wagg_release_scratch(void);
int64_t wagg_scratch_bytes(void);
int wagg_dense_clone(const wagg_dense *src, int device, wagg_dense **out);
int wagg_dense_destroy(wagg_dense *d);
int wagg_dense_get_den(const wagg_dense *d, double *den_host );
int wagg_dense_apply_f32(wagg_dense *d, const float *X_dev, int64_t T, int64_t ldx,
                         float *out_dev, int64_t ldo, int ksplit, void *stream);
int wagg_dense_apply_f64(wagg_dense *d, const double *X_dev, int64_t T, int64_t ldx,
                         double *out_dev, int64_t ldo, int ksplit, void *stream);
int wagg_dense_apply_poly_f32(wagg_dense *d, const float *X_dev, int64_t T, int64_t ldx, double offset,
                              int power, float *out_dev, int64_t ldo, int ksplit, void *stream);
int wagg_dense_apply_edd_f32(wagg_dense *d, const float *tasmin_dev, const float *tasmax_dev, int64_t T,
                             int64_t ldx, double offset, double threshold, float *out_dev, int64_t ldo,
                             int ksplit, void *stream);
int wagg_dense_apply_poly_f64(wagg_dense *d, const double *X_dev, int64_t T, int64_t ldx, double offset,
                              int power, double *out_dev, int64_t ldo, int ksplit, void *stream);
int wagg_dense_apply_edd_f64(wagg_dense *d, const double *tasmin_dev, const double *tasmax_dev, int64_t T,
                             int64_t ldx, double offset, double threshold, double *out_dev, int64_t ldo,
                             int ksplit, void *stream);
int wagg_dense_apply_host_f32(wagg_dense *d, const float *X_host, int64_t T, int64_t ldx,
                              float *out_host, int64_t ldo, int flags);
int wagg_dense_apply_host_f64(wagg_dense *d, const double *X_host, int64_t T, int64_t ldx,
                              double *out_host, int64_t ldo, int flags);
int wagg_dense_apply_host_multi_f32(wagg_dense *const *plans, const int *devices, int n_devices, const float *X_host,
                                    int64_t T, int64_t ldx, float *out_host, int64_t ldo, int flags);
int wagg_dense_apply_host_multi_f64(wagg_dense *const *plans, const int *devices, int n_devices, const double *X_host,
                                    int64_t T, int64_t ldx, double *out_host, int64_t ldo, int flags);
int wagg_dense_saw_inf(wagg_dense *d, void *stream, int *saw);

int wagg_synth_table_csr(int64_t G, int32_t R, uint32_t seed, double fill, int blocklocal, int64_t *rowptr_host,
                         int32_t *col_host, double *val_host, int64_t capacity, int64_t *nnz_out);
int wagg_synth_field_f32(float *X_dev, int64_t T, int64_t G, int64_t ldx, uint32_t seed,
                         float base, float amp, void *stream);
int wagg_synth_field_f64(double *X_dev, int64_t T, int64_t G, int64_t ldx, uint32_t seed,
                         double base, double amp, void *stream);

typedef struct wagg_shard_group wagg_shard_group;
#define WAGG_GATHER_AUTO 0
#define WAGG_GATHER_RCCL 1
#define WAGG_GATHER_PEER 2
int wagg_shard_group_create(const int *devices, int n, int transport, wagg_shard_group **out);
int wagg_shard_group_destroy(wagg_shard_group *g);
int wagg_shard_group_info(const wagg_shard_group *g, int *n_shards, int *transport );
int wagg_apply_sharded_f32(wagg_shard_group *g, const wagg_plan *const *plans, const float *const *X_dev, const int64_t *rows,
                           int64_t ldx, float *out_root, int64_t ldo, int root);
int wagg_apply_sharded_f64(wagg_shard_group *g, const wagg_plan *const *plans, const double *const *X_dev, const int64_t *rows,
                           int64_t ldx, double *out_root, int64_t ldo, int root);
int wagg_dense_apply_sharded_f32(wagg_shard_group *g, wagg_dense *const *plans, const float *const *X_dev, const int64_t *rows,
                                 int64_t ldx, float *out_root, int64_t ldo, int root);
int wagg_dense_apply_sharded_f64(wagg_shard_group *g, wagg_dense *const *plans, const double *const *X_dev, const int64_t *rows,
                                 int64_t ldx, double *out_root, int64_t ldo, int root);

#define WAGG_PLAN_SEGMENT 0
#define WAGG_PLAN_DENSE 1
#define WAGG_SRC_DEVICE 0
#define WAGG_SRC_HOST 1
#define WAGG_SRC_HOST_MULTI 2
#define WAGG_SRC_SHARDED 3
#define WAGG_XF_NONE 0
#define WAGG_XF_POLY 1
#define WAGG_XF_EDD 2
#define WAGG_APPLY_EXACT_F32 0x10000
#define WAGG_APPLY_COMPACT_ROWS 0x20000
typedef struct wagg_apply_desc {
    uint64_t struct_size;
    int32_t plan_kind, elem, source, transform;
    const void *plan;
    const void *x, *x2;
    void *out;
    int64_t T, ldx, ldo, out_pstride;
    int32_t layout, out_layout;
    double offset;
    int32_t pow_first, n_pow;
    const double *thresholds;
    int32_t n_thr, flags;
    int32_t ksplit, n_plans;
    const int32_t *devices;
    const int64_t *rows;
    void *group;
    int32_t root, reserved0;
    void *stream;
} wagg_apply_desc;
int wagg_apply(const wagg_apply_desc *desc);

int wagg_plan_create_many(const int32_t *cell_idx, const int32_t *region_code, const double *const *w_eff, int n_weights,
                          int64_t nseg, int64_t G, int32_t R, int64_t row_len, const int32_t *const *level_code,
                          const int32_t *level_R, int n_levels, int flags, wagg_plan **out);
int wagg_plan_many_info(const wagg_plan *plan, int *n_weights, int *n_levels, int32_t *level_R, int64_t *out_cols);
int wagg_plan_get_den_many(const wagg_plan *plan, int weighting, int level, double *den_host );

#define WAGG_PERIOD_KEEP_NAN 1
#define WAGG_PERIOD_ROWS_CHECKED 2
int wagg_period_reduce_f32(const float *X_dev, const float *X2_dev, int64_t T, int64_t n, int64_t ldx,
                           const int32_t *row_begin_dev, const int32_t *rows_dev, int32_t P, int64_t n_rows, int transform,
                           double offset, int pow_first, int n_pow, const double *thresholds, int n_thr, int flags,
                           float *out_dev, int64_t ldo, int64_t out_pstride, int32_t *status_dev, void *work_dev,
                           int64_t work_bytes, void *stream);
int wagg_period_reduce_f64(const double *X_dev, const double *X2_dev, int64_t T, int64_t n, int64_t ldx,
                           const int32_t *row_begin_dev, const int32_t *rows_dev, int32_t P, int64_t n_rows, int transform,
                           double offset, int pow_first, int n_pow, const double *thresholds, int n_thr, int flags,
                           double *out_dev, int64_t ldo, int64_t out_pstride, int32_t *status_dev, void *work_dev,
                           int64_t work_bytes, void *stream);
int64_t wagg_period_reduce_work_bytes(int64_t n, int32_t P, int64_t n_rows, int planes);

#define WAGG_SEASON_INVERT (1 << 20)
#define WAGG_SEASON_NULL (1 << 21)
int wagg_season_reduce_f32(const float *X_dev, const float *X2_dev, int64_t T, int64_t n, int64_t ldx,
                           const int32_t *row_begin_dev, const int32_t *rows_dev, int32_t P, int64_t n_rows,
                           const int32_t *doy_dev, const int32_t *win_dev, int transform, double offset, int pow_first, int n_pow,
                           const double *thresholds, int n_thr, int flags, float *out_dev, int64_t ldo, int64_t out_pstride,
                           int32_t *status_dev, void *work_dev, int64_t work_bytes, void *stream);
int wagg_season_reduce_f64(const double *X_dev, const double *X2_dev, int64_t T, int64_t n, int64_t ldx,
                           const int32_t *row_begin_dev, const int32_t *rows_dev, int32_t P, int64_t n_rows,
                           const int32_t *doy_dev, const int32_t *win_dev, int transform, double offset, int pow_first, int n_pow,
                           const double *thresholds, int n_thr, int flags, double *out_dev, int64_t ldo, int64_t out_pstride,
                           int32_t *status_dev, void *work_dev, int64_t work_bytes, void *stream);
int64_t wagg_season_reduce_work_bytes(int64_t n, int32_t P, int64_t n_rows, int planes);
int wagg_season_mask(const int32_t *doy_dev, int64_t T, const int32_t *win_dev, int64_t n, double *out_dev , void *stream);

#define WAGG_EDD_LADDER_MAX 64
#define WAGG_EDD_LADDER_GROUP 8
int wagg_edd_ladder_reduce_f32(const float *tasmin_dev, const float *tasmax_dev, int64_t T, int64_t n, int64_t ldx,
                               const int32_t *row_begin_dev, const int32_t *rows_dev, int32_t P, int64_t n_rows,
                               const int32_t *doy_dev, const int32_t *win_dev, double offset, const double *thresholds, int n_thr,
                               int flags, float *out_dev, int64_t ldo, int64_t out_pstride, int32_t *status_dev, void *work_dev,
                               int64_t work_bytes, void *stream);
int wagg_edd_ladder_reduce_f64(const double *tasmin_dev, const double *tasmax_dev, int64_t T, int64_t n, int64_t ldx,
                               const int32_t *row_begin_dev, const int32_t *rows_dev, int32_t P, int64_t n_rows,
                               const int32_t *doy_dev, const int32_t *win_dev, double offset, const double *thresholds, int n_thr,
                               int flags, double *out_dev, int64_t ldo, int64_t out_pstride, int32_t *status_dev, void *work_dev,
                               int64_t work_bytes, void *stream);
int64_t wagg_edd_ladder_work_bytes(int64_t n, int32_t P, int64_t n_rows, int n_thr);

#define WAGG_BIN_EDGES_MAX 65
#define WAGG_BIN_GROUP 8
int wagg_bin_days_reduce_f32(const float *X_dev, int64_t T, int64_t n, int64_t ldx, const int32_t *row_begin_dev,
                             const int32_t *rows_dev, int32_t P, int64_t n_rows, const int32_t *doy_dev, const int32_t *win_dev,
                             double offset, const double *edges, int n_edges, int flags, float *out_dev, int64_t ldo,
                             int64_t out_pstride, int32_t *status_dev, void *work_dev, int64_t work_bytes, void *stream);
int wagg_bin_days_reduce_f64(const double *X_dev, int64_t T, int64_t n, int64_t ldx, const int32_t *row_begin_dev,
                             const int32_t *rows_dev, int32_t P, int64_t n_rows, const int32_t *doy_dev, const int32_t *win_dev,
                             double offset, const double *edges, int n_edges, int flags, double *out_dev, int64_t ldo,
                             int64_t out_pstride, int32_t *status_dev, void *work_dev, int64_t work_bytes, void *stream);
int64_t wagg_bin_days_work_bytes(int64_t n, int32_t P, int64_t n_rows, int n_edges);

#define WAGG_HINGE_MAX 64
#define WAGG_HINGE_GROUP 8
#define WAGG_HINGE_ABOVE 0
#define WAGG_HINGE_BELOW 1
int wagg_hinge_reduce_f32(const float *X_dev, int64_t T, int64_t n, int64_t ldx, const int32_t *row_begin_dev,
                          const int32_t *rows_dev, int32_t P, int64_t n_rows, const int32_t *doy_dev, const int32_t *win_dev,
                          double offset, const double *knots, int n_knots, int power, int side, const double *tail_knots,
                          const double *tail_a, const double *tail_b, int flags, float *out_dev, int64_t ldo, int64_t out_pstride,
                          int32_t *status_dev, void *work_dev, int64_t work_bytes, void *stream);
int wagg_hinge_reduce_f64(const double *X_dev, int64_t T, int64_t n, int64_t ldx, const int32_t *row_begin_dev,
                          const int32_t *rows_dev, int32_t P, int64_t n_rows, const int32_t *doy_dev, const int32_t *win_dev,
                          double offset, const double *knots, int n_knots, int power, int side, const double *tail_knots,
                          const double *tail_a, const double *tail_b, int flags, double *out_dev, int64_t ldo, int64_t out_pstride,
// ... 19 lines not shown
```

Measured before the change: 226300 billion.

## Precompute split fp16 hi/lo weight image at plan build for split kernel

```diff
diff --git a/climate_toolbox_amd/_lib.py b/climate_toolbox_amd/_lib.py
--- a/climate_toolbox_amd/_lib.py
+++ b/climate_toolbox_amd/_lib.py
@@ -30,7 +30,7 @@
     "wagg_any_less_f32", "wagg_any_less_f64",
     "wagg_dense_create_synth", "wagg_dense_create_host", "wagg_dense_create_from_segments", "wagg_dense_create_synth_blocklocal", "wagg_dense_create_synth_sparse", "wagg_dense_get_info",
     "wagg_dense_destroy", "wagg_dense_clone", "wagg_release_scratch", "wagg_scratch_bytes", "wagg_dense_get_den", "wagg_dense_apply_f32", "wagg_dense_apply_poly_f32",
-    "wagg_dense_apply_edd_f32", "wagg_dense_saw_inf",
+    "wagg_dense_apply_edd_f32", "wagg_dense_saw_inf", "wagg_dense_read_w",
     "wagg_dense_create_synth_f64", "wagg_dense_create_host_f64", "wagg_dense_create_from_segments_f64",
     "wagg_dense_create_synth_blocklocal_f64", "wagg_dense_apply_f64", "wagg_dense_apply_poly_f64", "wagg_dense_apply_edd_f64",
     "wagg_synth_field_f32", "wagg_synth_field_f64",
@@ -93,7 +93,7 @@
                 ("form", C.c_int32), ("elem_bytes", C.c_int32), ("nnz", C.c_int64),
                 ("build_s", C.c_double), ("build_upload_s", C.c_double),
                 ("est_full_s", C.c_double), ("est_tiles_s", C.c_double), ("est_entries_s", C.c_double), ("walked_entries", C.c_int64),
-                ("one_pass_sort", C.c_int32), ("reserved0", C.c_int32)]
+                ("one_pass_sort", C.c_int32), ("reserved0", C.c_int32), ("w_image_bytes", C.c_int64)]
 
 
 class WaggError(RuntimeError):
@@ -295,7 +295,11 @@
         getattr(L, name).argtypes = [vp, vp, vp, C.c_int64, C.c_int64, vp, C.c_int64, vp]
     for name in ("wagg_pack_rows_host_f32", "wagg_pack_rows_host_f64"):
         getattr(L, name).argtypes = [vp, vp, vp, C.c_int64, C.c_int64, vp, C.c_int64, C.c_int]
+    if hasattr(L, "wagg_dense_read_w"):
+        L.wagg_dense_read_w.argtypes = [vp, C.c_int, vp, C.c_uint64]
     for name in EXPORTS:
+        if name == "wagg_dense_read_w" and not hasattr(L, name):
+            continue
         fn = getattr(L, name)
         if name not in ("wagg_last_error", "wagg_scratch_bytes", "wagg_period_reduce_work_bytes", "wagg_season_reduce_work_bytes",
                         "wagg_edd_ladder_work_bytes", "wagg_bin_days_work_bytes", "wagg_hinge_work_bytes"):
diff --git a/climate_toolbox_amd/csrc/wagg_common.h b/climate_toolbox_amd/csrc/wagg_common.h
--- a/climate_toolbox_amd/csrc/wagg_common.h
+++ b/climate_toolbox_amd/csrc/wagg_common.h
@@ -168,6 +168,7 @@
     DevBuf(const DevBuf &) = delete;
     DevBuf &operator=(const DevBuf &) = delete;
     ~DevBuf() { if (p) (void)hipFree(p); }
+    void reset() { if (p) (void)hipFree(p); p = nullptr; n = 0; }
     hipError_t alloc(size_t count) {
         if (p) { (void)hipFree(p); p = nullptr; }
         n = count;
diff --git a/climate_toolbox_amd/csrc/wagg_dense.hip b/climate_toolbox_amd/csrc/wagg_dense.hip
--- a/climate_toolbox_amd/csrc/wagg_dense.hip
+++ b/climate_toolbox_amd/csrc/wagg_dense.hip
@@ -335,6 +335,7 @@
     return dense_den_to_host(d);
 }
 
+static void dense_build_image(wagg_dense *d, hipStream_t st);
 static int dense_finish_scales(wagg_dense *d, hipStream_t st = nullptr) {
     if (d->f64 || d->tiled || d->spmm) return WAGG_OK;
     const int kt_per_block = 128;
@@ -344,6 +345,7 @@
     hipLaunchKernelGGL(dense_colmax_kernel, dim3((unsigned)d->n_nt, (unsigned)n_strips), dim3(512), 0, st,
                        reinterpret_cast<const f32x4 *>(d->W.p), d->n_kt, kt_per_block, reinterpret_cast<unsigned *>(d->wmax.p));
     WAGG_HIP(hipGetLastError());
+    dense_build_image(d, st);
     return WAGG_OK;
 }
 
@@ -462,6 +464,24 @@
         if (eff >= 0.985) break;
     }
     return best;
+}
+
+static void dense_build_image(wagg_dense *d, hipStream_t st) {
+    if (d->f64 || d->tiled || d->spmm || !d->wmax.p || d->n_tiles <= 0) return;
+    const char *off = getenv("WAGG_DENSE_NO_W_IMAGE");
+    if (off && off[0] && off[0] != '0') return;
+    constexpr size_t bm = (size_t)DT<float>::MT_MAX * 16;
+    const size_t S = (size_t)pick_ksplit(d->n_nt, d->n_kt);
+    const size_t workspace = (size_t)d->n_kt * bm * D_ROWB + (size_t)d->n_nt * S * bm * D_BN * sizeof(float) + bm * sizeof(float);
+    const size_t bytes = (size_t)d->w_slots() * 16;
+    size_t free_b = 0, total_b = 0;
+    if (hipMemGetInfo(&free_b, &total_b) != hipSuccess) { (void)hipGetLastError(); return; }
+    if (free_b < bytes || free_b - bytes < workspace) return;
+    if (d->wimg.alloc(bytes / sizeof(float)) != hipSuccess) { (void)hipGetLastError(); d->wimg.reset(); return; }
+    const int64_t grid = d->n_tiles < (int64_t)d->ncu * 8 ? d->n_tiles : (int64_t)d->ncu * 8;
+    hipLaunchKernelGGL(dense_split_image_kernel, dim3((unsigned)grid), dim3(D_THREADS), 0, st, (const float *)d->W.p,
+                       (const float *)d->wmax.p, d->n_kt, d->n_tiles, d->wimg.p);
+    if (hipGetLastError() != hipSuccess) d->wimg.reset();
 }
 
 template <typename T>
@@ -773,8 +793,8 @@
 #undef WAGG_PICK
 }
 
-static const void *pick_split_kernel(int MT) {
-#define WAGG_PICK(M) case M: return (const void *)dense_split_kernel<M>
+static const void *pick_split_kernel(int MT, bool img) {
+#define WAGG_PICK(M) case M: return img ? (const void *)dense_split_kernel<M, 0, true> : (const void *)dense_split_kernel<M>
     switch (MT) {
         WAGG_PICK(1); WAGG_PICK(2); WAGG_PICK(3); WAGG_PICK(4); WAGG_PICK(5); WAGG_PICK(6); WAGG_PICK(8);
         WAGG_PICK(10); WAGG_PICK(12); WAGG_PICK(14); WAGG_PICK(16); WAGG_PICK(18); WAGG_PICK(20);
@@ -790,23 +810,27 @@
     const int kt_per_slice = (n_kt + S - 1) / S;
     const int64_t nblk = (int64_t)n_nt * n_mb * S;
     WAGG_REQUIRE(nblk < (int64_t)0x7fffffff, "grid too large");
-    const void *kern = pick_split_kernel(MT);
-    if (!kern) { set_error("no split kernel for MT=%d", MT); return WAGG_EINVAL; }
     const size_t need = (size_t)nblk * bm * D_BN;
     if (d->slabs.n < need) WAGG_HIP(d->slabs.alloc(need));
     const int64_t x_slots = (int64_t)n_mb * n_kt * bm * 8;
     if (d->xp.n < (size_t)x_slots * 4) WAGG_HIP(d->xp.alloc((size_t)x_slots * 4));
     if (d->xmax.n < (size_t)Tn) WAGG_HIP(d->xmax.alloc((size_t)Tn));
+    bool img = d->wimg.p != nullptr && n_mb == 1;
+#ifdef WAGG_DIAG
+    if (const char *e = getenv("WAGG_SPLIT_IMG")) img = img && e[0] != '0';
+#endif
+    const void *kern = pick_split_kernel(MT, img);
+    if (!kern) { set_error("no split kernel for MT=%d", MT); return WAGG_EINVAL; }
     const int aligned = ((ldx * sizeof(float)) % 16 == 0) && ((reinterpret_cast<uintptr_t>(X_dev) & 15) == 0) &&
                         (xf.mode != XF_EDD || (reinterpret_cast<uintptr_t>(xf.X2) & 15) == 0);
 #ifdef WAGG_DIAG
     if (const char *dbg = MT == D_MT ? getenv("WAGG_SPLIT_DBG") : nullptr) {
         switch (atoi(dbg)) {
-            case 1: kern = (const void *)dense_split_kernel<D_MT, 1>; break;
-            case 4: kern = (const void *)dense_split_kernel<D_MT, 4>; break;
-            case 5: kern = (const void *)dense_split_kernel<D_MT, 5>; break;
-            case 8: kern = (const void *)dense_split_kernel<D_MT, 8>; break;
-            case 9: kern = (const void *)dense_split_kernel<D_MT, 9>; break;
+            case 1: kern = img ? (const void *)dense_split_kernel<D_MT, 1, true> : (const void *)dense_split_kernel<D_MT, 1>; break;
+            case 4: kern = img ? (const void *)dense_split_kernel<D_MT, 4, true> : (const void *)dense_split_kernel<D_MT, 4>; break;
+            case 5: kern = img ? (const void *)dense_split_kernel<D_MT, 5, true> : (const void *)dense_split_kernel<D_MT, 5>; break;
+            case 8: kern = (const void *)dense_split_kernel<D_MT, 8>; img = false; break;
+            case 9: kern = (const void *)dense_split_kernel<D_MT, 9>; img = false; break;
             default: break;
         }
     }
@@ -821,7 +845,7 @@
                        (const unsigned *)xmax, reinterpret_cast<f16x8 *>(d->xp.p), xf, d->inf_dev);
     WAGG_HIP(hipGetLastError());
     const f16x8 *xp = reinterpret_cast<const f16x8 *>(d->xp.p);
-    const float *wp = d->W.p, *wmax = d->wmax.p;
+    const float *wp = img ? d->wimg.p : d->W.p, *wmax = d->wmax.p;
     float *slabs = d->slabs.p;
     int n_kt_a = n_kt, n_nt_a = n_nt, n_mb_a = n_mb, S_a = S, kps = kt_per_slice;
     void *args[] = {&xp, &wp, &wmax, &n_kt_a, &n_nt_a, &n_mb_a, &S_a, &kps, &slabs};
@@ -1056,6 +1080,7 @@
     info->walked_entries = d->walked_entries;
     info->one_pass_sort = d->one_pass_sort ? 1 : 0;
     info->reserved0 = 0;
+    info->w_image_bytes = d->wimg.p ? d->w_slots() * 16 : 0;
     copy_sized(info_buf, size, &st, sizeof(st));
     return WAGG_OK;
 }
@@ -1108,6 +1133,7 @@
         if (e == hipSuccess) e = clone_buf(d->tile_kt, device, src->tile_kt, src->device);
         if (e == hipSuccess) e = clone_buf(d->sp.ent, device, src->sp.ent, src->device);
         if (e == hipSuccess) e = clone_buf(d->sp.grp_off, device, src->sp.grp_off, src->device);
+        if (e == hipSuccess) dense_build_image(d, nullptr);
         if (e == hipSuccess) e = hipStreamSynchronize(nullptr);
         d->build.total_s = d->build.device_s = wall_s() - t0;
     } catch (const std::bad_alloc &) {
@@ -1128,6 +1154,19 @@
 
 extern "C" int wagg_dense_destroy(wagg_dense *d) {
     delete d;
+    return WAGG_OK;
+}
+
+extern "C" int wagg_dense_read_w(const wagg_dense *d, int image, void *host, uint64_t bytes) {
+    using namespace wagg;
+    clear_error();
+    WAGG_REQUIRE(d && host, "NULL argument");
+    WAGG_REQUIRE(!d->spmm, "an entry-list plan holds no W matrix");
+    const float *src = image ? d->wimg.p : d->W.p;
+    WAGG_REQUIRE(src != nullptr, "the plan holds no image of W");
+    WAGG_REQUIRE(bytes == (uint64_t)d->w_slots() * 16, "W is %lld bytes, the buffer %llu", (long long)d->w_slots() * 16,
+                 (unsigned long long)bytes);
+    WAGG_HIP(hipMemcpy(host, src, bytes, hipMemcpyDeviceToHost));
     return WAGG_OK;
 }
 
diff --git a/climate_toolbox_amd/csrc/wagg_dense_int.h b/climate_toolbox_amd/csrc/wagg_dense_int.h
--- a/climate_toolbox_amd/csrc/wagg_dense_int.h
+++ b/climate_toolbox_amd/csrc/wagg_dense_int.h
@@ -63,6 +63,7 @@
     wagg::DevBuf<float> W, den32, slabs, xp;
     wagg::DevBuf<double> den64;
     wagg::DevBuf<float> wmax, xmax;
+    wagg::DevBuf<float> wimg;
     std::vector<double> den_host;
     bool tiled = false;
     int64_t n_tiles = 0;
diff --git a/climate_toolbox_amd/csrc/wagg_dense_split.inc b/climate_toolbox_amd/csrc/wagg_dense_split.inc
--- a/climate_toolbox_amd/csrc/wagg_dense_split.inc
+++ b/climate_toolbox_amd/csrc/wagg_dense_split.inc
@@ -36,7 +36,10 @@
     return __builtin_amdgcn_make_buffer_rsrc(reinterpret_cast<void *>(u), (short)0, bytes, 0x00020000);
 }
 
-template <int MT, int DBG = 0>
+__device__ __forceinline__ unsigned split_frag0(int lr, int kq) { return (lr * 8 + (kq ^ (lr >> 1))) * 16; }
+__device__ __forceinline__ unsigned split_frag1(int lr, int kq) { return (lr * 8 + ((kq ^ (lr >> 1)) ^ 4)) * 16; }
+
+template <int MT, int DBG = 0, bool IMG = false>
 __global__ __launch_bounds__(D_THREADS, 2) void dense_split_kernel(
     const f16x8 *__restrict__ Xp, const float *__restrict__ Wp, const float *__restrict__ wmax, int n_kt, int n_nt, int n_mb,
     int S, int kt_per_slice, float *__restrict__ slabs) {
@@ -62,12 +65,11 @@
     const int kt1 = kt0 + kt_per_slice < n_kt ? kt0 + kt_per_slice : n_kt;
     const int ntiles = kt1 > kt0 ? kt1 - kt0 : 0;
     const int64_t w_first = (int64_t)nt * n_kt + kt0;
-    const int ew0 = split_exp(wmax[nt * D_BN + wave * 32 + lr]);
-    const int ew1 = split_exp(wmax[nt * D_BN + wave * 32 + 16 + lr]);
-
-    const int f = lr >> 1;
-    const unsigned frag0 = (lr * 8 + (kq ^ f)) * 16;
-    const unsigned frag1 = (lr * 8 + ((kq ^ f) ^ 4)) * 16;
+    const int ew0 = IMG ? 0 : split_exp(wmax[nt * D_BN + wave * 32 + lr]);
+    const int ew1 = IMG ? 0 : split_exp(wmax[nt * D_BN + wave * 32 + 16 + lr]);
+
+    const unsigned frag0 = split_frag0(lr, kq);
+    const unsigned frag1 = split_frag1(lr, kq);
     const char *xslice = reinterpret_cast<const char *>(Xp) + ((int64_t)mb * n_kt + kt0) * XT4;
     const char *wslice = reinterpret_cast<const char *>(Wp) + w_first * D_WTB;
     const unsigned lane16 = lane * 16;
@@ -89,13 +91,13 @@
         if constexpr (NXP > 4) WAGG_DMA_X(NXP > 4 ? 4 : 0, xr_, buf);                             \
         if constexpr (NXP > 5) WAGG_DMA_X(NXP > 5 ? 5 : 0, xr_, buf);                             \
     } while (0)
-#define WAGG_LOAD_W(tile)                                                                         \
+#define WAGG_LOAD_W(tile, D00, D01, D10, D11)                                                     \
     do {                                                                                          \
         const auto wr_ = WAGG_RSRC(wslice + (int64_t)(tile) * D_WTB, D_WTB);                      \
-        b00 = __builtin_bit_cast(f32x4, __builtin_amdgcn_raw_buffer_load_b128(wr_, wfrag0, 0, 0));        \
-        b01 = __builtin_bit_cast(f32x4, __builtin_amdgcn_raw_buffer_load_b128(wr_, wfrag1, 0, 0));        \
-        b10 = __builtin_bit_cast(f32x4, __builtin_amdgcn_raw_buffer_load_b128(wr_, wfrag0 + 2048, 0, 0)); \
-        b11 = __builtin_bit_cast(f32x4, __builtin_amdgcn_raw_buffer_load_b128(wr_, wfrag1 + 2048, 0, 0)); \
+        D00 = __builtin_bit_cast(f32x4, __builtin_amdgcn_raw_buffer_load_b128(wr_, wfrag0, 0, 0));        \
+        D01 = __builtin_bit_cast(f32x4, __builtin_amdgcn_raw_buffer_load_b128(wr_, wfrag1, 0, 0));        \
+        D10 = __builtin_bit_cast(f32x4, __builtin_amdgcn_raw_buffer_load_b128(wr_, wfrag0 + 2048, 0, 0)); \
+        D11 = __builtin_bit_cast(f32x4, __builtin_amdgcn_raw_buffer_load_b128(wr_, wfrag1 + 2048, 0, 0)); \
     } while (0)
 
     f32x4 acc[MT][2];
@@ -105,7 +107,7 @@
     f32x4 b00, b01, b10, b11;
     if (ntiles > 0) {
         const int t1 = ntiles > 1 ? 1 : 0;
-        WAGG_LOAD_W(0);
+        WAGG_LOAD_W(0, b00, b01, b10, b11);
         WAGG_DMA_XALL(0, 0);
         WAGG_DMA_XALL(t1, 1);
         asm volatile("s_waitcnt vmcnt(0)" ::: "memory");
@@ -114,7 +116,7 @@
 
 #define WAGG_SPLIT(A, B, E, HI, LO)                                                               \
     do {                                                                                          \
-        if constexpr (DBG & 8) { HI = __builtin_bit_cast(f16x8, A); LO = __builtin_bit_cast(f16x8, B); } \
+        if constexpr (IMG || (DBG & 8)) { HI = __builtin_bit_cast(f16x8, A); LO = __builtin_bit_cast(f16x8, B); } \
         else split_w8(A, B, E, HI, LO);                                                           \
     } while (0)
 #define WAGG_MFMA16(RB, CB, A, B) acc[RB][CB] = __builtin_amdgcn_mfma_f32_16x16x32_f16(A, B, acc[RB][CB], 0, 0, 0)
@@ -157,54 +159,65 @@
         }                                                                                         \
     } while (0)
 
+#define WAGG_TILE(tile, C00, C01, C10, C11, N00, N01, N10, N11)                                                               \
+    do {                                                                                                                      \
+        const char *img = lds + bcur * XT4;                                                                                   \
+        const int bfar = bcur == 0 ? 2 : bcur - 1;                             \
+        const int tnext = (tile) + 1 < ntiles ? (tile) + 1 : ntiles - 1;  \
+        const int tfar = (tile) + 2 < ntiles ? (tile) + 2 : ntiles - 1;                                                       \
+        const auto xfar = WAGG_RSRC(xslice + (int64_t)tfar * XT4, XT4);                                                       \
+        f16x8 wh0, wl0, wh1, wl1, aAh, aAl, aBh, aBl;                                                                         \
+                 \
+        WAGG_READ_A(aAh, aAl, 0);                                                                                             \
+        WAGG_SPLIT(C00, C01, ew0, wh0, wl0);                                                                                  \
+        if constexpr (MT > 1) WAGG_READ_A(aBh, aBl, MT > 1 ? 1 : 0);                                                          \
+        __builtin_amdgcn_sched_barrier(0);                                                                                    \
+        WAGG_MFMA16(0, 0, aAh, wl0);                                                                                          \
+        WAGG_MFMA16(0, 0, aAl, wh0);                                                                                          \
+        WAGG_MFMA16(0, 0, aAh, wh0);                                                                                          \
+        if constexpr (MT > 1) {                                                                                               \
+            WAGG_MFMA16(MT > 1 ? 1 : 0, 0, aBh, wl0);                                                                         \
+            WAGG_MFMA16(MT > 1 ? 1 : 0, 0, aBl, wh0);                                                                         \
+            WAGG_MFMA16(MT > 1 ? 1 : 0, 0, aBh, wh0);                                                                         \
+        }                                                                                                                     \
+        WAGG_SPLIT(C10, C11, ew1, wh1, wl1);                                                                                  \
+        __builtin_amdgcn_sched_barrier(0);                                                                                    \
+        if constexpr (!(DBG & 1)) WAGG_LOAD_W(tnext, N00, N01, N10, N11);                                                     \
+        __builtin_amdgcn_sched_barrier(0);                                                                                    \
+        WAGG_MFMA16(0, 1, aAh, wl1);                                                                                          \
+        WAGG_MFMA16(0, 1, aAl, wh1);                                                                                          \
+        WAGG_MFMA16(0, 1, aAh, wh1);                                                                                          \
+        __builtin_amdgcn_sched_barrier(0);                                                                                    \
+        if constexpr (MT > 2) WAGG_READ_A(aAh, aAl, MT > 2 ? 2 : 0);                                                          \
+        __builtin_amdgcn_sched_barrier(0);                                                                                    \
+        if constexpr (MT > 1) {                                                                                               \
+            WAGG_MFMA16(MT > 1 ? 1 : 0, 1, aBh, wl1);                                                                         \
+            WAGG_MFMA16(MT > 1 ? 1 : 0, 1, aBl, wh1);                                                                         \
+            WAGG_MFMA16(MT > 1 ? 1 : 0, 1, aBh, wh1);                                                                         \
+        }                                                                                                                     \
+        __builtin_amdgcn_sched_barrier(0);                                                                                    \
+        WAGG_DMA_BLOCK(0); WAGG_DMA_BLOCK(1);                                                                                 \
+        WAGG_BLOCK(2); WAGG_BLOCK(3); WAGG_BLOCK(4); WAGG_BLOCK(5);                                                           \
+        WAGG_BLOCK(6); WAGG_BLOCK(7); WAGG_BLOCK(8); WAGG_BLOCK(9); WAGG_BLOCK(10); WAGG_BLOCK(11);                           \
+        WAGG_BLOCK(12); WAGG_BLOCK(13); WAGG_BLOCK(14); WAGG_BLOCK(15); WAGG_BLOCK(16); WAGG_BLOCK(17);                       \
+        WAGG_BLOCK(18); WAGG_BLOCK(19); WAGG_BLOCK(20); WAGG_BLOCK(21); WAGG_BLOCK(22);                                       \
+        static_assert(MT <= 23, "row blocks are written out up to 22");                                                       \
+        __builtin_amdgcn_sched_barrier(0);                                                                                    \
+        if constexpr (!(DBG & 4)) {                                                                                           \
+            __builtin_amdgcn_s_waitcnt(WAIT_TILE);                                                                            \
+            __builtin_amdgcn_s_barrier();                                                                                     \
+        }                                                                                                                     \
+        bcur = bcur == 2 ? 0 : bcur + 1;                                                                                      \
+    } while (0)
     int bcur = 0;
-    for (int tile = 0; tile < ntiles; ++tile) {
-        const char *img = lds + bcur * XT4;
-        const int bfar = bcur == 0 ? 2 : bcur - 1;
-        const int tnext = tile + 1 < ntiles ? tile + 1 : ntiles - 1;
-        const int tfar = tile + 2 < ntiles ? tile + 2 : ntiles - 1;
-        const auto xfar = WAGG_RSRC(xslice + (int64_t)tfar * XT4, XT4);
-        f16x8 wh0, wl0, wh1, wl1, aAh, aAl, aBh, aBl;
-        WAGG_READ_A(aAh, aAl, 0);
-        WAGG_SPLIT(b00, b01, ew0, wh0, wl0);
-        if constexpr (MT > 1) WAGG_READ_A(aBh, aBl, MT > 1 ? 1 : 0);
-        __builtin_amdgcn_sched_barrier(0);
-        WAGG_MFMA16(0, 0, aAh, wl0);
-        WAGG_MFMA16(0, 0, aAl, wh0);
-        WAGG_MFMA16(0, 0, aAh, wh0);
-        if constexpr (MT > 1) {
-            WAGG_MFMA16(MT > 1 ? 1 : 0, 0, aBh, wl0);
-            WAGG_MFMA16(MT > 1 ? 1 : 0, 0, aBl, wh0);
-            WAGG_MFMA16(MT > 1 ? 1 : 0, 0, aBh, wh0);
+    if constexpr (IMG) {
+        f32x4 d00, d01, d10, d11;
+        for (int tile = 0; tile < ntiles; tile += 2) {
+            WAGG_TILE(tile, b00, b01, b10, b11, d00, d01, d10, d11);
+            if (tile + 1 < ntiles) WAGG_TILE(tile + 1, d00, d01, d10, d11, b00, b01, b10, b11);
         }
-        WAGG_SPLIT(b10, b11, ew1, wh1, wl1);
-        __builtin_amdgcn_sched_barrier(0);
-        if constexpr (!(DBG & 1)) WAGG_LOAD_W(tnext);
-        __builtin_amdgcn_sched_barrier(0);
-        WAGG_MFMA16(0, 1, aAh, wl1);
-        WAGG_MFMA16(0, 1, aAl, wh1);
-        WAGG_MFMA16(0, 1, aAh, wh1);
-        __builtin_amdgcn_sched_barrier(0);
-        if constexpr (MT > 2) WAGG_READ_A(aAh, aAl, MT > 2 ? 2 : 0);
-        __builtin_amdgcn_sched_barrier(0);
-        if constexpr (MT > 1) {
-            WAGG_MFMA16(MT > 1 ? 1 : 0, 1, aBh, wl1);
-            WAGG_MFMA16(MT > 1 ? 1 : 0, 1, aBl, wh1);
-            WAGG_MFMA16(MT > 1 ? 1 : 0, 1, aBh, wh1);
-        }
-        __builtin_amdgcn_sched_barrier(0);
-        WAGG_DMA_BLOCK(0); WAGG_DMA_BLOCK(1);
-        WAGG_BLOCK(2); WAGG_BLOCK(3); WAGG_BLOCK(4); WAGG_BLOCK(5);
-        WAGG_BLOCK(6); WAGG_BLOCK(7); WAGG_BLOCK(8); WAGG_BLOCK(9); WAGG_BLOCK(10); WAGG_BLOCK(11);
-        WAGG_BLOCK(12); WAGG_BLOCK(13); WAGG_BLOCK(14); WAGG_BLOCK(15); WAGG_BLOCK(16); WAGG_BLOCK(17);
-        WAGG_BLOCK(18); WAGG_BLOCK(19); WAGG_BLOCK(20); WAGG_BLOCK(21); WAGG_BLOCK(22);
-        static_assert(MT <= 23, "row blocks are written out up to 22");
-        __builtin_amdgcn_sched_barrier(0);
-        if constexpr (!(DBG & 4)) {
-            __builtin_amdgcn_s_waitcnt(WAIT_TILE);
-            __builtin_amdgcn_s_barrier();
-        }
-        bcur = bcur == 2 ? 0 : bcur + 1;
+    } else {
+        for (int tile = 0; tile < ntiles; ++tile) WAGG_TILE(tile, b00, b01, b10, b11, b00, b01, b10, b11);
     }
     asm volatile("s_waitcnt vmcnt(0)" ::: "memory");
 
@@ -227,6 +240,30 @@
 #undef WAGG_READ_A
 #undef WAGG_BLOCK_
 #undef WAGG_BLOCK
+#undef WAGG_TILE
+}
+
+__global__ __launch_bounds__(D_THREADS) void dense_split_image_kernel(const float *__restrict__ Wp, const float *__restrict__ wmax,
+                                                                      int n_kt, int64_t n_tiles, float *__restrict__ image) {
+    const int lane = threadIdx.x & 63, wave = threadIdx.x >> 6;
+    const int lr = lane & 15, kq = lane >> 4;
+    const unsigned wfrag0 = wave * 4096 + split_frag0(lr, kq), wfrag1 = wave * 4096 + split_frag1(lr, kq);
+    for (int64_t t = blockIdx.x; t < n_tiles; t += gridDim.x) {
+        const int64_t nt = t / n_kt;
+        const int ew0 = split_exp(wmax[nt * D_BN + wave * 32 + lr]);
+        const int ew1 = split_exp(wmax[nt * D_BN + wave * 32 + 16 + lr]);
+        const char *src = reinterpret_cast<const char *>(Wp) + t * D_WTB;
+        char *dst = reinterpret_cast<char *>(image) + t * D_WTB;
+        const f32x4 b00 = *reinterpret_cast<const f32x4 *>(src + wfrag0), b01 = *reinterpret_cast<const f32x4 *>(src + wfrag1);
+        const f32x4 b10 = *reinterpret_cast<const f32x4 *>(src + wfrag0 + 2048), b11 = *reinterpret_cast<const f32x4 *>(src + wfrag1 + 2048);
+        f16x8 wh0, wl0, wh1, wl1;
+        split_w8(b00, b01, ew0, wh0, wl0);
+        split_w8(b10, b11, ew1, wh1, wl1);
+        *reinterpret_cast<f16x8 *>(dst + wfrag0) = wh0;
+        *reinterpret_cast<f16x8 *>(dst + wfrag1) = wl0;
+        *reinterpret_cast<f16x8 *>(dst + wfrag0 + 2048) = wh1;
+        *reinterpret_cast<f16x8 *>(dst + wfrag1 + 2048) = wl1;
+    }
 }
 
 __global__ void dense_rowmax_kernel(const float *__restrict__ X, int64_t ldx, int64_t G, PackXfT<float> xf,
diff --git a/climate_toolbox_amd/csrc/wagg_desc.hip b/climate_toolbox_amd/csrc/wagg_desc.hip
--- a/climate_toolbox_amd/csrc/wagg_desc.hip
+++ b/climate_toolbox_amd/csrc/wagg_desc.hip
@@ -341,8 +341,8 @@
     number(a1, a2, a3, a4, a5, a6, a7, a8, a9, a10, a11, a12, a13, a14, a15, a16, a17, a18, a19);
 }
 void ordinals(wagg_dense_info &s) {
-    auto &[a1, a2, a3, a4, a5, a6, a7, a8, a9, a10, a11, a12, a13, a14, a15, a16] = s;
-    number(a1, a2, a3, a4, a5, a6, a7, a8, a9, a10, a11, a12, a13, a14, a15, a16);
+    auto &[a1, a2, a3, a4, a5, a6, a7, a8, a9, a10, a11, a12, a13, a14, a15, a16, a17] = s;
+    number(a1, a2, a3, a4, a5, a6, a7, a8, a9, a10, a11, a12, a13, a14, a15, a16, a17);
 }
 void ordinals(wagg_host_stats &s) {
     auto &[a1, a2, a3, a4, a5, a6, a7, a8, a9, a10, a11, a12, a13, a14, a15, a16, a17, a18] = s;
diff --git a/climate_toolbox_amd/engine.py b/climate_toolbox_amd/engine.py
--- a/climate_toolbox_amd/engine.py
+++ b/climate_toolbox_amd/engine.py
@@ -465,6 +465,12 @@
         _lib.check(_lib.load().wagg_dense_clone(self._h, int(device), C.byref(h)), "wagg_dense_clone")
         return type(self)(h, self.G, self.R, int(device))
 
+    def read_w(self, image=False):
+        fn = _lib.load().wagg_dense_read_w
+        buf = np.empty(self.info["w_bytes"], dtype=np.uint8)
+        _lib.check(fn(self._h, 1 if image else 0, buf.ctypes.data_as(C.c_void_p), buf.nbytes), "wagg_dense_read_w")
+        return buf
+
     def close(self):
         for r in getattr(self, "_replicas", {}).values():
             r.close()
diff --git a/include/wagg.h b/include/wagg.h
--- a/include/wagg.h
+++ b/include/wagg.h
@@ -218,6 +218,7 @@
     double est_row_s[3];
     int64_t walked_entries;
     int32_t one_pass_sort, reserved0;
+    int64_t w_image_bytes;
 } wagg_dense_info;
 int wagg_dense_get_info(const wagg_dense *d, wagg_dense_info *info);
 int wagg_dense_get_info_sized(const wagg_dense *d, void *info, uint64_t size);
@@ -226,6 +227,7 @@
 int wagg_dense_clone(const wagg_dense *src, int device, wagg_dense **out);
 int wagg_dense_destroy(wagg_dense *d);
 int wagg_dense_get_den(const wagg_dense *d, double *den_host );
+int wagg_dense_read_w(const wagg_dense *d, int image, void *host, uint64_t bytes);
 int wagg_dense_apply_f32(wagg_dense *d, const float *X_dev, int64_t T, int64_t ldx,
                          float *out_dev, int64_t ldo, int ksplit, void *stream);
 int wagg_dense_apply_f64(wagg_dense *d, const double *X_dev, int64_t T, int64_t ldx,
```

Result: faster. 233400 billion (median of 6 runs) (+3.1%).
